# Beryl2000/SE-UNet-AirSeg

Measured on AMD Instinct MI355X. Metric: voxels/sec SE-UNet fwd+bwd, 128^3 patch, higher is better.
Workload: dtype bf16

## Files before the change

### include/seunet_hip.h

```cpp
#ifndef SEUNET_HIP_H
#define SEUNET_HIP_H
#include <stddef.h>

#ifdef __cplusplus
extern "C" {
#endif

#ifndef SEUNET_F32
#define SEUNET_F32 0
#define SEUNET_BF16 1
#define SEUNET_F16 2
#endif
#define SEUNET_CONV_MFMA 0
#define SEUNET_CONV_NAIVE 1
#define SEUNET_CONV_MARCH 2
#define SEUNET_CONV_TILED 3

typedef void* seunet_stream_t;
typedef struct seunet_dims { int n, d, h, w; } seunet_dims;

int seunet_version(void);
const char* seunet_last_error(void);
int seunet_init(int device);

int seunet_pack_cl(int dtype, const float* in_ncdhw, int c, void* out_cl, int c_pad, seunet_dims dims, seunet_stream_t s);
int seunet_unpack_cl(int dtype, const void* in_cl, int c, float* out_ncdhw, seunet_dims dims, seunet_stream_t s);

size_t seunet_conv_wpack_bytes(int dtype, int taps, int cin, int cout);
int seunet_conv_pack_weights(int dtype, const float* w, int taps, int cin, int cout, int transpose_flip, void* wpack, seunet_stream_t s);
int seunet_conv_stats_slots(int impl, int taps, int dilation, seunet_dims dims);
int seunet_conv3d_fwd(int dtype, int impl, int taps, int dilation, int nsrc, const void* const* src, const int* src_c,
                      int cin, const void* weights, int transpose_flip, const float* bias, int ndst, void* const* dst,
                      const int* dst_c, const int* dst_accumulate, double* stats_partial, seunet_dims dims, seunet_stream_t s);
int seunet_conv3d_stream_supported(int dtype, int dilation, int src_c, int dst_c);
size_t seunet_conv3d_stream_wpack_bytes(int src_c);
int seunet_conv3d_stream_slots(int dilation, seunet_dims dims);
int seunet_conv3d_stream_pack(int dtype, const float* w, int cin_w, int cout_w, int transpose_flip, int src_c, int dst_c, void* wpack,
                              seunet_stream_t s);
int seunet_conv3d_stream(int dtype, int dilation, const void* src, int src_c, const void* wpack, const float* bias, void* dst, int dst_c,
                         int dst_accumulate, double* stats_partial, seunet_dims dims, seunet_stream_t s);
int seunet_conv3d_march_supported(int dtype, int dilation, int nsrc, const int* src_c, int ndst, const int* dst_c);
size_t seunet_conv3d_march_wpack_bytes(int cin, int cout);
int seunet_conv3d_march_slots(int dilation, int cin, int cout, seunet_dims dims);
int seunet_conv3d_march_pack(int dtype, const float* w, int cin_w, int cout_w, int transpose_flip, int cin, int cout, void* wpack,
                             seunet_stream_t s);
int seunet_conv3d_march(int dtype, int dilation, int nsrc, const void* const* src, const int* src_c, const void* wpack, const float* bias,
                        int ndst, void* const* dst, const int* dst_c, const int* dst_accumulate, double* stats_partial, seunet_dims dims,
                        seunet_stream_t s);
int seunet_conv3d_wgrad_stream_supported(int dtype, int dilation, int x_c, int dy_c);
size_t seunet_conv3d_wgrad_stream_workspace_bytes(int x_c, int dy_c, int dilation, seunet_dims dims);
int seunet_conv3d_wgrad_stream(int dtype, int dilation, const void* x, int x_c, int cin, const void* dy, int dy_c, int cout, float* dw,
                               void* workspace, size_t workspace_bytes, seunet_dims dims, seunet_stream_t s);
size_t seunet_conv3d_wgrad_workspace_bytes(int taps, int cin, int cout);
int seunet_conv3d_wgrad(int dtype, int impl, int taps, int dilation, int nsrc, const void* const* src, const int* src_c,
                        int cin, const void* dy, int cout, float* dw, void* workspace, size_t workspace_bytes,
                        seunet_dims dims, seunet_stream_t s);

int seunet_epilogue_slots(seunet_dims dims);
int seunet_channel_stats(int dtype, const void* t, int c, double* partial, seunet_dims dims, seunet_stream_t s);
int seunet_stats_finalize(const double* partial, int slots, int c, int n, long long count, float eps, int mode,
                          float* out_a, float* out_b, seunet_stream_t s);

int seunet_gate_epilogue_fwd(int dtype, const void* raw, const float* mean, const float* rstd, int c, const float* w_se,
                             const float* w_se2, const float* w_side, const float* b_side, float slope, void* e_out,
                             float* side_out, float* level_map, int level_accumulate, const float* head_w,
                             const float* drop, int drop_stride, seunet_dims dims, seunet_stream_t s);
int seunet_gate_epilogue_bwd(int dtype, const void* raw, const float* mean, const float* rstd, int c, const float* w_se,
                             const float* w_se2, const float* w_side, const float* b_side, float slope, const void* g_e,
                             const float* g_side, const float* g_level, const float* head_w, const float* drop,
                             int drop_stride, const float* m1, const float* m2, void* draw_out, double* stat_partial,
                             float* pgrad_partial, seunet_dims dims, seunet_stream_t s);
int seunet_pgrad_reduce(const float* pgrad_partial, int records, int c, float* dw_se, float* dw_se2, float* dw_side,
                        float* db_side, float* dhead_w, seunet_stream_t s);
int seunet_gate_bwd_finalize(const double* stat_partial, int slots, int c, int n, long long count, float* m1, float* m2,
                             const float* pgrad_partial, int records, float* dw_se, float* dw_se2, float* dw_side,
                             float* db_side, float* dhead_w, seunet_stream_t s);

int seunet_cat_epilogue_fwd(int dtype, const void* raw, const float* mean, const float* rstd, const void* raw2,
                            const float* mean2, const float* rstd2, int c, float slope, void* out, seunet_dims dims,
                            seunet_stream_t s);
int seunet_cat_epilogue_bwd(int dtype, const void* g_out, const void* raw, const float* mean, const float* rstd,
                            const void* raw2, const float* mean2, const float* rstd2, int c, float slope,
                            const float* m1, const float* m2, const float* m1b, const float* m2b, void* dx, void* dx2,
                            double* stat_partial, double* stat_partial2, seunet_dims dims, seunet_stream_t s);

int seunet_xbranch_moment_slots(seunet_dims dims);
int seunet_xbranch_moments(int dtype, const void* x_in, double* partial , seunet_dims dims, seunet_stream_t s);
int seunet_xbranch_stats(const double* partial, int slots, const float* w2, int c, int in_channel, int n, long long count,
                         float eps, float* mean2, float* rstd2, double* moments_out , seunet_stream_t s);
int seunet_cat_epilogue_fwd_x(int dtype, const void* raw, const float* mean, const float* rstd, const void* x_in,
                              const float* w2, int in_channel, const float* mean2, const float* rstd2, int c, float slope,
                              void* out, seunet_dims dims, seunet_stream_t s);
int seunet_cat_epilogue_bwd_x(int dtype, const void* g_out, const void* raw, const float* mean, const float* rstd,
                              const void* x_in, const float* w2, int in_channel, const float* mean2, const float* rstd2,
                              int c, float slope, const float* m1, const float* m2, const float* m1b, const float* m2b,
                              void* dx, double* stat_partial, double* stat_partial2, double* xw_partial, seunet_dims dims,
                              seunet_stream_t s);
int seunet_cat_epilogue_fwd_x_pool(int dtype, const void* raw, const float* mean, const float* rstd, const void* x_in,
                                   const float* w2, int in_channel, const float* mean2, const float* rstd2, int c, float slope,
                                   void* out, void* pooled, unsigned int* argmax, seunet_dims dims, seunet_stream_t s);
int seunet_cat_epilogue_bwd_x_pool(int dtype, const void* g_out, const void* raw, const float* mean, const float* rstd,
                                   const void* x_in, const float* w2, int in_channel, const float* mean2, const float* rstd2,
                                   int c, float slope, const float* m1, const float* m2, const float* m1b, const float* m2b,
                                   void* dx, double* stat_partial, double* stat_partial2, double* xw_partial,
                                   const unsigned int* pool_argmax, const void* pool_g, seunet_dims dims, seunet_stream_t s);
int seunet_cat_xgrad_finalize(const double* xw_partial, const double* stat_partial2, int slots, const double* moments,
                              const float* w2, int c, int in_channel, int n, float eps, float* dw, seunet_stream_t s);

int seunet_maxpool_fwd(int dtype, const void* in, int c, void* out, seunet_dims in_dims, seunet_stream_t s);
int seunet_maxpool_bwd(int dtype, const void* in, const void* g_out, int c, void* g_in, int accumulate,
                       seunet_dims in_dims, seunet_stream_t s);
int seunet_upsample2_fwd(int dtype, const void* in, int c, void* out, seunet_dims in_dims, seunet_stream_t s);
int seunet_upsample2_bwd(int dtype, const void* g_out, int c, void* g_in, int accumulate, seunet_dims in_dims,
                         seunet_stream_t s);
int seunet_side_upsample(const float* side, int c, int scale, float* out_ncdhw, int c_total, int c_off,
                         seunet_dims low_dims, seunet_stream_t s);

int seunet_head_fwd(const float* const* level_maps, int nlevels, const float* bias, float* pred, seunet_dims dims,
                    seunet_stream_t s);
size_t seunet_head_bwd_tmp_floats(seunet_dims dims);
int seunet_head_bwd(const float* g_pred, float* const* g_levels, int nlevels, float* tmp, float* g_bias,
                    seunet_dims dims, seunet_stream_t s);

#define SEUNET_LOSS_DICE 1
#define SEUNET_LOSS_GUL 2
#define SEUNET_LOSS_ATR 4
int seunet_loss_partial_floats(void);
int seunet_loss_sums(const float* pred, int apply_sigmoid, const float* target, const float* weight, const float* skel,
                     long long n, float* partial, double* sums, int terms, seunet_stream_t s);
int seunet_loss_value(const double* sums0, double c_dice0, double c_gul0, double c_atr0, const double* sums1, double c_dice1,
                      double c_gul1, double c_atr1, float* value, seunet_stream_t s);
int seunet_loss_grad(const float* pred, int apply_sigmoid, const float* target, const float* weight, const float* skel,
                     long long n, const double* sums, float c_dice, float c_gul, float c_atr, float g_scale,
                     const float* g_scale_dev, float* g_pred, seunet_stream_t s);

int seunet_loss_sample_partial_floats(int batch);
int seunet_loss_sums_per_sample(const float* pred, int apply_sigmoid, const float* target, const float* weight, const float* skel,
                                int batch, long long n_per_sample, float* partial, double* sums, int terms, seunet_stream_t s);
int seunet_loss_sample_values(const double* sums, int batch, double c_dice, double c_gul, double c_atr, float* values,
                              seunet_stream_t s);

int seunet_pool_select(const float* new_keys, int batch, float* keys, long long* seq, long long* state, int capacity, int* slots_out,
                       seunet_stream_t s);
int seunet_pool_scatter(const int* slots_dev, int batch, int capacity, long long voxels, const float* data, const float* label,
                        const float* weight, const float* skel, float* pool_data, unsigned char* pool_label, float* pool_weight,
                        unsigned char* pool_skel, seunet_stream_t s);
int seunet_pool_gather(const int* slots_host, int n, int capacity, long long voxels, const float* pool_data,
                       const unsigned char* pool_label, const float* pool_weight, const unsigned char* pool_skel, float* data_out,
                       float* label_out, float* weight_out, float* skel_out, seunet_stream_t s);

int seunet_adamw_step(float* const* params, const float* const* grads, float* const* exp_avg, float* const* exp_avg_sq,
                      const long long* counts, int n_tensors, double lr, double beta1, double beta2, double eps,
                      double weight_decay, int step, int maximize, seunet_stream_t s);

#define SEUNET_IMG_I16 0
#define SEUNET_IMG_F32 1
#define SEUNET_W_F16 0
#define SEUNET_W_F32 1
#define SEUNET_W_F64 2
int seunet_crop_batch(const void* img, int img_dtype, const unsigned char* label, const void* weight, int weight_dtype,
                      const unsigned char* skeleton, int d, int h, int w, int cube, int ncrop, const int* starts, const int* aug,
                      double weight_exponent, int f64_math, float* data_out, float* label_out, float* weight_out, float* skel_out,
                      seunet_stream_t s);
int seunet_hu_two_channel(const void* img, int img_dtype, long long nvox, int f64_math, float* out, seunet_stream_t s);

int seunet_window_gather(const float* volume, int c, int x, int y, int z, int cube, int nwin, const int* starts, float* out,
                         seunet_stream_t s);
int seunet_window_accumulate(const float* logits, int apply_sigmoid, int nwin, const int* starts, int cube, double* acc, int x, int y,
                             int z, seunet_stream_t s);
int seunet_window_finalize(const double* acc, int x, int y, int z, int cube, int nx, const int* xs, int ny, const int* ys, int nz,
                           const int* zs, int dup0, double* out, seunet_stream_t s);

#define SEUNET_DTI_F64 0
#define SEUNET_DTI_F32 1
size_t seunet_dti_workspace_bytes(int h, int w, int z);
int seunet_dti(const double* pred, int h, int w, int z, double h_thresh, double l_thresh, int pred_dtype, unsigned char* out,
               void* workspace, size_t workspace_bytes, seunet_stream_t s);

#define SEUNET_CC_EVALUATION 0
#define SEUNET_CC_MAXIMUM_3D 1
#define SEUNET_CC_LARGEST_FILLED 2
size_t seunet_cc_workspace_bytes(int h, int w, int z);
int seunet_largest_component(const unsigned char* volume, int h, int w, int z, int rule, unsigned char* out, int* status_dev,
                             void* workspace, size_t workspace_bytes, seunet_stream_t s);
size_t seunet_metric_out_bytes(int nbins);
int seunet_metric_sums(const unsigned char* pred, const unsigned char* label, const unsigned char* skeleton, const int* parsing,
                       long long n, int nbins, void* out, size_t out_bytes, seunet_stream_t s);

size_t seunet_edt_workspace_bytes(int n0, int n1, int n2);
int seunet_edt(const unsigned char* volume, int n0, int n1, int n2, int* sqdist, double* dist, int* indices, int* status_dev,
               void* workspace, size_t workspace_bytes, seunet_stream_t s);
int seunet_mask_bits(const unsigned char* mask, long long n, unsigned long long* bits, seunet_stream_t s);
int seunet_hard_mining_masks(const unsigned char* label, const unsigned char* skeleton, const unsigned char* pred, int n0, int n1,
                             int n2, unsigned long long* skeleton_bits, unsigned long long* small_bits, seunet_stream_t s);
size_t seunet_lib_weight_workspace_bytes(int n0, int n1, int n2);
int seunet_lib_weight(const unsigned char* label, int n0, int n1, int n2, const float* table, void* out, void* workspace,
                      size_t workspace_bytes, seunet_stream_t s);
size_t seunet_break_weight_workspace_bytes(int n0, int n1, int n2);
int seunet_break_weight(const unsigned char* label, const unsigned char* pred, const unsigned char* skeleton, int n0, int n1, int n2,
                        void* w_br, unsigned char* br_skel, int* status_dev, void* workspace, size_t workspace_bytes,
                        seunet_stream_t s);

size_t seunet_skeleton_workspace_bytes(int n0, int n1, int n2);
int seunet_skeletonize(const unsigned char* volume, int n0, int n1, int n2, unsigned char* out, int* passes_dev, void* workspace,
                       size_t workspace_bytes, seunet_stream_t s);

size_t seunet_skeleton_branches_workspace_bytes(int n0, int n1, int n2);
int seunet_skeleton_branches(const unsigned char* skeleton, int n0, int n1, int n2, int min_voxels, int* cd, unsigned char* skeleton_parse,
                             int* num_dev, void* workspace, size_t workspace_bytes, seunet_stream_t s);
size_t seunet_parse_assign_workspace_bytes(int n0, int n1, int n2);
int seunet_parse_assign(const unsigned char* skeleton_parse, const int* cd, const unsigned char* label, int n0, int n1, int n2,
                        int* parsing, int* status_dev, void* workspace, size_t workspace_bytes, seunet_stream_t s);
int seunet_label_stats_max_num(void);
int seunet_label_stats(const int* parsing, int n0, int n1, int n2, int num, unsigned int* counts, unsigned long long* adjacency_bits,
                       int* status_dev, seunet_stream_t s);
int seunet_relabel(const int* parsing, long long n, const int* lut, int nlut, int* out, seunet_stream_t s);

#define SEUNET_MORPH_DILATE 0
#define SEUNET_MORPH_ERODE_BORDER0 1
#define SEUNET_MORPH_ERODE_BORDER1 2
#define SEUNET_MORPH_CLOSE 3
size_t seunet_binary_morph_workspace_bytes(int n0, int n1, int n2);
int seunet_binary_morph(const unsigned char* volume, int n0, int n1, int n2, int op, unsigned char* out, void* workspace,
                        size_t workspace_bytes, seunet_stream_t s);
int seunet_fill_holes(const unsigned char* volume, int n0, int n1, int n2, unsigned char* out, void* workspace, size_t workspace_bytes,
                      seunet_stream_t s);
int seunet_slice_moments(const unsigned char* mask, int n0, int n1, int n2, int k, unsigned long long* out_dev, seunet_stream_t s);
int seunet_scatter_labels(const long long* lin_index_dev, const int* value_dev, long long m, long long n, int* cd,
                          unsigned char* skeleton_parse, int* status_dev, seunet_stream_t s);

size_t seunet_mesh_workspace_bytes(int n0, int n1, int n2);
int seunet_mesh_count(const unsigned char* volume, int n0, int n1, int n2, long long* nverts, long long* nfaces, void* workspace,
                      size_t workspace_bytes, seunet_stream_t s);
int seunet_mesh_emit(int n0, int n1, int n2, double level, long long nverts, long long nfaces, float* verts, int* faces,
                     const void* workspace, size_t workspace_bytes, seunet_stream_t s);
int seunet_mesh_coord_sums(const unsigned char* mask, int n0, int n1, int n2, long long* sums_dev, seunet_stream_t s);
size_t seunet_mesh_adjacency_workspace_bytes(long long nverts, long long nfaces);
int seunet_mesh_adjacency(const int* faces, long long nfaces, long long nverts, int* indptr, int* indices, long long indices_capacity,
                          unsigned char* boundary, int* status_dev, void* workspace, size_t workspace_bytes, seunet_stream_t s);
int seunet_mesh_smooth(const float* verts, long long nverts, const int* indptr, const int* indices, const unsigned char* boundary,
                       int n_iter, float relaxation_factor, float* out, float* tmp, seunet_stream_t s);
int seunet_mesh_affine(const float* verts, long long nverts, const float* centre, const float* scale, float* out, seunet_stream_t s);
int seunet_mesh_stl_records(const float* verts, long long nverts, const int* faces, long long nfaces, const float* centre,
                            const float* scale, unsigned char* records, int* status_dev, seunet_stream_t s);

size_t seunet_mesh_label_workspace_bytes(int n0, int n1, int n2);
size_t seunet_mesh_label_sort_bytes(long long nverts, long long nfaces);
int seunet_mesh_label_count(const int* labels, int n0, int n1, int n2, int num, long long* nverts, long long* nfaces, int* num_used,
                            int* status, long long* vert_ptr_dev, long long* face_ptr_dev, int ptr_capacity, void* workspace,
                            size_t workspace_bytes, seunet_stream_t s);
int seunet_mesh_label_emit(const int* labels, int n0, int n1, int n2, int num, double level, long long nverts, long long nfaces,
                           float* verts, int* faces, const void* workspace, size_t workspace_bytes, void* sort_workspace,
                           size_t sort_bytes, seunet_stream_t s);

int seunet_value_counts(const short* ct, long long n, int shift, unsigned int* counts, seunet_stream_t s);
int seunet_shift_clamp(const short* ct, long long n, int shift, int clamp, int clamp_le, int clamp_to, short* out, seunet_stream_t s);
size_t seunet_get_l_workspace_bytes(int h, int w, int z);
int seunet_get_l(const short* ct, int h, int w, int z, double T, int min_area, unsigned char* out, void* workspace,
                 size_t workspace_bytes, seunet_stream_t s);
int seunet_mask_combine(const unsigned char* a, const unsigned char* b, long long n, int op, unsigned char* out, seunet_stream_t s);
int seunet_mask_box(const unsigned char* mask, int h, int w, int z, int* box_dev, seunet_stream_t s);
int seunet_crop3d(const void* src, int elem_bytes, int h, int w, int z, const int* box, void* dst, seunet_stream_t s);

typedef struct seunet_net_desc {
  int batch, in_channel, n_classes;
  int d, h, w;
  int width_mult;
  int dtype;
  int conv_impl;
  float negative_slope;
  float eps;
} seunet_net_desc;

int seunet_net_param_count(const seunet_net_desc* desc);
int seunet_net_param_info(const seunet_net_desc* desc, int index, char* name, int name_cap, int* shape5, int* ndim);
size_t seunet_net_workspace_bytes(const seunet_net_desc* desc);
int seunet_net_forward(const seunet_net_desc* desc, const float* const* params, const float* x, const float* drop1,
                       const float* drop2, float* pred0, float* pred1, void* workspace, size_t workspace_bytes,
                       seunet_stream_t s);
int seunet_net_forward_capture(const seunet_net_desc* desc, const float* const* params, const float* x, const float* drop1,
                               const float* drop2, float* pred0, float* pred1, void* workspace, size_t workspace_bytes,
                               seunet_stream_t s, void** graph_out);
int seunet_graph_launch(void* graph, seunet_stream_t s);
int seunet_graph_destroy(void* graph);
int seunet_net_read_tensor(const seunet_net_desc* desc, const float* const* params, const void* workspace, size_t workspace_bytes,
                           const char* name, int which, float* out, int* channels, seunet_stream_t s);
#define SEUNET_KERNEL_NAIVE 0
#define SEUNET_KERNEL_TILED 1
#define SEUNET_KERNEL_STREAM 2
#define SEUNET_KERNEL_MARCH 3
#define SEUNET_KERNEL_WGRAD1X1 4
typedef struct seunet_conv_info {
  char name[16];
  int taps, dilation, level;
  seunet_dims dims;
  int nsrc, src_c[3], src_is_input[3];
  int cin, cout;
  int need_dgrad;
  int fwd, dgrad, wgrad;
  char x_name[16];
  int x_materialised, x_fwd, x_wgrad;
  long long src_dist;
} seunet_conv_info;
int seunet_net_conv_info(const seunet_net_desc* desc, int index, seunet_conv_info* out);
int seunet_net_backward(const seunet_net_desc* desc, const float* const* params, const float* g_pred0,
                        const float* g_pred1, const float* drop1, const float* drop2, float* const* grads,
                        void* workspace, size_t workspace_bytes, seunet_stream_t s);
int seunet_net_backward_ev(const seunet_net_desc* desc, const float* const* params, const float* g_pred0,
                           const float* g_pred1, const float* drop1, const float* drop2, float* const* grads,
                           void* workspace, size_t workspace_bytes, seunet_stream_t s, void* decoder_done_event);
size_t seunet_net_input_grad_bytes(const seunet_net_desc* desc);
int seunet_net_backward_input(const seunet_net_desc* desc, const float* const* params, const float* g_pred0,
                              const float* g_pred1, const float* drop1, const float* drop2, float* const* grads, float* grad_x,
                              void* scratch, size_t scratch_bytes, void* workspace, size_t workspace_bytes, seunet_stream_t s,
                              void* decoder_done_event);

int seunet_prof_enable(int on);
int seunet_prof_enable_filtered(const char* tag_substring);
int seunet_prof_report(char* buf, size_t cap);

#ifdef __cplusplus
}
#endif
#endif
```

### se-unet-airseg_amd/_lib.py

```python
from __future__ import annotations

import ctypes as C
import os
from typing import Optional, Sequence

_HERE = os.path.dirname(os.path.abspath(__file__))
LIB_PATH = os.environ.get("SEUNET_LIB") or os.path.join(_HERE, "libseunet_hip.so")

F32, BF16, F16 = 0, 1, 2
CONV_MFMA, CONV_NAIVE, CONV_MARCH, CONV_TILED = 0, 1, 2, 3
LOSS_NSUMS = 7
DTI_F64, DTI_F32 = 0, 1
CC_EVALUATION, CC_MAXIMUM_3D, CC_LARGEST_FILLED = 0, 1, 2
MORPH_DILATE, MORPH_ERODE_BORDER0, MORPH_ERODE_BORDER1, MORPH_CLOSE = 0, 1, 2, 3


class Dims(C.Structure):
    _fields_ = [("n", C.c_int), ("d", C.c_int), ("h", C.c_int), ("w", C.c_int)]


class NetDesc(C.Structure):
    _fields_ = [("batch", C.c_int), ("in_channel", C.c_int), ("n_classes", C.c_int),
                ("d", C.c_int), ("h", C.c_int), ("w", C.c_int), ("width_mult", C.c_int),
                ("dtype", C.c_int), ("conv_impl", C.c_int),
                ("negative_slope", C.c_float), ("eps", C.c_float)]


KERNEL_NAIVE, KERNEL_TILED, KERNEL_STREAM, KERNEL_MARCH, KERNEL_WGRAD1X1 = range(5)
KERNEL_NAMES = ("Naive", "Tiled", "Stream", "March", "Wgrad1x1")


class ConvInfo(C.Structure):
    _fields_ = [("name", C.c_char * 16), ("taps", C.c_int), ("dilation", C.c_int), ("level", C.c_int), ("dims", Dims),
                ("nsrc", C.c_int), ("src_c", C.c_int * 3), ("src_is_input", C.c_int * 3), ("cin", C.c_int), ("cout", C.c_int),
                ("need_dgrad", C.c_int), ("fwd", C.c_int), ("dgrad", C.c_int), ("wgrad", C.c_int),
                ("x_name", C.c_char * 16), ("x_materialised", C.c_int), ("x_fwd", C.c_int), ("x_wgrad", C.c_int),
                ("src_dist", C.c_longlong)]


_vp, _i, _f, _ll, _sz, _d =C.c_void_p, C.c_int, C.c_float, C.c_longlong, C.c_size_t, C.c_double
_pp = C.POINTER(C.c_void_p)
_ip = C.POINTER(C.c_int)

PROTOTYPES = {
    "seunet_version": (_i, []),
    "seunet_last_error": (C.c_char_p, []),
    "seunet_pack_cl": (_i, [_i, _vp, _i, _vp, _i, Dims, _vp]),
    "seunet_unpack_cl": (_i, [_i, _vp, _i, _vp, Dims, _vp]),
    "seunet_conv_wpack_bytes": (_sz, [_i, _i, _i, _i]),
    "seunet_conv_pack_weights": (_i, [_i, _vp, _i, _i, _i, _i, _vp, _vp]),
    "seunet_conv_stats_slots": (_i, [_i, _i, _i, Dims]),
    "seunet_conv3d_fwd": (_i, [_i, _i, _i, _i, _i, _pp, _ip, _i, _vp, _i, _vp, _i, _pp, _ip, _ip, _vp, Dims, _vp]),
    "seunet_conv3d_stream_supported": (_i, [_i, _i, _i, _i]),
    "seunet_conv3d_stream_wpack_bytes": (_sz, [_i]),
    "seunet_conv3d_stream_slots": (_i, [_i, Dims]),
    "seunet_conv3d_stream_pack": (_i, [_i, _vp, _i, _i, _i, _i, _i, _vp, _vp]),
    "seunet_conv3d_stream": (_i, [_i, _i, _vp, _i, _vp, _vp, _vp, _i, _i, _vp, Dims, _vp]),
    "seunet_conv3d_march_supported": (_i, [_i, _i, _i, _ip, _i, _ip]),
    "seunet_conv3d_march_wpack_bytes": (_sz, [_i, _i]),
    "seunet_conv3d_march_slots": (_i, [_i, _i, _i, Dims]),
    "seunet_conv3d_march_pack": (_i, [_i, _vp, _i, _i, _i, _i, _i, _vp, _vp]),
    "seunet_conv3d_march": (_i, [_i, _i, _i, _pp, _ip, _vp, _vp, _i, _pp, _ip, _ip, _vp, Dims, _vp]),
    "seunet_conv3d_wgrad_stream_supported": (_i, [_i, _i, _i, _i]),
    "seunet_conv3d_wgrad_stream_workspace_bytes": (_sz, [_i, _i, _i, Dims]),
    "seunet_conv3d_wgrad_stream": (_i, [_i, _i, _vp, _i, _i, _vp, _i, _i, _vp, _vp, _sz, Dims, _vp]),
    "seunet_conv3d_wgrad_workspace_bytes": (_sz, [_i, _i, _i]),
    "seunet_conv3d_wgrad": (_i, [_i, _i, _i, _i, _i, _pp, _ip, _i, _vp, _i, _vp, _vp, _sz, Dims, _vp]),
    "seunet_epilogue_slots": (_i, [Dims]),
    "seunet_channel_stats": (_i, [_i, _vp, _i, _vp, Dims, _vp]),
    "seunet_stats_finalize": (_i, [_vp, _i, _i, _i, _ll, _f, _i, _vp, _vp, _vp]),
    "seunet_gate_epilogue_fwd": (_i, [_i, _vp, _vp, _vp, _i, _vp, _vp, _vp, _vp, _f, _vp, _vp, _vp, _i, _vp, _vp, _i, Dims, _vp]),
    "seunet_gate_epilogue_bwd": (_i, [_i, _vp, _vp, _vp, _i, _vp, _vp, _vp, _vp, _f, _vp, _vp, _vp, _vp, _vp, _i, _vp, _vp, _vp, _vp, _vp, Dims, _vp]),
    "seunet_pgrad_reduce": (_i, [_vp, _i, _i, _vp, _vp, _vp, _vp, _vp, _vp]),
    "seunet_gate_bwd_finalize": (_i, [_vp, _i, _i, _i, _ll, _vp, _vp, _vp, _i, _vp, _vp, _vp, _vp, _vp, _vp]),
    "seunet_cat_epilogue_fwd": (_i, [_i, _vp, _vp, _vp, _vp, _vp, _vp, _i, _f, _vp, Dims, _vp]),
    "seunet_cat_epilogue_bwd": (_i, [_i, _vp, _vp, _vp, _vp, _vp, _vp, _vp, _i, _f, _vp, _vp, _vp, _vp, _vp, _vp, _vp, _vp, Dims, _vp]),
    "seunet_maxpool_fwd": (_i, [_i, _vp, _i, _vp, Dims, _vp]),
    "seunet_maxpool_bwd": (_i, [_i, _vp, _vp, _i, _vp, _i, Dims, _vp]),
    "seunet_upsample2_fwd": (_i, [_i, _vp, _i, _vp, Dims, _vp]),
    "seunet_upsample2_bwd": (_i, [_i, _vp, _i, _vp, _i, Dims, _vp]),
    "seunet_side_upsample": (_i, [_vp, _i, _i, _vp, _i, _i, Dims, _vp]),
    "seunet_head_fwd": (_i, [_pp, _i, _vp, _vp, Dims, _vp]),
    "seunet_head_bwd_tmp_floats": (_sz, [Dims]),
    "seunet_head_bwd": (_i, [_vp, _pp, _i, _vp, _vp, Dims, _vp]),
    "seunet_loss_partial_floats": (_i, []),
    "seunet_loss_sums": (_i, [_vp, _i, _vp, _vp, _vp, _ll, _vp, _vp, _i, _vp]),
    "seunet_loss_value": (_i, [_vp, _d, _d, _d, _vp, _d, _d, _d, _vp, _vp]),
    "seunet_loss_grad": (_i, [_vp, _i, _vp, _vp, _vp, _ll, _vp, _f, _f, _f, _f, _vp, _vp, _vp]),
    "seunet_loss_sample_partial_floats": (_i, [_i]),
    "seunet_loss_sums_per_sample": (_i, [_vp, _i, _vp, _vp, _vp, _i, _ll, _vp, _vp, _i, _vp]),
    "seunet_loss_sample_values": (_i, [_vp, _i, _d, _d, _d, _vp, _vp]),
    "seunet_pool_select": (_i, [_vp, _i, _vp, _vp, _vp, _i, _vp, _vp]),
    "seunet_pool_scatter": (_i, [_vp, _i, _i, _ll, _vp, _vp, _vp, _vp, _vp, _vp, _vp, _vp, _vp]),
    "seunet_pool_gather": (_i, [_ip, _i, _i, _ll, _vp, _vp, _vp, _vp, _vp, _vp, _vp, _vp, _vp]),
    "seunet_xbranch_moment_slots": (_i, [Dims]),
    "seunet_xbranch_moments": (_i, [_i, _vp, _vp, Dims, _vp]),
    "seunet_xbranch_stats": (_i, [_vp, _i, _vp, _i, _i, _i, _ll, _f, _vp, _vp, _vp, _vp]),
    "seunet_cat_epilogue_fwd_x": (_i, [_i, _vp, _vp, _vp, _vp, _vp, _i, _vp, _vp, _i, _f, _vp, Dims, _vp]),
    "seunet_cat_epilogue_bwd_x": (_i, [_i, _vp, _vp, _vp, _vp, _vp, _vp, _i, _vp, _vp, _i, _f, _vp, _vp, _vp, _vp, _vp, _vp, _vp, _vp, Dims, _vp]),
    "seunet_cat_epilogue_fwd_x_pool": (_i, [_i, _vp, _vp, _vp, _vp, _vp, _i, _vp, _vp, _i, _f, _vp, _vp, _vp, Dims, _vp]),
    "seunet_cat_epilogue_bwd_x_pool": (_i, [_i, _vp, _vp, _vp, _vp, _vp, _vp, _i, _vp, _vp, _i, _f, _vp, _vp, _vp, _vp, _vp, _vp, _vp, _vp, _vp, _vp, Dims, _vp]),
    "seunet_cat_xgrad_finalize": (_i, [_vp, _vp, _i, _vp, _vp, _i, _i, _i, _f, _vp, _vp]),
    "seunet_cc_workspace_bytes": (_sz, [_i, _i, _i]),
    "seunet_largest_component": (_i, [_vp, _i, _i, _i, _i, _vp, _vp, _vp, _sz, _vp]),
    "seunet_metric_out_bytes": (_sz, [_i]),
    "seunet_metric_sums": (_i, [_vp, _vp, _vp, _vp, _ll, _i, _vp, _sz, _vp]),
    "seunet_value_counts": (_i, [_vp, _ll, _i, _vp, _vp]),
    "seunet_shift_clamp": (_i, [_vp, _ll, _i, _i, _i, _i, _vp, _vp]),
    "seunet_get_l_workspace_bytes": (_sz, [_i, _i, _i]),
    "seunet_get_l": (_i, [_vp, _i, _i, _i, _d, _i, _vp, _vp, _sz, _vp]),
    "seunet_mask_combine": (_i, [_vp, _vp, _ll, _i, _vp, _vp]),
    "seunet_mask_box": (_i, [_vp, _i, _i, _i, _vp, _vp]),
    "seunet_crop3d": (_i, [_vp, _i, _i, _i, _i, _ip, _vp, _vp]),
    "seunet_crop_batch": (_i, [_vp, _i, _vp, _vp, _i, _vp, _i, _i, _i, _i, _i, _ip, _ip, C.c_double, _i, _vp, _vp, _vp, _vp, _vp]),
    "seunet_hu_two_channel": (_i, [_vp, _i, _ll, _i, _vp, _vp]),
    "seunet_window_gather": (_i, [_vp, _i, _i, _i, _i, _i, _i, _ip, _vp, _vp]),
    "seunet_window_accumulate": (_i, [_vp, _i, _i, _ip, _i, _vp, _i, _i, _i, _vp]),
    "seunet_window_finalize": (_i, [_vp, _i, _i, _i, _i, _i, _ip, _i, _ip, _i, _ip, _i, _vp, _vp]),
    "seunet_dti_workspace_bytes": (_sz, [_i, _i, _i]),
    "seunet_dti": (_i, [_vp, _i, _i, _i, C.c_double, C.c_double, _i, _vp, _vp, _sz, _vp]),
    "seunet_edt_workspace_bytes": (_sz, [_i, _i, _i]),
    "seunet_edt": (_i, [_vp, _i, _i, _i, _vp, _vp, _vp, _vp, _vp, _sz, _vp]),
    "seunet_mask_bits": (_i, [_vp, _ll, _vp, _vp]),
    "seunet_hard_mining_masks": (_i, [_vp, _vp, _vp, _i, _i, _i, _vp, _vp, _vp]),
    "seunet_lib_weight_workspace_bytes": (_sz, [_i, _i, _i]),
    "seunet_lib_weight": (_i, [_vp, _i, _i, _i, _vp, _vp, _vp, _sz, _vp]),
    "seunet_break_weight_workspace_bytes": (_sz, [_i, _i, _i]),
    "seunet_break_weight": (_i, [_vp, _vp, _vp, _i, _i, _i, _vp, _vp, _vp, _vp, _sz, _vp]),
    "seunet_skeleton_workspace_bytes": (_sz, [_i, _i, _i]),
    "seunet_skeletonize": (_i, [_vp, _i, _i, _i, _vp, _vp, _vp, _sz, _vp]),
    "seunet_skeleton_branches_workspace_bytes": (_sz, [_i, _i, _i]),
    "seunet_skeleton_branches": (_i, [_vp, _i, _i, _i, _i, _vp, _vp, _vp, _vp, _sz, _vp]),
    "seunet_parse_assign_workspace_bytes": (_sz, [_i, _i, _i]),
    "seunet_parse_assign": (_i, [_vp, _vp, _vp, _i, _i, _i, _vp, _vp, _vp, _sz, _vp]),
    "seunet_label_stats_max_num": (_i, []),
    "seunet_label_stats": (_i, [_vp, _i, _i, _i, _i, _vp, _vp, _vp, _vp]),
    "seunet_relabel": (_i, [_vp, _ll, _vp, _i, _vp, _vp]),
    "seunet_binary_morph_workspace_bytes": (_sz, [_i, _i, _i]),
    "seunet_binary_morph": (_i, [_vp, _i, _i, _i, _i, _vp, _vp, _sz, _vp]),
    "seunet_fill_holes": (_i, [_vp, _i, _i, _i, _vp, _vp, _sz, _vp]),
    "seunet_slice_moments": (_i, [_vp, _i, _i, _i, _i, _vp, _vp]),
    "seunet_scatter_labels": (_i, [_vp, _vp, _ll, _ll, _vp, _vp, _vp, _vp]),
    "seunet_mesh_workspace_bytes": (_sz, [_i, _i, _i]),
    "seunet_mesh_count": (_i, [_vp, _i, _i, _i, C.POINTER(_ll), C.POINTER(_ll), _vp, _sz, _vp]),
    "seunet_mesh_emit": (_i, [_i, _i, _i, _d, _ll, _ll, _vp, _vp, _vp, _sz, _vp]),
    "seunet_mesh_label_workspace_bytes": (_sz, [_i, _i, _i]),
    "seunet_mesh_label_sort_bytes": (_sz, [_ll, _ll]),
    "seunet_mesh_label_count": (_i, [_vp, _i, _i, _i, _i, C.POINTER(_ll), C.POINTER(_ll), _ip, _ip, _vp, _vp, _i, _vp, _sz, _vp]),
    "seunet_mesh_label_emit": (_i, [_vp, _i, _i, _i, _i, _d, _ll, _ll, _vp, _vp, _vp, _sz, _vp, _sz, _vp]),
    "seunet_mesh_coord_sums": (_i, [_vp, _i, _i, _i, _vp, _vp]),
    "seunet_mesh_adjacency_workspace_bytes": (_sz, [_ll, _ll]),
    "seunet_mesh_adjacency": (_i, [_vp, _ll, _ll, _vp, _vp, _ll, _vp, _vp, _vp, _sz, _vp]),
    "seunet_mesh_smooth": (_i, [_vp, _ll, _vp, _vp, _vp, _i, _f, _vp, _vp, _vp]),
    "seunet_mesh_affine": (_i, [_vp, _ll, C.POINTER(_f), C.POINTER(_f), _vp, _vp]),
    "seunet_mesh_stl_records": (_i, [_vp, _ll, _vp, _ll, C.POINTER(_f), C.POINTER(_f), _vp, _vp, _vp]),
    "seunet_adamw_step": (_i, [_vp, _vp, _vp, _vp, _vp, _i, C.c_double, C.c_double, C.c_double, C.c_double, C.c_double, _i, _i, _vp]),
    "seunet_net_param_count": (_i, [C.POINTER(NetDesc)]),
    "seunet_net_param_info": (_i, [C.POINTER(NetDesc), _i, C.c_char_p, _i, _ip, _ip]),
    "seunet_net_workspace_bytes": (_sz, [C.POINTER(NetDesc)]),
    "seunet_net_forward": (_i, [C.POINTER(NetDesc), _pp, _vp, _vp, _vp, _vp, _vp, _vp, _sz, _vp]),
    "seunet_prof_enable": (_i, [_i]),
    "seunet_prof_enable_filtered": (_i, [C.c_char_p]),
    "seunet_prof_report": (_i, [C.c_char_p, _sz]),
    "seunet_init": (_i, [_i]),
    "seunet_net_forward_capture": (_i, [C.POINTER(NetDesc), _pp, _vp, _vp, _vp, _vp, _vp, _vp, _sz, _vp, C.POINTER(C.c_void_p)]),
    "seunet_graph_launch": (_i, [_vp, _vp]),
    "seunet_graph_destroy": (_i, [_vp]),
    "seunet_net_read_tensor": (_i, [C.POINTER(NetDesc), _pp, _vp, _sz, C.c_char_p, _i, _vp, _ip, _vp]),
    "seunet_net_conv_info": (_i, [C.POINTER(NetDesc), _i, C.POINTER(ConvInfo)]),
    "seunet_net_backward": (_i, [C.POINTER(NetDesc), _pp, _vp, _vp, _vp, _vp, _pp, _vp, _sz, _vp]),
    "seunet_net_backward_ev": (_i, [C.POINTER(NetDesc), _pp, _vp, _vp, _vp, _vp, _pp, _vp, _sz, _vp, _vp]),
    "seunet_net_input_grad_bytes": (_sz, [C.POINTER(NetDesc)]),
    "seunet_net_backward_input": (_i, [C.POINTER(NetDesc), _pp, _vp, _vp, _vp, _vp, _pp, _vp, _vp, _sz, _vp, _sz, _vp, _vp]),
}

_lib: Optional[C.CDLL] = None


def load() -> C.CDLL:
    global _lib
    if _lib is not None:
        return _lib
    if not os.path.exists(LIB_PATH):
        raise RuntimeError(
            f"{LIB_PATH} is missing: build it with `python -c 'import __graft_entry__ as g; g.build()'` "
            "(or `make -C se-unet-airseg_amd/csrc`).  There is no CPU or PyTorch fallback for the HIP path.")
    lib = C.CDLL(LIB_PATH)
    for name, (res, args) in PROTOTYPES.items():
        fn = getattr(lib, name)
        fn.restype, fn.argtypes = res, args
    _lib = lib
    return lib


def last_error() -> str:
    return load().seunet_last_error().decode(errors="replace")


def check(status: int, what: str = "") -> None:
    if status != 0:
        raise RuntimeError(f"libseunet_hip {what}: {last_error()}")


def ptr(t) -> Optional[int]:
    return None if t is None else t.data_ptr()


def ptr_array(tensors: Sequence) -> C.Array:
    arr = (C.c_void_p * len(tensors))()
    for i, t in enumerate(tensors):
        arr[i] = None if t is None else (t if isinstance(t, int) else t.data_ptr())
    return arr


def int_array(vals: Sequence[int]) -> C.Array:
    return (C.c_int * len(vals))(*vals)


def stream_ptr() -> int:
    import torch
    return torch.cuda.current_stream().cuda_stream


def dtype_code(name: str) -> int:
    name = str(name).lower().replace("torch.", "")
    if name in ("bf16", "bfloat16"):
        return BF16
    if name in ("fp32", "f32", "float32", "float"):
        return F32
    if name in ("fp16", "f16", "float16", "half"):
        return F16
    raise ValueError(f"unsupported activation dtype {name!r} (fp32, bf16 or fp16)")
```

### se-unet-airseg_amd/csrc/abi.cpp

```cpp
#include "seunet_common.h"
#include "epilogue.h"
#include "volume.h"
#include "../../include/seunet_hip.h"

using namespace seunet;

static inline Dims D(seunet_dims d) { return Dims{d.n, d.d, d.h, d.w}; }
static inline hipStream_t S(seunet_stream_t s) { return reinterpret_cast<hipStream_t>(s); }

static int make_src(int nsrc, const void* const* src, const int* src_c, SrcList& l) {
  SEUNET_CHECK(nsrc >= 1 && nsrc <= 3 && src && src_c, "bad source list");
  l = SrcList{};
  l.n = nsrc;
  for (int i = 0; i < nsrc; ++i) { l.ptr[i] = src[i]; l.C[i] = src_c[i]; }
  return 0;
}

namespace seunet { extern unsigned long long* g_conv_debug; }

extern "C" {

int seunet_debug_set_buffer(void* p) { seunet::g_conv_debug = reinterpret_cast<unsigned long long*>(p); return 0; }
int seunet_debug_upsample2_form(int dtype, int c, seunet_dims dims, int backward) { return upsample2_form(dtype, c, D(dims), backward != 0); }

int seunet_debug_volume_layout(int op, int n0, int n1, int n2, size_t* offsets, int cap) {
  if (n0 < 1 || n1 < 1 || n2 < 1) return 0;
  size_t at[16];
  WsCarver c(nullptr);
  c.log = at;
  c.log_cap = 16;
  switch (op) {
    case 0: cc_ws(c, n0, n1, n2); break;
    case 1: get_l_ws(c, n0, n1, n2); break;
    case 2: case 8: edt_ws(c, n0, n1, n2); break;
    case 3: lib_weight_ws(c, n0, n1, n2); break;
    case 4: break_weight_ws(c, n0, n1, n2); break;
    case 5: branches_ws(c, n0, n1, n2); break;
    case 6: dti_ws(c, n0, n1, n2); break;
    case 7: if (!skeleton_ws(c, n0, n1, n2)) return 0; break;
    case 9: morph_ws(c, n0, n1, n2); break;
    case 10: if ((long long)n0 * n1 * n2 >= (1ll << 31)) return 0; mesh_ws(c, n0, n1, n2); break;
    case 11: if ((long long)n0 * n1 * n2 >= (1ll << 31)) return 0; mesh_label_ws(c, n0, n1, n2); break;
    default: return -1;
  }
  if (c.taken > c.log_cap) return -1;
  for (int i = 0; i < c.taken && i < cap && offsets; ++i) {
    offsets[2 * i] = at[i];
    offsets[2 * i + 1] = (i + 1 < c.taken ? at[i + 1] : c.bytes()) - at[i];
  }
  return c.taken;
}

int seunet_version(void) { return 201; }
const char* seunet_last_error(void) { return get_error(); }

int seunet_init(int device) {
  int count = 0, prev = 0;
  SEUNET_HIP(hipGetDeviceCount(&count));
  SEUNET_CHECK(device >= 0 && device < count, "init: device %d out of range (%d visible)", device, count);
  SEUNET_HIP(hipGetDevice(&prev));
  SEUNET_HIP(hipSetDevice(device));
  const void* page = seunet::device_zero_page();
  (void)hipSetDevice(prev);
  SEUNET_CHECK(page != nullptr, "init: could not allocate the zero page on device %d", device);
  return 0;
}

int seunet_pack_cl(int dtype, const float* in, int c, void* out, int c_pad, seunet_dims dims, seunet_stream_t s) {
  SEUNET_CHECK(in && out, "pack_cl: null tensor");
  return launch_pack_cl(dtype, in, c, out, c_pad, D(dims), S(s));
}
int seunet_unpack_cl(int dtype, const void* in, int c, float* out, seunet_dims dims, seunet_stream_t s) {
  SEUNET_CHECK(in && out, "unpack_cl: null tensor");
  return launch_unpack_cl(dtype, in, c, out, D(dims), S(s));
}

size_t seunet_conv_wpack_bytes(int dtype, int taps, int cin, int cout) { return conv_wpack_bytes(dtype, taps, cin, cout); }
int seunet_conv_pack_weights(int dtype, const float* w, int taps, int cin, int cout, int tflip, void* wpack, seunet_stream_t s) {
  SEUNET_CHECK(w && wpack, "conv_pack_weights: null tensor");
  return launch_conv_pack_weights(dtype, w, taps, cin, cout, tflip, wpack, S(s));
}
int seunet_conv_stats_slots(int impl, int taps, int dilation, seunet_dims dims) {
  return impl == SEUNET_CONV_NAIVE ? epi_partials(D(dims)) : conv_stats_tiles(D(dims), taps, dilation);
}
int seunet_conv3d_fwd(int dtype, int impl, int taps, int dilation, int nsrc, const void* const* src, const int* src_c, int cin,
                      const void* weights, int tflip, const float* bias, int ndst, void* const* dst, const int* dst_c,
                      const int* dst_acc, double* stats_partial, seunet_dims dims, seunet_stream_t s) {
  SrcList sl;
  if (int e = make_src(nsrc, src, src_c, sl)) return e;
  SEUNET_CHECK(ndst >= 1 && ndst <= 3 && dst && dst_c && weights, "conv3d_fwd: bad destination list / weights");
  DstList dl{};
  dl.n = ndst;
  for (int i = 0; i < ndst; ++i) { dl.ptr[i] = dst[i]; dl.C[i] = dst_c[i]; dl.acc[i] = dst_acc ? dst_acc[i] : 0; }
  if (impl == SEUNET_CONV_NAIVE) {
    if (int e = launch_conv_naive(dtype, taps, dilation, sl, cin, (const float*)weights, tflip, bias, dl, D(dims), S(s))) return e;
    if (stats_partial) {
      SEUNET_CHECK(ndst == 1, "conv3d_fwd: statistics need a single destination");
      return launch_channel_stats(dtype, dst[0], dst_c[0], stats_partial, D(dims), S(s));
    }
    return 0;
  }
  return launch_conv_igemm(dtype, taps, dilation, sl, cin, weights, bias, dl, stats_partial, D(dims), S(s));
}
int seunet_conv3d_stream_supported(int dtype, int dilation, int src_c, int dst_c) { return conv_stream_supported(dtype, 27, dilation, src_c, dst_c) ? 1 : 0; }
size_t seunet_conv3d_stream_wpack_bytes(int src_c) { return conv_stream_wpack_bytes(src_c); }
int seunet_conv3d_stream_slots(int dilation, seunet_dims dims) { return conv_stream_slots(D(dims), dilation); }
int seunet_conv3d_stream_pack(int dtype, const float* w, int cin_w, int cout_w, int transpose_flip, int src_c, int dst_c, void* wpack,
                              seunet_stream_t s) {
  return launch_conv_stream_pack(dtype, w, cin_w, cout_w, transpose_flip, src_c, dst_c, wpack, S(s));
}
int seunet_conv3d_stream(int dtype, int dilation, const void* src, int src_c, const void* wpack, const float* bias, void* dst, int dst_c,
                         int dst_accumulate, double* stats_partial, seunet_dims dims, seunet_stream_t s) {
  return launch_conv_stream(dtype, dilation, src, src_c, wpack, bias, dst, dst_c, dst_accumulate, stats_partial, D(dims), S(s));
}
static int make_dst(int ndst, void* const* dst, const int* dst_c, const int* dst_acc, DstList& dl) {
  SEUNET_CHECK(ndst >= 1 && ndst <= 3 && dst_c, "bad destination list");
  dl = DstList{};
  dl.n = ndst;
  for (int i = 0; i < ndst; ++i) { dl.ptr[i] = dst ? dst[i] : nullptr; dl.C[i] = dst_c[i]; dl.acc[i] = dst_acc ? dst_acc[i] : 0; }
  return 0;
}
int seunet_conv3d_march_supported(int dtype, int dilation, int nsrc, const int* src_c, int ndst, const int* dst_c) {
  if (nsrc < 1 || nsrc > 3 || ndst < 1 || ndst > 3 || !src_c || !dst_c) return 0;
  SrcList sl{}; DstList dl{};
  sl.n = nsrc; dl.n = ndst;
  for (int i = 0; i < nsrc; ++i) sl.C[i] = src_c[i];
  for (int i = 0; i < ndst; ++i) dl.C[i] = dst_c[i];
  return conv_march_supported(dtype, 27, dilation, sl, dl) ? 1 : 0;
}
size_t seunet_conv3d_march_wpack_bytes(int cin, int cout) { return conv_march_wpack_bytes(cin, cout); }
int seunet_conv3d_march_slots(int dilation, int cin, int cout, seunet_dims dims) { return conv_march_slots(D(dims), dilation, cin, cout); }
int seunet_conv3d_march_pack(int dtype, const float* w, int cin_w, int cout_w, int transpose_flip, int cin, int cout, void* wpack,
                             seunet_stream_t s) {
  return launch_conv_march_pack(dtype, w, cin_w, cout_w, transpose_flip, cin, cout, wpack, S(s));
}
int seunet_conv3d_march(int dtype, int dilation, int nsrc, const void* const* src, const int* src_c, const void* wpack, const float* bias,
                        int ndst, void* const* dst, const int* dst_c, const int* dst_accumulate, double* stats_partial, seunet_dims dims,
                        seunet_stream_t s) {
  SrcList sl; DstList dl;
  if (int e = make_src(nsrc, src, src_c, sl)) return e;
  SEUNET_CHECK(dst != nullptr, "conv3d_march: null destination list");
  if (int e = make_dst(ndst, dst, dst_c, dst_accumulate, dl)) return e;
  return launch_conv_march(dtype, dilation, sl, wpack, bias, dl, stats_partial, D(dims), S(s));
}
int seunet_conv3d_wgrad_stream_supported(int dtype, int dilation, int x_c, int dy_c) { return wgrad_stream_supported(dtype, 27, dilation, x_c, dy_c) ? 1 : 0; }
size_t seunet_conv3d_wgrad_stream_workspace_bytes(int x_c, int dy_c, int dilation, seunet_dims dims) {
  return wgrad_stream_workspace_bytes(x_c, dy_c, dilation, D(dims));
}
int seunet_conv3d_wgrad_stream(int dtype, int dilation, const void* x, int x_c, int cin, const void* dy, int dy_c, int cout, float* dw,
                               void* workspace, size_t workspace_bytes, seunet_dims dims, seunet_stream_t s) {
  return launch_wgrad_stream(dtype, dilation, x, x_c, cin, dy, dy_c, cout, dw, workspace, workspace_bytes, D(dims), S(s));
}
size_t seunet_conv3d_wgrad_workspace_bytes(int taps, int cin, int cout) { return wgrad_workspace_bytes(taps, cin, cout); }
int seunet_conv3d_wgrad(int dtype, int impl, int taps, int dilation, int nsrc, const void* const* src, const int* src_c, int cin,
                        const void* dy, int cout, float* dw, void* workspace, size_t workspace_bytes, seunet_dims dims,
                        seunet_stream_t s) {
  SrcList sl;
  if (int e = make_src(nsrc, src, src_c, sl)) return e;
  SEUNET_CHECK(dy && dw, "conv3d_wgrad: null tensor");
  if (impl == SEUNET_CONV_NAIVE) return launch_wgrad_naive(dtype, taps, dilation, sl, cin, dy, cout, dw, D(dims), S(s));
  SEUNET_CHECK(workspace, "conv3d_wgrad: null workspace");
  const ConvKernel k = impl == SEUNET_CONV_MARCH ? (taps == 1 ? ConvKernel::Wgrad1x1 : ConvKernel::March)
                       : impl == SEUNET_CONV_TILED ? ConvKernel::Tiled
                                                   : wgrad_kernel(dtype, taps, dilation, sl, cin, cout, D(dims), sl.gap());
  return run_wgrad(k, dtype, taps, dilation, sl, cin, dy, cout, dw, workspace, workspace_bytes, D(dims), S(s));
}

int seunet_epilogue_slots(seunet_dims dims) { return epi_partials(D(dims)); }
int seunet_channel_stats(int dtype, const void* t, int c, double* partial, seunet_dims dims, seunet_stream_t s) {
  SEUNET_CHECK(t && partial, "channel_stats: null tensor");
  return launch_channel_stats(dtype, t, c, partial, D(dims), S(s));
}
int seunet_stats_finalize(const double* partial, int slots, int c, int n, long long count, float eps, int mode, float* out_a,
                          float* out_b, seunet_stream_t s) {
  SEUNET_CHECK(partial && out_a && out_b && slots >= 1 && count >= 1, "stats_finalize: bad argument");
  return launch_stats_finalize(partial, slots, c, n, count, eps, mode, out_a, out_b, S(s));
}

int seunet_gate_epilogue_fwd(int dtype, const void* raw, const float* mean, const float* rstd, int c, const float* w_se,
                             const float* w_se2, const float* w_side, const float* b_side, float slope, void* e_out,
                             float* side_out, float* level_map, int level_accumulate, const float* head_w, const float* drop,
                             int drop_stride, seunet_dims dims, seunet_stream_t s) {
  SEUNET_CHECK(raw && mean && rstd && w_se && w_side && b_side && e_out, "gate_epilogue_fwd: null tensor");
  SEUNET_CHECK(!level_map || head_w, "gate_epilogue_fwd: level_map needs head_w");
  const GateBlock b{{raw, mean, rstd}, c, {w_se, w_se2, w_side, b_side, slope}};
  SseHead h{side_out, level_map, level_accumulate, head_w, drop, drop_stride};
  return launch_sse_fwd(dtype, b, e_out, h, D(dims), S(s));
}
int seunet_gate_epilogue_bwd(int dtype, const void* raw, const float* mean, const float* rstd, int c, const float* w_se,
                             const float* w_se2, const float* w_side, const float* b_side, float slope, const void* g_e,
                             const float* g_side, const float* g_level, const float* head_w, const float* drop, int drop_stride,
                             const float* m1, const float* m2, void* draw_out, double* stat_partial, float* pgrad_partial,
                             seunet_dims dims, seunet_stream_t s) {
  SEUNET_CHECK(raw && mean && rstd && w_se && w_side && b_side, "gate_epilogue_bwd: null tensor");
  SEUNET_CHECK(!g_level || head_w, "gate_epilogue_bwd: g_level needs head_w");
  const GateBlock b{{raw, mean, rstd}, c, {w_se, w_se2, w_side, b_side, slope}};
  SseBwdIn g{g_e, g_side, g_level};
  SseHead h{nullptr, nullptr, 0, head_w, drop, drop_stride};
  if (m1 == nullptr) return launch_sse_bwd_sums(dtype, b, g, h, {stat_partial, pgrad_partial}, D(dims), S(s));
  return launch_sse_bwd_apply(dtype, b, g, h, {m1, m2, draw_out}, D(dims), S(s));
}
int seunet_pgrad_reduce(const float* pgrad_partial, int records, int c, float* dw_se, float* dw_se2, float* dw_side,
                        float* db_side, float* dhead_w, seunet_stream_t s) {
  SEUNET_CHECK(pgrad_partial && records >= 1, "pgrad_reduce: bad argument");
  return launch_pgrad_reduce(pgrad_partial, records, c, dw_se, dw_se2, dw_side, db_side, dhead_w, S(s));
}
int seunet_gate_bwd_finalize(const double* stat_partial, int slots, int c, int n, long long count, float* m1, float* m2,
                             const float* pgrad_partial, int records, float* dw_se, float* dw_se2, float* dw_side,
                             float* db_side, float* dhead_w, seunet_stream_t s) {
  SEUNET_CHECK(stat_partial && m1 && m2 && pgrad_partial && slots >= 1 && n >= 1 && count >= 1, "gate_bwd_finalize: bad argument");
  SEUNET_CHECK(c % 8 == 0 && c >= 8 && c <= 128 && (c & (c - 1)) == 0, "channel count %d must be a power of two in [8,128]", c);
  SEUNET_CHECK(records == n * slots, "gate_bwd_finalize: records=%d, pass A wrote n * slots = %d", records, n * slots);
  return launch_gate_bwd_finalize(stat_partial, slots, c, n, count, m1, m2, pgrad_partial, records, dw_se, dw_se2, dw_side,
                                  db_side, dhead_w, S(s));
}
static int cat_epilogue_bwd(int dtype, const CatBlock& b, const void* g_out, const PoolGrad& pool, const float* m1, const float* m2,
                            const float* m1b, const float* m2b, void* dx, void* dx2, double* stat_partial, double* stat_partial2,
                            double* xw_partial, seunet_dims dims, seunet_stream_t s) {
  if (m1 == nullptr) return launch_cat_bwd_sums(dtype, b, g_out, pool, {stat_partial, stat_partial2, xw_partial}, D(dims), S(s));
  return launch_cat_bwd_apply(dtype, b, g_out, pool, {m1, m2, m1b, m2b, dx, dx2, nullptr, 0}, D(dims), S(s));
}
int seunet_cat_epilogue_fwd(int dtype, const void* raw, const float* mean, const float* rstd, const void* raw2,
                            const float* mean2, const float* rstd2, int c, float slope, void* out, seunet_dims dims,
                            seunet_stream_t s) {
  SEUNET_CHECK(raw && mean && rstd && out && (!raw2 || (mean2 && rstd2)), "cat_epilogue_fwd: null tensor");
  const CatBlock b{{raw, mean, rstd}, {raw2 ? Branch2::Stored : Branch2::None, raw2, mean2, rstd2, nullptr, 0}, c, slope};
  return launch_cat_fwd(dtype, b, out, PoolOut{}, D(dims), S(s));
}
int seunet_cat_epilogue_bwd(int dtype, const void* g_out, const void* raw, const float* mean, const float* rstd,
                            const void* raw2, const float* mean2, const float* rstd2, int c, float slope, const float* m1,
                            const float* m2, const float* m1b, const float* m2b, void* dx, void* dx2, double* stat_partial,
                            double* stat_partial2, seunet_dims dims, seunet_stream_t s) {
  SEUNET_CHECK(g_out && raw && mean && rstd, "cat_epilogue_bwd: null tensor");
  SEUNET_CHECK(!raw2 || (mean2 && rstd2), "cat_epilogue_bwd: second branch incomplete");
  const CatBlock b{{raw, mean, rstd}, {raw2 ? Branch2::Stored : Branch2::None, raw2, mean2, rstd2, nullptr, 0}, c, slope};
  return cat_epilogue_bwd(dtype, b, g_out, PoolGrad{}, m1, m2, m1b, m2b, dx, dx2, stat_partial, stat_partial2, nullptr, dims, s);
}

int seunet_maxpool_fwd(int dtype, const void* in, int c, void* out, seunet_dims d, seunet_stream_t s) {
  SEUNET_CHECK(in && out, "maxpool_fwd: null tensor");
  return launch_maxpool_fwd(dtype, in, c, out, D(d), S(s));
}
int seunet_maxpool_bwd(int dtype, const void* in, const void* g_out, int c, void* g_in, int accumulate, seunet_dims d,
                       seunet_stream_t s) {
  SEUNET_CHECK(in && g_out && g_in, "maxpool_bwd: null tensor");
  return launch_maxpool_bwd(dtype, in, g_out, c, g_in, accumulate, D(d), S(s));
}
int seunet_upsample2_fwd(int dtype, const void* in, int c, void* out, seunet_dims d, seunet_stream_t s) {
  SEUNET_CHECK(in && out, "upsample2_fwd: null tensor");
  return launch_upsample2_fwd(dtype, in, c, out, D(d), S(s));
}
int seunet_upsample2_bwd(int dtype, const void* g_out, int c, void* g_in, int accumulate, seunet_dims d, seunet_stream_t s) {
  SEUNET_CHECK(g_out && g_in, "upsample2_bwd: null tensor");
  return launch_upsample2_bwd(dtype, g_out, c, g_in, accumulate, D(d), S(s));
}
int seunet_side_upsample(const float* side, int c, int scale, float* out, int c_total, int c_off, seunet_dims low,
                         seunet_stream_t s) {
  SEUNET_CHECK(side && out && scale >= 1, "side_upsample: bad argument");
  return launch_side_upsample(side, c, scale, out, c_total, c_off, D(low), S(s));
}

int seunet_head_fwd(const float* const* level_maps, int nlevels, const float* bias, float* pred, seunet_dims d, seunet_stream_t s) {
  SEUNET_CHECK(level_maps && bias && pred, "head_fwd: null tensor");
  return launch_head_fwd(level_maps, nlevels, bias, pred, D(d), S(s));
}
size_t seunet_head_bwd_tmp_floats(seunet_dims d) { return head_bwd_tmp_floats(D(d)); }
int seunet_head_bwd(const float* g_pred, float* const* g_levels, int nlevels, float* tmp, float* g_bias, seunet_dims d,
                    seunet_stream_t s) {
  SEUNET_CHECK(g_pred && g_levels && tmp, "head_bwd: null tensor");
  return launch_head_bwd(g_pred, g_levels, nlevels, tmp, g_bias, D(d), S(s));
}

int seunet_loss_partial_floats(void) { return loss_partials() * SEUNET_LOSS_NSUMS; }
int seunet_loss_sums(const float* pred, int apply_sigmoid, const float* target, const float* weight, const float* skel,
                     long long n, float* partial, double* sums, int terms, seunet_stream_t s) {
  SEUNET_CHECK(pred && target && partial && sums && n >= 1, "loss_sums: bad argument");
  SEUNET_CHECK(terms >= 0 && terms <= 7, "loss_sums: terms=%d is not a mask of SEUNET_LOSS_DICE | _GUL | _ATR", terms);
  return launch_loss_sums(pred, apply_sigmoid, target, weight, skel, n, partial, sums, S(s), terms);
}
int seunet_loss_value(const double* sums0, double c_dice0, double c_gul0, double c_atr0, const double* sums1, double c_dice1,
                      double c_gul1, double c_atr1, float* value, seunet_stream_t s) {
  SEUNET_CHECK(sums0 && value, "loss_value: null argument");
  return launch_loss_value(sums0, c_dice0, c_gul0, c_atr0, sums1, c_dice1, c_gul1, c_atr1, value, S(s));
}
int seunet_loss_grad(const float* pred, int apply_sigmoid, const float* target, const float* weight, const float* skel,
                     long long n, const double* sums, float c_dice, float c_gul, float c_atr, float g_scale,
                     const float* g_scale_dev, float* g_pred, seunet_stream_t s) {
  SEUNET_CHECK(pred && target && sums && g_pred && n >= 1, "loss_grad: bad argument");
  return launch_loss_grad(pred, apply_sigmoid, target, weight, skel, n, sums, c_dice, c_gul, c_atr, g_scale, g_scale_dev, g_pred, S(s));
}

int seunet_loss_sample_partial_floats(int batch) {
  if (batch < 1 || batch > 65535) { fail("loss_sample_partial_floats: batch %d (1..65535)", batch); return 0; }
  return loss_sample_partials(batch) * SEUNET_LOSS_NSUMS;
}
int seunet_loss_sums_per_sample(const float* pred, int apply_sigmoid, const float* target, const float* weight, const float* skel,
                                int batch, long long n_per_sample, float* partial, double* sums, int terms, seunet_stream_t s) {
  SEUNET_CHECK(pred && target && partial && sums && n_per_sample >= 1, "loss_sums_per_sample: bad argument");
  SEUNET_CHECK(batch >= 1 && batch <= 65535, "loss_sums_per_sample: batch %d (1..65535)", batch);
  SEUNET_CHECK(terms >= 0 && terms <= 7, "loss_sums_per_sample: terms=%d is not a mask of SEUNET_LOSS_DICE | _GUL | _ATR", terms);
  return launch_loss_sums_per_sample(pred, apply_sigmoid, target, weight, skel, batch, n_per_sample, partial, sums, terms, S(s));
}
int seunet_loss_sample_values(const double* sums, int batch, double c_dice, double c_gul, double c_atr, float* values, seunet_stream_t s) {
  SEUNET_CHECK(sums && values && batch >= 1, "loss_sample_values: bad argument");
  return launch_loss_sample_values(sums, batch, c_dice, c_gul, c_atr, values, S(s));
}

int seunet_pool_select(const float* new_keys, int batch, float* keys, long long* seq, long long* state, int capacity, int* slots_out,
                       seunet_stream_t s) {
  return launch_pool_select(new_keys, batch, keys, seq, state, capacity, slots_out, S(s));
}
int seunet_pool_scatter(const int* slots_dev, int batch, int capacity, long long voxels, const float* data, const float* label,
                        const float* weight, const float* skel, float* pool_data, unsigned char* pool_label, float* pool_weight,
                        unsigned char* pool_skel, seunet_stream_t s) {
  return launch_pool_scatter(slots_dev, batch, capacity, voxels, data, label, weight, skel, pool_data, pool_label, pool_weight, pool_skel,
                             S(s));
}
int seunet_pool_gather(const int* slots_host, int n, int capacity, long long voxels, const float* pool_data,
                       const unsigned char* pool_label, const float* pool_weight, const unsigned char* pool_skel, float* data_out,
                       float* label_out, float* weight_out, float* skel_out, seunet_stream_t s) {
// ... 285 lines not shown
```

### se-unet-airseg_amd/csrc/net.cpp

```cpp
#include "seunet_common.h"
#include "epilogue.h"
#include "../../include/seunet_hip.h"

#include <algorithm>
#include <cstdio>
#include <cstdlib>
#include <cstring>
#include <string>
#include <vector>

namespace seunet {
namespace {

struct BlockDesc { const char* name; char kind; int cin; int cout; };
const BlockDesc kBlocks[] = {
    {"ec1", 'g', -1, 8},   {"ec2", 'g', 8, 16},    {"ec3", 'g', 16, 32},  {"ec33", 'c', 56, 32},  {"x33", 'c', -1, 32},
    {"ec4", 'G', 32, 32},  {"ec5", 'G', 32, 32},   {"ec6", 'G', 32, 64},  {"ec63", 'c', 128, 64}, {"x63", 'c', -1, 64},
    {"ec7", 'G', 64, 64},  {"ec8", 'G', 64, 64},   {"ec9", 'G', 64, 64},  {"ec93", 'c', 192, 64}, {"x93", 'c', -1, 64},
    {"ec10", 'G', 64, 64}, {"ec11", 'G', 64, 64},  {"ec12", 'G', 64, 64}, {"ec123", 'c', 192, 64},
    {"dc1", 'G', 128, 64}, {"dc2", 'G', 64, 64},   {"dc22", 'c', 128, 64},
    {"dc3", 'G', 128, 64}, {"dc4", 'G', 64, 32},   {"dc42", 'c', 96, 32},
    {"dc5", 'g', 64, 32},  {"dc6", 'g', 32, 16},   {"dc62", 'c', 48, 16},
};
constexpr int kNumBlocks = sizeof(kBlocks) / sizeof(kBlocks[0]);
// ... 46 lines not shown
    {0, 8}, {0, 16}, {0, 32}, {0, 32}, {1, 32}, {1, 32}, {1, 32}, {1, 64}, {1, 64}, {2, 64}, {2, 64}, {2, 64}, {2, 64}, {2, 64},
    {3, 64}, {3, 64}, {3, 64}, {3, 64}, {3, 64}, {2, 64}, {2, 64}, {2, 64}, {2, 64}, {1, 64}, {1, 64}, {1, 32}, {1, 32}, {0, 32}, {0, 32}, {0, 16},
};

enum OpKind { OP_GATED, OP_CAT, OP_POOL, OP_UP };
struct OpDesc {
  OpKind kind; const char* name; int nsrc; int src[3]; int dst;
  int dil; int gates; int head; int m;
  const char* xname; int xsrc;
};
const OpDesc kOps[] = {
    {OP_GATED, "ec1", 1, {T_X0, 0, 0}, T_E0, 1, 1, 0, 0, nullptr, 0},
    {OP_GATED, "ec2", 1, {T_E0, 0, 0}, T_E1A, 1, 1, 0, 1, nullptr, 0},
    {OP_GATED, "ec3", 1, {T_E1A, 0, 0}, T_E1_1, 2, 1, 0, 2, nullptr, 0},
    {OP_CAT, "ec33", 3, {T_E1_1, T_E0, T_E1A}, T_E1, 0, 0, 0, 0, "x33", T_X0},
    {OP_POOL, "pool0", 1, {T_E1, 0, 0}, T_E2IN, 0, 0, 0, 0, nullptr, 0},
    {OP_POOL, "pool0x", 1, {T_X0, 0, 0}, T_X1, 0, 0, 0, 0, nullptr, 0},
    {OP_GATED, "ec4", 1, {T_E2IN, 0, 0}, T_E2, 1, 2, 0, 3, nullptr, 0},
    {OP_GATED, "ec5", 1, {T_E2, 0, 0}, T_E3A, 2, 2, 0, 4, nullptr, 0},
    {OP_GATED, "ec6", 1, {T_E3A, 0, 0}, T_E3_1, 2, 2, 0, 5, nullptr, 0},
    {OP_CAT, "ec63", 3, {T_E3_1, T_E2, T_E3A}, T_E3, 0, 0, 0, 0, "x63", T_X1},
    {OP_POOL, "pool1", 1, {T_E3, 0, 0}, T_E4IN, 0, 0, 0, 0, nullptr, 0},
    {OP_POOL, "pool1x", 1, {T_X1, 0, 0}, T_X2, 0, 0, 0, 0, nullptr, 0},
    {OP_GATED, "ec7", 1, {T_E4IN, 0, 0}, T_E4, 1, 2, 0, 6, nullptr, 0},
    {OP_GATED, "ec8", 1, {T_E4, 0, 0}, T_E5A, 2, 2, 0, 7, nullptr, 0},
    {OP_GATED, "ec9", 1, {T_E5A, 0, 0}, T_E5_1, 2, 2, 0, 8, nullptr, 0},
    {OP_CAT, "ec93", 3, {T_E5_1, T_E4, T_E5A}, T_E5, 0, 0, 0, 0, "x93", T_X2},
    {OP_POOL, "pool2", 1, {T_E5, 0, 0}, T_E6IN, 0, 0, 0, 0, nullptr, 0},
    {OP_GATED, "ec10", 1, {T_E6IN, 0, 0}, T_E6, 1, 2, 0, 9, nullptr, 0},
    {OP_GATED, "ec11", 1, {T_E6, 0, 0}, T_E7A, 1, 2, 0, 10, nullptr, 0},
    {OP_GATED, "ec12", 1, {T_E7A, 0, 0}, T_E7_1, 1, 2, 0, 11, nullptr, 0},
    {OP_CAT, "ec123", 3, {T_E7_1, T_E6, T_E7A}, T_E7, 0, 0, 0, 0, nullptr, 0},
    {OP_UP, "up0", 1, {T_E7, 0, 0}, T_E8, 0, 0, 0, 0, nullptr, 0},
    {OP_GATED, "dc1", 2, {T_E8, T_E5, 0}, T_D0A, 1, 2, 1, 0, nullptr, 0},
    {OP_GATED, "dc2", 1, {T_D0A, 0, 0}, T_D0_1, 1, 2, 1, 1, nullptr, 0},
    {OP_CAT, "dc22", 2, {T_D0_1, T_D0A, 0}, T_D0, 0, 0, 0, 0, nullptr, 0},
    {OP_UP, "up1", 1, {T_D0, 0, 0}, T_D1U, 0, 0, 0, 0, nullptr, 0},
    {OP_GATED, "dc3", 2, {T_D1U, T_E3, 0}, T_D1A, 1, 2, 1, 2, nullptr, 0},
    {OP_GATED, "dc4", 1, {T_D1A, 0, 0}, T_D1_1, 1, 2, 1, 3, nullptr, 0},
    {OP_CAT, "dc42", 2, {T_D1_1, T_D1A, 0}, T_D1, 0, 0, 0, 0, nullptr, 0},
    {OP_UP, "up2", 1, {T_D1, 0, 0}, T_D2U, 0, 0, 0, 0, nullptr, 0},
    {OP_GATED, "dc5", 2, {T_D2U, T_E1, 0}, T_D2A, 1, 1, 1, 4, nullptr, 0},
    {OP_GATED, "dc6", 1, {T_D2A, 0, 0}, T_D2_1, 1, 1, 1, 5, nullptr, 0},
};
constexpr int kNumOps = sizeof(kOps) / sizeof(kOps[0]);

inline bool is_input(int t) { return t <= T_X2; }

inline bool march_level(const Dims& d, int dil) {
  return d.W >= 32 && (d.vox() >= 48LL * 48 * 48 || (dil == 2 && d.vox() >= 32LL * 32 * 32));
}

int conv_slots(ConvKernel k, const Dims& dm, int taps, int dil, int cin, int cout) {
  switch (k) {
    case ConvKernel::Stream: return conv_stream_slots(dm, dil);
    case ConvKernel::March: return conv_march_slots(dm, dil, cin, cout);
    case ConvKernel::Naive: return epi_partials(dm);
    default: return conv_stats_tiles(dm, taps, dil);
  }
}

}

ConvKernel wgrad_kernel(int dtype, int taps, int dil, const SrcList& x, int cin_logical, int cout, Dims d, long long src_dist) {
  if (taps == 1) {
    const int combos = cdiv(cin_logical, 32) * cdiv(cout, 32);
    const long long nv = (long long)d.N * d.vox();
    const bool pays = combos >= 16 || (combos >= 8 && nv >= 500000);
    return pays && wgrad_1x1_supported(dtype, x, cin_logical, cout) ? ConvKernel::Wgrad1x1 : ConvKernel::Tiled;
  }
  const bool fine = d.W >= 32 && (long long)d.D * d.H * d.W >= 48LL * 48 * 48;
  const bool pays = fine || dil == 2 || cin_logical >= 256;
  return pays && wgrad_march_supported(dtype, taps, dil, x, cin_logical, cout, d, src_dist) ? ConvKernel::March : ConvKernel::Tiled;
}

int run_wgrad(ConvKernel k, int dtype, int taps, int dil, const SrcList& x, int cin_logical, const void* dy, int cout, float* dw,
              void* workspace, size_t ws_bytes, Dims d, hipStream_t s) {
  switch (k) {
    case ConvKernel::Naive: return launch_wgrad_naive(dtype, taps, dil, x, cin_logical, dy, cout, dw, d, s);
    case ConvKernel::Tiled: return launch_wgrad(dtype, taps, dil, x, cin_logical, dy, cout, dw, workspace, ws_bytes, d, s);
    case ConvKernel::Stream:
      return launch_wgrad_stream(dtype, dil, x.ptr[0], x.C[0], cin_logical, dy, cout, cout, dw, workspace, ws_bytes, d, s);
    case ConvKernel::March: return launch_wgrad_march(dtype, taps, dil, x, cin_logical, dy, cout, dw, workspace, ws_bytes, d, s);
    case ConvKernel::Wgrad1x1: return launch_wgrad_1x1(dtype, x, cin_logical, dy, cout, dw, workspace, ws_bytes, d, s);
  }
  return fail("wgrad: unknown kernel %d", (int)k);
}

namespace {

struct OpRes {
  size_t raw = 0, raw2 = 0, mean = 0, rstd = 0, mean2 = 0, rstd2 = 0, xtot = 0, wp_f = 0, wp_d = 0, wp_x = 0;
  int cin = 0, cout = 0, taps = 0;
  bool need_dgrad = false;
  ConvKernel fwd = ConvKernel::Tiled, dgrad = ConvKernel::Tiled, wgrad = ConvKernel::Tiled;
  ConvKernel x_fwd = ConvKernel::Tiled, x_wgrad = ConvKernel::Tiled;
  size_t pool_idx = 0; bool has_pool_idx = false;
  size_t side = 0;
};

struct Plan {
  seunet_net_desc d;
  size_t esz;
  Dims dims[4];
  int C[T_COUNT];
  size_t feat[T_COUNT], grad[T_COUNT];
  OpRes op[kNumOps];
  size_t lvl[2][4], glvl[2][4];
  size_t stats, stats2, pgrad, m1, m2, m1b, m2b, wgrad_ws, head_tmp, gx, gx_bytes = 0, xwp = 0, xmom = 0;
  size_t gside = 0, cls_part = 0, cls_bias = 0;
  bool fuse_x = false;
  size_t wgrad_ws_bytes;
  size_t total;
  int stat_slots_max;
  size_t ig_gx[3] = {0, 0, 0}, ig_total = 0;
  void plan_input_grad() {
    size_t c = 0;
    for (int l = 0; l < 3; ++l) { ig_gx[l] = c; c = align_up(c + (size_t)d.batch * dims[l].vox() * d.in_channel * 4, 256); }
    ig_total = c;
  }

  size_t cur = 0;
  size_t take(size_t bytes) { size_t o = cur; cur = align_up(cur + bytes, 256); return o; }

  void route(int i) {
    const OpDesc& o = kOps[i];
    OpRes& r = op[i];
    if (d.conv_impl == SEUNET_CONV_NAIVE) { r.fwd = r.dgrad = r.wgrad = r.x_fwd = r.x_wgrad = ConvKernel::Naive; return; }
    const Dims& dm = dims[kT[o.dst].level];
    SrcList x{}, gy{};
    DstList y{}, gx{};
    x.n = gx.n = o.nsrc;
    for (int k = 0; k < o.nsrc; ++k) x.C[k] = gx.C[k] = C[o.src[k]];
    y.n = gy.n = 1;
    y.C[0] = gy.C[0] = r.cout;
    const int c0 = C[o.src[0]];
    const bool stream_ok = o.kind == OP_GATED && o.nsrc == 1 && (long long)dm.D * dm.H * dm.W * 32 * (long long)esz < 0xFFFFFFFFll;
    const bool stream_f = stream_ok && conv_stream_supported(d.dtype, 27, o.dil, c0, r.cout);
    const bool stream_d = stream_ok && conv_stream_supported(d.dtype, 27, o.dil, r.cout, c0);
    const bool march_ok = o.kind == OP_GATED && !stream_f && march_level(dm, o.dil);
    r.fwd = stream_f ? ConvKernel::Stream
          : march_ok && conv_march_supported(d.dtype, 27, o.dil, x, y) ? ConvKernel::March : ConvKernel::Tiled;
    r.dgrad = stream_d ? ConvKernel::Stream
            : march_ok && conv_march_supported(d.dtype, 27, o.dil, gy, gx) ? ConvKernel::March : ConvKernel::Tiled;
    const long long src_dist = o.nsrc == 2 ? (long long)feat[o.src[1]] - (long long)feat[o.src[0]] : 0;
    r.wgrad = stream_ok && wgrad_stream_supported(d.dtype, 27, o.dil, c0, r.cout)
                  ? ConvKernel::Stream : wgrad_kernel(d.dtype, r.taps, o.dil, x, r.cin, r.cout, dm, src_dist);
    if (o.xname) {
      SrcList xs{};
      xs.n = 1; xs.C[0] = 8;
      r.x_fwd = ConvKernel::Tiled;
      r.x_wgrad = wgrad_kernel(d.dtype, 1, 1, xs, d.in_channel, r.cout, dm, 0);
    }
  }
  size_t wpack_bytes(ConvKernel k, int taps, int src_c, int cin, int cout) const {
    switch (k) {
      case ConvKernel::Stream: return conv_stream_wpack_bytes(src_c);
      case ConvKernel::March: return conv_march_wpack_bytes(cin, cout);
      default: return conv_wpack_bytes(d.dtype, taps, cin, cout);
    }
  }

  int init(const seunet_net_desc& desc) {
    d = desc;
    SEUNET_CHECK(d.batch >= 1 && d.in_channel >= 1 && d.in_channel <= 8, "net: batch/in_channel out of range");
    SEUNET_CHECK(d.n_classes >= 1 && d.n_classes <= class_max(), "net: n_classes=%d out of range (1 .. %d)", d.n_classes, class_max());
    SEUNET_CHECK(d.d % 8 == 0 && d.h % 8 == 0 && d.w % 8 == 0 && d.d >= 8 && d.h >= 8 && d.w >= 8,
                 "net: spatial extents (%d,%d,%d) must be multiples of 8", d.d, d.h, d.w);
    SEUNET_CHECK(d.width_mult == 1 || d.width_mult == 2, "net: width_mult %d unsupported (1 or 2)", d.width_mult);
    SEUNET_CHECK(dtype_ok(d.dtype), "net: dtype %d unsupported (SEUNET_F32 | SEUNET_BF16 | SEUNET_F16)", d.dtype);
    esz = dtype_size(d.dtype);
    for (int l = 0; l < 4; ++l) dims[l] = Dims{d.batch, d.d >> l, d.h >> l, d.w >> l};
    for (int t = 0; t < T_COUNT; ++t) C[t] = kT[t].cbase == 0 ? 8 : kT[t].cbase * d.width_mult;
    bool placed[T_COUNT] = {};
    for (int t = 0; t < T_COUNT; ++t) {
      const size_t bytes = (size_t)d.batch * dims[kT[t].level].vox() * C[t] * esz;
      if (!placed[t]) { feat[t] = take(bytes); placed[t] = true; }
      const int mate = t == T_E1 ? T_D2U : -1;
      if (mate >= 0 && !placed[mate]) {
        feat[mate] = take((size_t)d.batch * dims[kT[mate].level].vox() * C[mate] * esz);
        placed[mate] = true;
      }
      grad[t] = is_input(t) ? 0 : take(bytes);
    }
    size_t gx_max = 0, wg_max = 0, xw_max = 0, xmom_max = 0;
    fuse_x = d.in_channel <= 2 && d.conv_impl != SEUNET_CONV_NAIVE;
    int slots_max = 1, cmax = 8;
    for (int i = 0; i < kNumOps; ++i) {
      const OpDesc& o = kOps[i];
      OpRes& r = op[i];
      if (o.kind == OP_POOL && i > 0 && kOps[i - 1].kind == OP_CAT && kOps[i - 1].xname && kOps[i - 1].dst == o.src[0] &&
          fuse_x && !is_input(o.src[0])) {
        const Dims& dl = dims[kT[o.dst].level];
        r.pool_idx = take((size_t)d.batch * dl.vox() * (C[o.src[0]] / 8) * 4);
        r.has_pool_idx = true;
      }
      if (o.kind == OP_POOL || o.kind == OP_UP) continue;
      const int lv = kT[o.dst].level;
      r.cout = C[o.dst];
      r.taps = o.kind == OP_GATED ? 27 : 1;
      int cin = 0;
      bool any_grad = false;
      for (int k = 0; k < o.nsrc; ++k) { cin += C[o.src[k]]; any_grad |= !is_input(o.src[k]); }
      if (o.nsrc == 1 && is_input(o.src[0])) cin = d.in_channel;
      r.cin = cin;
      r.need_dgrad = any_grad;
      const size_t act = (size_t)d.batch * dims[lv].vox() * r.cout * esz;
      r.raw = take(act);
      r.mean = take((size_t)d.batch * r.cout * 4);
      r.rstd = take((size_t)d.batch * r.cout * 4);
      route(i);
      r.wp_f = take(wpack_bytes(r.fwd, r.taps, C[o.src[0]], r.cin, r.cout));
      if (r.need_dgrad) r.wp_d = take(wpack_bytes(r.dgrad, r.taps, r.cout, r.cout, r.cin));
      slots_max = std::max(slots_max, conv_slots(r.fwd, dims[lv], r.taps, o.dil, cin, r.cout));
      if (r.wgrad == ConvKernel::Stream) wg_max = std::max(wg_max, wgrad_stream_workspace_bytes(C[o.src[0]], r.cout, o.dil, dims[lv]));
      wg_max = std::max(wg_max, wgrad_workspace_bytes(r.taps, r.cin, r.cout));
      if (o.xname) {
        r.mean2 = take((size_t)d.batch * r.cout * 4);
        r.rstd2 = take((size_t)d.batch * r.cout * 4);
        if (fuse_x) {
          xw_max = std::max(xw_max, (size_t)d.batch * epi_partials(dims[lv]) * r.cout * 2 * 8);
          r.xtot = take((size_t)d.batch * 5 * 8);
          xmom_max = std::max(xmom_max, (size_t)d.batch * xbranch_moment_slots(dims[lv]) * 5 * 8);
        } else {
          r.raw2 = take(act);
          r.wp_x = take(wpack_bytes(r.x_fwd, 1, 8, d.in_channel, r.cout));
          gx_max = std::max(gx_max, act);
          wg_max = std::max(wg_max, wgrad_workspace_bytes(1, d.in_channel, r.cout));
        }
      }
      slots_max = std::max(slots_max, std::max(std::max(conv_stats_tiles(dims[lv], 27, 1), conv_stats_tiles(dims[lv], 27, 2)), epi_partials(dims[lv])));
      cmax = std::max(cmax, r.cout);
      if (d.n_classes > 1 && o.kind == OP_GATED) r.side = take((size_t)d.batch * dims[lv].vox() * 2 * 4);
    }
    stat_slots_max = slots_max;
    for (int h = 0; h < 2; ++h)
      for (int l = 0; l < 4; ++l) {
        lvl[h][l] = take((size_t)d.n_classes * d.batch * dims[l].vox() * 4);
        glvl[h][l] = take((size_t)d.n_classes * d.batch * dims[l].vox() * 4);
      }
    if (d.n_classes > 1) {
      gside = take((size_t)d.batch * dims[0].vox() * 2 * 4);
      cls_part = take((size_t)d.batch * 256 * 2 * d.n_classes * 8);
      cls_bias = take((size_t)d.batch * d.n_classes * 4);
    }
    const size_t stat_bytes = (size_t)d.batch * slots_max * cmax * 2 * 8;
    stats = take(stat_bytes);
    stats2 = take(stat_bytes);
    pgrad = take((size_t)d.batch * slots_max * (4 * cmax + 4) * 4);
    m1 = take((size_t)d.batch * cmax * 4);
    m2 = take((size_t)d.batch * cmax * 4);
    m1b = take((size_t)d.batch * cmax * 4);
    m2b = take((size_t)d.batch * cmax * 4);
    wgrad_ws_bytes = wg_max;
    wgrad_ws = take(wg_max);
    head_tmp = take(head_bwd_tmp_floats(dims[0]) * 4);
    gx = take(gx_max);
    gx_bytes = gx_max;
    xwp = take(xw_max);
    xmom = take(xmom_max);
    total = cur;
    plan_input_grad();
    return 0;
  }
};

struct Exec {
  Plan p;
  unsigned char* ws = nullptr;
  const float* const* params = nullptr;
  hipStream_t s = nullptr;
  float* grad_x = nullptr;
  unsigned char* igs = nullptr;

  BlockParams opp[kNumOps];
  int head_w[2], head_b[2];
  const float* drops[2] = {nullptr, nullptr};

  float* gxl(int l) const { return reinterpret_cast<float*>(igs + p.ig_gx[l]); }
  void mark(const char* tag, const char* name = "") const { if (prof_on()) prof_mark((std::string(tag) + name).c_str(), s); }
  void* at(size_t off) const { return ws + off; }
  float* fat(size_t off) const { return reinterpret_cast<float*>(ws + off); }
  double* dat(size_t off) const { return reinterpret_cast<double*>(ws + off); }
  const float* par(int i) const { return i < 0 ? nullptr : params[i]; }

  int setup(const seunet_net_desc* desc, const float* const* prm, void* workspace, size_t bytes, hipStream_t st) {
    SEUNET_CHECK(desc && prm && workspace, "net: null argument");
    if (int e = p.init(*desc)) return e;
    SEUNET_CHECK(bytes >= p.total, "net: workspace too small (%zu < %zu bytes)", bytes, p.total);
    SEUNET_CHECK((reinterpret_cast<uintptr_t>(workspace) & 255) == 0, "net: workspace must be 256-byte aligned");
    BlockParams blocks[kNumBlocks];
    const std::vector<ParamInfo> reg = build_registry(p.d, blocks, head_w, head_b);
    for (int i = 0; i < kNumOps; ++i) {
      const OpDesc& o = kOps[i];
      if (o.kind != OP_GATED && o.kind != OP_CAT) continue;
      const int b = find_block(o.name), bx = o.xname ? find_block(o.xname) : -1;
      SEUNET_CHECK(b >= 0 && (!o.xname || bx >= 0), "net: internal: no parameters for %s", o.name);
      opp[i] = blocks[b];
      if (bx >= 0) opp[i].xw = blocks[bx].conv1_w;
    }
    ws = reinterpret_cast<unsigned char*>(workspace);
    params = prm;
    s = st;
    for (size_t i = 0; i < reg.size(); ++i)
      SEUNET_CHECK(prm[i] != nullptr || reg[i].name.rfind("dc62", 0) == 0, "net: parameter %s is null", reg[i].name.c_str());
    return 0;
// ... 30 lines not shown
    }
    mark("stats");
    return launch_stats_finalize(dat(p.stats), conv_slots(k, dm, taps, dil, src.total(), cout), cout, dm.N, dm.vox(), p.d.eps, 0,
                                 fat(mean_off), fat(rstd_off), s);
  }

  GateBlock gate_block(int i) const {
    const OpRes& r = p.op[i];
    const BlockParams& bp = opp[i];
    return GateBlock{{at(r.raw), fat(r.mean), fat(r.rstd)}, r.cout,
                     {par(bp.se), par(bp.se2), par(bp.conv2_w), par(bp.conv2_b), p.d.negative_slope}};
  }
  CatBlock cat_block(int i) const {
    const OpDesc& o = kOps[i];
    const OpRes& r = p.op[i];
    Branch2 x{};
    if (o.xname && p.fuse_x) x = {Branch2::Recomputed, at(p.feat[o.xsrc]), fat(r.mean2), fat(r.rstd2), par(opp[i].xw), p.d.in_channel};
    else if (o.xname) x = {Branch2::Stored, at(r.raw2), fat(r.mean2), fat(r.rstd2), nullptr, 0};
    return CatBlock{{at(r.raw), fat(r.mean), fat(r.rstd)}, x, r.cout, p.d.negative_slope};
  }
  SrcList xbranch_src(const OpDesc& o) const { return SrcList{{at(p.feat[o.xsrc])}, {8}, 1}; }
  bool skip_enc_head = false;

  struct HeadSlice { const float* w; const float* drop; int stride; float* gw; };
  HeadSlice head_slice(const OpDesc& o, float* const* grads = nullptr) const {
    const float* dr = drops[o.head];
    float* g = grads ? grads[head_w[o.head]] : nullptr;
    return HeadSlice{params[head_w[o.head]] + 2 * o.m, dr ? dr + 2 * o.m : nullptr, o.head == 0 ? 24 : 12, g ? g + 2 * o.m : nullptr};
  }

  SseHead sse_head(const OpDesc& o, bool first_of_level) const {
    if (o.head == 0 && skip_enc_head) return SseHead{};
    const int acc = first_of_level ? 0 : 1;
    if (p.d.n_classes > 1) return SseHead{fat(p.op[&o - kOps].side), nullptr, acc, nullptr, nullptr, 0};
    const HeadSlice hs = head_slice(o);
    return SseHead{nullptr, fat(p.lvl[o.head][kT[o.dst].level]), acc, hs.w, hs.drop, hs.stride};
  }

  int pack_all_weights(bool dgrad) {
    if (p.d.conv_impl == SEUNET_CONV_NAIVE) return 0;
    mark("pack_w");
    std::vector<ConvPackJob> jobs;
    std::vector<MarchPackJob> mjobs;
    std::vector<StreamPackJob> sjobs;
    const int tf = dgrad ? 1 : 0;
    auto add = [&](ConvKernel k, const float* w, size_t wp, int taps, int cin, int cout, int src_c, int dst_c) {
      if (k == ConvKernel::Stream) sjobs.push_back({w, at(wp), cin, cout, tf, src_c, dst_c});
      else if (k == ConvKernel::March) mjobs.push_back({w, at(wp), cin, cout, tf, src_c, dst_c});
      else jobs.push_back({w, at(wp), taps, cin, cout, tf});
    };
    for (int i = 0; i < kNumOps; ++i) {
      const OpDesc& o = kOps[i];
      if (o.kind != OP_GATED && o.kind != OP_CAT) continue;
      const OpRes& r = p.op[i];
      int ctot = 0;
      for (int k = 0; k < o.nsrc; ++k) ctot += p.C[o.src[k]];
      if (!dgrad) {
        add(r.fwd, par(opp[i].conv1_w), r.wp_f, r.taps, r.cin, r.cout, ctot, r.cout);
        if (o.xname && !p.fuse_x) add(r.x_fwd, par(opp[i].xw), r.wp_x, 1, p.d.in_channel, r.cout, 8, r.cout);
      } else if (r.need_dgrad) {
        add(r.dgrad, par(opp[i].conv1_w), r.wp_d, r.taps, r.cin, r.cout, r.cout, ctot);
      }
    }
    if (!sjobs.empty())
      if (int e = launch_conv_stream_pack_multi(p.d.dtype, sjobs.data(), (int)sjobs.size(), s)) return e;
    if (!mjobs.empty())
      if (int e = launch_conv_march_pack_multi(p.d.dtype, mjobs.data(), (int)mjobs.size(), s)) return e;
    return launch_conv_pack_weights_multi(p.d.dtype, jobs.data(), (int)jobs.size(), s);
  }

  int forward(const float* x, const float* drop1, const float* drop2, float* pred0, float* pred1) {
    skip_enc_head = pred0 == nullptr;
    drops[0] = drop1; drops[1] = drop2;
    if (int e = pack_all_weights(false)) return e;
    mark("pack_input");
    if (int e = launch_pack_input(p.d.dtype, x, p.d.in_channel, at(p.feat[T_X0]), p.dims[0], s)) return e;
    bool lvl_written[2][4] = {{false, false, false, false}, {false, false, false, false}};
    bool pool_done[kNumOps] = {};
    for (int i = 0; i < kNumOps; ++i) {
      const OpDesc& o = kOps[i];
      const OpRes& r = p.op[i];
      const BlockParams& bp = opp[i];
      const int lv = kT[o.dst].level;
      const Dims& dm = p.dims[lv];
      if (o.kind == OP_POOL) {
        if (pool_done[i]) continue;
        mark("pool_fwd:", o.name);
        if (int e = launch_maxpool_fwd(p.d.dtype, at(p.feat[o.src[0]]), p.C[o.src[0]], at(p.feat[o.dst]), p.dims[kT[o.src[0]].level], s)) return e;
      } else if (o.kind == OP_UP) {
        mark("up_fwd:", o.name);
        if (int e = launch_upsample2_fwd(p.d.dtype, at(p.feat[o.src[0]]), p.C[o.src[0]], at(p.feat[o.dst]), p.dims[kT[o.src[0]].level], s)) return e;
      } else if (o.kind == OP_GATED) {
        if (int e = conv_and_stats(o.name, r.fwd, 27, o.dil, srcs(o), r.cin, par(bp.conv1_w), par(bp.conv1_b), r.wp_f, r.raw,
                                   r.cout, r.mean, r.rstd, dm)) return e;
        const SseHead hd = sse_head(o, !lvl_written[o.head][lv]);
        lvl_written[o.head][lv] = true;
        mark("epi_fwd:", o.name);
        if (int e = launch_sse_fwd(p.d.dtype, gate_block(i), at(p.feat[o.dst]), hd, dm, s)) return e;
        if (p.d.n_classes > 1 && hd.side_out != nullptr) {
          const HeadSlice hs = head_slice(o);
          if (int e = launch_side_to_level(fat(r.side), hs.w, hs.stride, hs.drop, hs.stride, p.d.n_classes, fat(p.lvl[o.head][lv]),
                                           hd.level_accumulate, dm, s)) return e;
        }
      } else {
        const CatBlock blk = cat_block(i);
        if (int e = conv_and_stats(o.name, r.fwd, 1, 1, srcs(o), r.cin, par(bp.conv1_w), nullptr, r.wp_f, r.raw, r.cout, r.mean,
                                   r.rstd, dm)) return e;
        PoolOut pool_out{};
        if (blk.b.kind == Branch2::Recomputed) {
          mark("stats");
          if (int e = launch_xbranch_moments(p.d.dtype, blk.b.src, dat(p.xmom), dm, s)) return e;
          if (int e = launch_xbranch_stats(dat(p.xmom), xbranch_moment_slots(dm), blk.b.w2, r.cout, p.d.in_channel, dm.N, dm.vox(),
                                           p.d.eps, fat(r.mean2), fat(r.rstd2), dat(r.xtot), s)) return e;
          const OpDesc& pool = kOps[i + 1];
          SEUNET_CHECK(pool.kind == OP_POOL && pool.src[0] == o.dst && p.op[i + 1].has_pool_idx,
                       "net: internal: %s is not followed by its max-pool", o.name);
          pool_out = PoolOut{at(p.feat[pool.dst]), reinterpret_cast<unsigned*>(at(p.op[i + 1].pool_idx))};
          pool_done[i + 1] = true;
        } else if (blk.b.kind == Branch2::Stored) {
          if (int e = conv_and_stats(o.xname, r.x_fwd, 1, 1, xbranch_src(o), p.d.in_channel, par(bp.xw), nullptr, r.wp_x, r.raw2,
                                     r.cout, r.mean2, r.rstd2, dm)) return e;
        }
        mark("cat_fwd:", o.name);
        if (int e = launch_cat_fwd(p.d.dtype, blk, at(p.feat[o.dst]), pool_out, dm, s)) return e;
      }
    }
    const float* enc[4] = {fat(p.lvl[0][0]), fat(p.lvl[0][1]), fat(p.lvl[0][2]), fat(p.lvl[0][3])};
    const float* dec[3] = {fat(p.lvl[1][0]), fat(p.lvl[1][1]), fat(p.lvl[1][2])};
    mark("head_fwd");
    if (p.d.n_classes > 1) {
      const int K = p.d.n_classes, N = p.d.batch;
      const Dims d1{1, p.dims[0].D, p.dims[0].H, p.dims[0].W};
      for (int hd = 0; hd < 2; ++hd) {
        float* pred = hd == 0 ? pred0 : pred1;
        if (pred == nullptr) continue;
        const int nl = hd == 0 ? 4 : 3;
        for (int n = 0; n < N; ++n)
          for (int c = 0; c < K; ++c) {
            const float* lm[4] = {nullptr, nullptr, nullptr, nullptr};
            for (int l = 0; l < nl; ++l) lm[l] = fat(p.lvl[hd][l]) + ((size_t)c * N + n) * p.dims[l].vox();
            if (int e = launch_head_fwd(lm, nl, par(head_b[hd]) + c, pred + ((size_t)n * K + c) * d1.vox(), d1, s)) return e;
          }
      }
      mark("outside");
      return 0;
    }
    if (!skip_enc_head)
      if (int e = launch_head_fwd(enc, 4, par(head_b[0]), pred0, p.dims[0], s)) return e;
    if (int e = launch_head_fwd(dec, 3, par(head_b[1]), pred1, p.dims[0], s)) return e;
    mark("outside");
    return 0;
  }

  int conv_backward(int i, const SrcList& x, float* const* grads, bool* written) {
    const OpDesc& o = kOps[i];
    const OpRes& r = p.op[i];
    const int lv = kT[o.dst].level;
    const int wi = opp[i].conv1_w;
    if (grads[wi]) {
      mark("wgrad:", o.name);
      if (int e = run_wgrad(r.wgrad, p.d.dtype, r.taps, o.dil, x, r.cin, at(p.grad[o.dst]), r.cout, grads[wi], at(p.wgrad_ws),
                            p.wgrad_ws_bytes, p.dims[lv], s)) return e;
    }
    if (!r.need_dgrad) return 0;
    SrcList gsrc{};
    gsrc.n = 1; gsrc.ptr[0] = at(p.grad[o.dst]); gsrc.C[0] = r.cout;
    DstList gd{};
    gd.n = o.nsrc;
    for (int k = 0; k < o.nsrc; ++k) {
      const int t = o.src[k];
      gd.C[k] = p.C[t];
      gd.ptr[k] = is_input(t) ? nullptr : at(p.grad[t]);
      gd.acc[k] = (!is_input(t) && written[t]) ? 1 : 0;
      if (!is_input(t)) written[t] = true;
    }
    mark("dgrad:", o.name);
    return run_conv(r.dgrad, r.taps, o.dil, gsrc, r.cout, params[wi], 1, at(r.wp_d), nullptr, gd, nullptr, p.dims[lv]);
  }

  hipEvent_t decoder_done = nullptr;

  int backward(const float* g_pred0, const float* g_pred1, const float* drop1, const float* drop2, float* const* grads) {
    drops[0] = drop1; drops[1] = drop2;
    if (int e = pack_all_weights(true)) return e;
    bool written[T_COUNT];
    for (int t = 0; t < T_COUNT; ++t) written[t] = false;
    {
      mark("head_bwd");
      float* ge[4] = {nullptr, fat(p.glvl[0][1]), fat(p.glvl[0][2]), fat(p.glvl[0][3])};
      float* gd[4] = {nullptr, fat(p.glvl[1][1]), fat(p.glvl[1][2]), nullptr};
      if (p.d.n_classes > 1) {
        const int K = p.d.n_classes, N = p.d.batch;
        const Dims d1{1, p.dims[0].D, p.dims[0].H, p.dims[0].W};
        for (int hd = 0; hd < 2; ++hd) {
          const float* gp = hd == 0 ? g_pred0 : g_pred1;
          const int nl = hd == 0 ? 4 : 3;
          for (int n = 0; n < N; ++n)
            for (int c = 0; c < K; ++c) {
              float* gl[4] = {nullptr, nullptr, nullptr, nullptr};
              for (int l = 1; l < nl; ++l) gl[l] = fat(p.glvl[hd][l]) + ((size_t)c * N + n) * p.dims[l].vox();
              if (int e = launch_head_bwd(gp + ((size_t)n * K + c) * d1.vox(), gl, nl, fat(p.head_tmp), fat(p.cls_bias) + n * K + c, d1, s)) return e;
            }
          if (float* gb = grads[head_b[hd]])
            if (int e = launch_class_bias_grad(fat(p.cls_bias), N, K, gb, s)) return e;
        }
      } else {
      if (int e = launch_head_bwd(g_pred0, ge, 4, fat(p.head_tmp), grads[head_b[0]], p.dims[0], s)) return e;
      if (int e = launch_head_bwd(g_pred1, gd, 3, fat(p.head_tmp), grads[head_b[1]], p.dims[0], s)) return e;
      }
    }
    std::vector<float*> zero_ptrs;
    std::vector<int> zero_counts;
    PoolGrad pool_grad[T_COUNT] = {};
    for (int i = kNumOps - 1; i >= 0; --i) {
      const OpDesc& o = kOps[i];
      const OpRes& r = p.op[i];
      const BlockParams& bp = opp[i];
      if (decoder_done && strcmp(o.name, "up0") == 0) {
        SEUNET_HIP(hipEventRecord(decoder_done, s));
      }
      if (o.kind == OP_POOL || o.kind == OP_UP) {
        const int t = o.src[0];
        if (grad_x && o.dst == T_X2) {
          mark("input_grad:unpool1");
          if (int e = launch_xgrad_unpool(p.d.dtype, at(p.feat[T_X1]), p.d.in_channel, gxl(2), gxl(1), p.dims[1], s)) return e;
        }
        if (is_input(t)) continue;
        SEUNET_CHECK(written[o.dst], "net: internal: gradient of %s output missing", o.name);
        mark(o.kind == OP_POOL ? "pool_bwd:" : "up_bwd:", o.name);
        if (o.kind == OP_POOL) {
          if (r.has_pool_idx) {
            SEUNET_CHECK(written[t], "net: internal: gradient of %s input missing before its deferred pool gradient", o.name);
            pool_grad[t] = PoolGrad{reinterpret_cast<const unsigned*>(at(r.pool_idx)), at(p.grad[o.dst])};
            continue;
          }
          if (int e = launch_maxpool_bwd(p.d.dtype, at(p.feat[t]), at(p.grad[o.dst]), p.C[t], at(p.grad[t]), written[t] ? 1 : 0,
                                         p.dims[kT[t].level], s)) return e;
        } else {
          if (int e = launch_upsample2_bwd(p.d.dtype, at(p.grad[o.dst]), p.C[t], at(p.grad[t]), written[t] ? 1 : 0,
                                           p.dims[kT[t].level], s)) return e;
        }
        written[t] = true;
        continue;
      }
      const int lv = kT[o.dst].level;
      const Dims& dm = p.dims[lv];
      const int P_slots = epi_partials(dm);
      if (o.kind == OP_GATED) {
        const GateBlock blk = gate_block(i);
        SseBwdIn g{written[o.dst] ? at(p.grad[o.dst]) : nullptr, nullptr,
                   lv == 0 ? (o.head == 0 ? g_pred0 : g_pred1) : fat(p.glvl[o.head][lv])};
        SseHead hd = sse_head(o, false);
        const HeadSlice hs = head_slice(o, grads);
        float* g_head = hs.gw;
        if (p.d.n_classes > 1) {
          const int K = p.d.n_classes;
          const long long V = dm.vox();
          const long long cstride = lv == 0 ? V : (long long)dm.N * V, nstride = lv == 0 ? (long long)K * V : V;
          mark("epi_bwd:", o.name);
          if (int e = launch_level_to_side_grad(g.g_level, cstride, nstride, fat(r.side), hs.w, hs.stride, hs.drop, hs.stride, K,
                                                fat(p.gside), dat(p.cls_part), hs.gw, dm, s)) return e;
          g.g_level = nullptr;
          g.g_side = fat(p.gside);
          hd.side_out = nullptr;
          g_head = nullptr;
        }
        mark("epi_bwd:", o.name);
        if (int e = launch_sse_bwd_sums(p.d.dtype, blk, g, hd, SseSums{dat(p.stats), fat(p.pgrad)}, dm, s)) return e;
        mark("stats");
        if (int e = launch_gate_bwd_finalize(dat(p.stats), P_slots, r.cout, dm.N, dm.vox(), fat(p.m1), fat(p.m2), fat(p.pgrad),
                                             dm.N * P_slots, grads[bp.se], bp.se2 >= 0 ? grads[bp.se2] : nullptr, grads[bp.conv2_w],
                                             grads[bp.conv2_b], g_head, s)) return e;
        mark("in_bwd:", o.name);
        if (int e = launch_sse_bwd_apply(p.d.dtype, blk, g, hd, SseApply{fat(p.m1), fat(p.m2), at(p.grad[o.dst])}, dm, s)) return e;
        written[o.dst] = true;
        if (float* gb = grads[bp.conv1_b]) { zero_ptrs.push_back(gb); zero_counts.push_back(r.cout); }
        if (int e = conv_backward(i, srcs(o), grads, written)) return e;
      } else {
        SEUNET_CHECK(written[o.dst], "net: internal: gradient of %s output missing", o.name);
        const CatBlock blk = cat_block(i);
        const bool two = blk.b.kind != Branch2::None, recomputed = blk.b.kind == Branch2::Recomputed;
        float* gxw = two ? grads[bp.xw] : nullptr;
        const void* g_out = at(p.grad[o.dst]);
        const PoolGrad pool = pool_grad[o.dst];
        mark("cat_bwd:", o.name);
        const CatSums sums{dat(p.stats), dat(p.stats2), recomputed && gxw ? dat(p.xwp) : nullptr};
        if (int e = launch_cat_bwd_sums(p.d.dtype, blk, g_out, pool, sums, dm, s)) return e;
        mark("stats");
        if (recomputed && gxw)
          if (int e = launch_cat_xgrad_finalize(dat(p.xwp), dat(p.stats2), P_slots, dat(r.xtot), blk.b.w2, r.cout, p.d.in_channel, dm.N,
                                                p.d.eps, gxw, s)) return e;
        if (int e = launch_stats_finalize(dat(p.stats), P_slots, r.cout, dm.N, dm.vox(), 0.f, 1, fat(p.m1), fat(p.m2), s)) return e;
        if (two)
          if (int e = launch_stats_finalize(dat(p.stats2), P_slots, r.cout, dm.N, dm.vox(), 0.f, 1, fat(p.m1b), fat(p.m2b), s)) return e;
        mark("in_bwd:", o.name);
        CatApply ap{fat(p.m1), fat(p.m2), fat(p.m1b), fat(p.m2b), at(p.grad[o.dst]), two && !recomputed ? at(p.gx) : nullptr, nullptr, 0};
        if (recomputed && grad_x) { ap.gx_out = gxl(lv); ap.gx_acc = lv == 1 ? 1 : 0; }
        if (int e = launch_cat_bwd_apply(p.d.dtype, blk, g_out, pool, ap, dm, s)) return e;
        if (two && !recomputed) {
          if (grad_x) {
            mark("input_grad:", o.xname);
            if (int e = launch_xgrad_contract(p.d.dtype, at(p.gx), r.cout, par(bp.xw), p.d.in_channel, gxl(lv), lv == 1 ? 1 : 0, dm, s)) return e;
          }
          if (gxw) {
            mark("wgrad:", o.xname);
            if (int e = run_wgrad(r.x_wgrad, p.d.dtype, 1, 1, xbranch_src(o), p.d.in_channel, at(p.gx), r.cout, gxw, at(p.wgrad_ws),
                                  p.wgrad_ws_bytes, dm, s)) return e;
          }
        }
        if (int e = conv_backward(i, srcs(o), grads, written)) return e;
      }
    }
    if (!zero_ptrs.empty()) {
      mark("stats");
      if (int e = launch_multi_zero(zero_ptrs.data(), zero_counts.data(), (int)zero_ptrs.size(), s)) return e;
    }
    if (grad_x) {
      mark("input_grad:ec1");
      if (int e = launch_input_grad(p.d.dtype, at(p.grad[T_E0]), p.C[T_E0], par(opp[0].conv1_w), at(p.feat[T_X0]), p.d.in_channel,
                                    gxl(0), gxl(1), grad_x, p.dims[0], s)) return e;
    }
    mark("outside");
    return 0;
  }
};

}
}

using namespace seunet;

extern "C" {

int seunet_net_param_count(const seunet_net_desc* desc) {
  if (!desc) return -1;
  return (int)build_registry(*desc).size();
}

int seunet_net_param_info(const seunet_net_desc* desc, int index, char* name, int name_cap, int* shape5, int* ndim) {
  SEUNET_CHECK(desc && name && shape5 && ndim, "param_info: null argument");
  const std::vector<ParamInfo> reg = build_registry(*desc);
  SEUNET_CHECK(index >= 0 && index < (int)reg.size(), "param_info: index %d out of range", index);
  snprintf(name, (size_t)name_cap, "%s", reg[index].name.c_str());
  for (int k = 0; k < 5; ++k) shape5[k] = reg[index].shape[k];
  *ndim = reg[index].ndim;
  return 0;
}

size_t seunet_net_workspace_bytes(const seunet_net_desc* desc) {
  if (!desc) return 0;
  Plan p;
  if (p.init(*desc)) return 0;
  return p.total;
}

int seunet_net_forward(const seunet_net_desc* desc, const float* const* params, const float* x, const float* drop1,
                       const float* drop2, float* pred0, float* pred1, void* workspace, size_t workspace_bytes,
                       seunet_stream_t s) {
  SEUNET_CHECK(x && pred1, "net_forward: null tensor");
  Exec ex;
  if (int e = ex.setup(desc, params, workspace, workspace_bytes, (hipStream_t)s)) return e;
  return ex.forward(x, drop1, drop2, pred0, pred1);
}

struct NetGraph {
  hipGraph_t graph = nullptr;
  hipGraphExec_t exec = nullptr;
};

int seunet_net_forward_capture(const seunet_net_desc* desc, const float* const* params, const float* x, const float* drop1,
                               const float* drop2, float* pred0, float* pred1, void* workspace, size_t workspace_bytes,
                               seunet_stream_t s, void** graph_out) {
  SEUNET_CHECK(x && pred1 && graph_out, "net_forward_capture: null argument");
  SEUNET_CHECK(s != nullptr, "net_forward_capture: stream capture needs a stream other than the null stream");
  SEUNET_CHECK(!prof_on(), "net_forward_capture: switch the launch-group timer off before capturing");
  *graph_out = nullptr;
  Exec ex;
  if (int e = ex.setup(desc, params, workspace, workspace_bytes, (hipStream_t)s)) return e;
  SEUNET_CHECK(device_zero_page() != nullptr, "net_forward_capture: zero page allocation failed");
  SEUNET_HIP(hipStreamBeginCapture((hipStream_t)s, hipStreamCaptureModeThreadLocal));
  const int rc = ex.forward(x, drop1, drop2, pred0, pred1);
  NetGraph* g = new NetGraph;
  const hipError_t e_end = hipStreamEndCapture((hipStream_t)s, &g->graph);
  if (rc != 0 || e_end != hipSuccess) {
    if (g->graph) (void)hipGraphDestroy(g->graph);
    delete g;
    if (rc != 0) return rc;
    return fail("net_forward_capture: hipStreamEndCapture failed: %s", hipGetErrorString(e_end));
  }
  const hipError_t e_inst = hipGraphInstantiate(&g->exec, g->graph, nullptr, nullptr, 0);
  if (e_inst != hipSuccess) {
    (void)hipGraphDestroy(g->graph);
    delete g;
    return fail("net_forward_capture: hipGraphInstantiate failed: %s", hipGetErrorString(e_inst));
  }
  *graph_out = g;
  return 0;
}

int seunet_graph_launch(void* graph, seunet_stream_t s) {
  SEUNET_CHECK(graph != nullptr, "graph_launch: null graph");
  SEUNET_HIP(hipGraphLaunch(static_cast<NetGraph*>(graph)->exec, (hipStream_t)s));
  return 0;
}

int seunet_graph_destroy(void* graph) {
  if (!graph) return 0;
  NetGraph* g = static_cast<NetGraph*>(graph);
  if (g->exec) (void)hipGraphExecDestroy(g->exec);
  if (g->graph) (void)hipGraphDestroy(g->graph);
  delete g;
  return 0;
}

int seunet_net_read_tensor(const seunet_net_desc* desc, const float* const* params, const void* workspace, size_t workspace_bytes,
                           const char* name, int which, float* out, int* channels, seunet_stream_t s) {
  SEUNET_CHECK(desc && workspace && name && out, "net_read_tensor: null argument");
  Plan p;
  if (int e = p.init(*desc)) return e;
  SEUNET_CHECK(workspace_bytes >= p.total, "net_read_tensor: workspace too small");
  const unsigned char* ws = reinterpret_cast<const unsigned char*>(workspace);
  for (int i = 0; i < kNumOps; ++i) {
    const OpDesc& o = kOps[i];
    if (o.kind != OP_GATED && o.kind != OP_CAT) continue;
    const OpRes& r = p.op[i];
    const int lv = kT[o.dst].level;
    if (o.xname && std::string(o.xname) == name) {
      SEUNET_CHECK(which >= 0 && which <= 2, "net_read_tensor: which=%d is not stored for an x-branch", which);
      if (channels) *channels = r.cout;
      if (which == 0 && p.fuse_x) {
        SEUNET_CHECK(params != nullptr, "net_read_tensor: the recomputed x-branch %s needs the parameter list", name);
        BlockParams blocks[kNumBlocks];
        build_registry(p.d, blocks);
        const int wi = blocks[find_block(o.xname)].conv1_w;
        SEUNET_CHECK(params[wi], "net_read_tensor: no weight for %s", name);
        return launch_xbranch_values(p.d.dtype, ws + p.feat[o.xsrc], params[wi], r.cout, p.d.in_channel, out, p.dims[lv], (hipStream_t)s);
      }
      if (which == 0) return launch_unpack_cl(p.d.dtype, ws + r.raw2, r.cout, out, p.dims[lv], (hipStream_t)s);
      SEUNET_HIP(hipMemcpyAsync(out, ws + (which == 1 ? r.mean2 : r.rstd2), (size_t)p.d.batch * r.cout * 4, hipMemcpyDeviceToDevice, (hipStream_t)s));
      return 0;
    }
    if (std::string(o.name) != name) continue;
    if (channels) *channels = which == 3 ? p.C[o.dst] : r.cout;
    if (which == 0) return launch_unpack_cl(p.d.dtype, ws + r.raw, r.cout, out, p.dims[lv], (hipStream_t)s);
    if (which == 3) return launch_unpack_cl(p.d.dtype, ws + p.feat[o.dst], p.C[o.dst], out, p.dims[lv], (hipStream_t)s);
    SEUNET_CHECK(which == 1 || which == 2, "net_read_tensor: which=%d", which);
    SEUNET_HIP(hipMemcpyAsync(out, ws + (which == 1 ? r.mean : r.rstd), (size_t)p.d.batch * r.cout * 4, hipMemcpyDeviceToDevice, (hipStream_t)s));
    return 0;
  }
  return fail("net_read_tensor: no block named %s", name);
}

static_assert((int)ConvKernel::Naive == SEUNET_KERNEL_NAIVE && (int)ConvKernel::Tiled == SEUNET_KERNEL_TILED &&
                  (int)ConvKernel::Stream == SEUNET_KERNEL_STREAM && (int)ConvKernel::March == SEUNET_KERNEL_MARCH &&
                  (int)ConvKernel::Wgrad1x1 == SEUNET_KERNEL_WGRAD1X1,
              "SEUNET_KERNEL_* are the values of ConvKernel");

int seunet_net_conv_info(const seunet_net_desc* desc, int index, seunet_conv_info* out) {
  SEUNET_CHECK(desc && out, "net_conv_info: null argument");
  Plan p;
  if (int e = p.init(*desc)) return e;
  SEUNET_CHECK(index >= 0, "net_conv_info: index %d out of range", index);
  int seen = 0;
  for (int i = 0; i < kNumOps; ++i) {
    const OpDesc& o = kOps[i];
    if (o.kind != OP_GATED && o.kind != OP_CAT) continue;
    if (seen++ != index) continue;
    const OpRes& r = p.op[i];
    const int lv = kT[o.dst].level;
    *out = seunet_conv_info{};
    snprintf(out->name, sizeof out->name, "%s", o.name);
    out->taps = r.taps;
    out->dilation = o.kind == OP_GATED ? o.dil : 1;
    out->level = lv;
    out->dims = seunet_dims{p.dims[lv].N, p.dims[lv].D, p.dims[lv].H, p.dims[lv].W};
    out->nsrc = o.nsrc;
    for (int k = 0; k < o.nsrc; ++k) { out->src_c[k] = p.C[o.src[k]]; out->src_is_input[k] = is_input(o.src[k]) ? 1 : 0; }
    out->cin = r.cin;
    out->cout = r.cout;
    out->need_dgrad = r.need_dgrad ? 1 : 0;
    out->fwd = (int)r.fwd;
    out->dgrad = (int)r.dgrad;
    out->wgrad = (int)r.wgrad;
    if (o.xname) {
      snprintf(out->x_name, sizeof out->x_name, "%s", o.xname);
      out->x_materialised = p.fuse_x ? 0 : 1;
      out->x_fwd = (int)r.x_fwd;
      out->x_wgrad = (int)r.x_wgrad;
    }
    out->src_dist = o.nsrc == 2 ? (long long)p.feat[o.src[1]] - (long long)p.feat[o.src[0]] : 0;
    return 0;
  }
  return fail("net_conv_info: index %d is past the last convolution (%d)", index, seen);
}

int seunet_net_backward(const seunet_net_desc* desc, const float* const* params, const float* g_pred0,
                        const float* g_pred1, const float* drop1, const float* drop2, float* const* grads,
                        void* workspace, size_t workspace_bytes, seunet_stream_t s) {
  return seunet_net_backward_ev(desc, params, g_pred0, g_pred1, drop1, drop2, grads, workspace, workspace_bytes, s, nullptr);
}

int seunet_net_backward_ev(const seunet_net_desc* desc, const float* const* params, const float* g_pred0,
                           const float* g_pred1, const float* drop1, const float* drop2, float* const* grads,
                           void* workspace, size_t workspace_bytes, seunet_stream_t s, void* decoder_done_event) {
  SEUNET_CHECK(g_pred0 && g_pred1 && grads, "net_backward: null tensor");
  Exec ex;
  if (int e = ex.setup(desc, params, workspace, workspace_bytes, (hipStream_t)s)) return e;
  ex.decoder_done = reinterpret_cast<hipEvent_t>(decoder_done_event);
  return ex.backward(g_pred0, g_pred1, drop1, drop2, grads);
}

size_t seunet_net_input_grad_bytes(const seunet_net_desc* desc) {
  if (!desc) { (void)fail("net_input_grad_bytes: null descriptor"); return 0; }
  Plan p;
  if (p.init(*desc)) return 0;
  return p.ig_total;
}

int seunet_net_backward_input(const seunet_net_desc* desc, const float* const* params, const float* g_pred0, const float* g_pred1,
                              const float* drop1, const float* drop2, float* const* grads, float* grad_x, void* scratch,
                              size_t scratch_bytes, void* workspace, size_t workspace_bytes, seunet_stream_t s,
                              void* decoder_done_event) {
  if (grad_x == nullptr)
    return seunet_net_backward_ev(desc, params, g_pred0, g_pred1, drop1, drop2, grads, workspace, workspace_bytes, s, decoder_done_event);
  SEUNET_CHECK(g_pred0 && g_pred1 && grads && scratch, "net_backward_input: null tensor");
  Exec ex;
  if (int e = ex.setup(desc, params, workspace, workspace_bytes, (hipStream_t)s)) return e;
  SEUNET_CHECK(scratch_bytes >= ex.p.ig_total, "net_backward_input: scratch too small (%zu < %zu bytes)", scratch_bytes, ex.p.ig_total);
  SEUNET_CHECK((reinterpret_cast<uintptr_t>(scratch) & 255) == 0, "net_backward_input: scratch must be 256-byte aligned");
  ex.decoder_done = reinterpret_cast<hipEvent_t>(decoder_done_event);
  ex.grad_x = grad_x;
  ex.igs = reinterpret_cast<unsigned char*>(scratch);
  return ex.backward(g_pred0, g_pred1, drop1, drop2, grads);
}

}
```

### se-unet-airseg_amd/csrc/seunet_common.h

```cpp
#pragma once
#include <hip/hip_runtime.h>
#include <stdint.h>
#include <string>

#define SEUNET_F32 0
#define SEUNET_BF16 1
#define SEUNET_F16 2

typedef __bf16 bf16_t;
typedef _Float16 f16_t;

namespace seunet {

void set_error(const std::string& msg);
const char* get_error();
int fail(const char* fmt, ...);
bool prof_on();
void prof_mark(const char* tag, hipStream_t s);

#define SEUNET_CHECK(cond, ...)                       \
  do {                                                \
    if (!(cond)) return ::seunet::fail(__VA_ARGS__);  \
  } while (0)

// ... 97 lines not shown
  v[0] = bf16_bits_to_f32(u.x & 0xffffu); v[1] = bf16_bits_to_f32(u.x >> 16);
  v[2] = bf16_bits_to_f32(u.y & 0xffffu); v[3] = bf16_bits_to_f32(u.y >> 16);
  v[4] = bf16_bits_to_f32(u.z & 0xffffu); v[5] = bf16_bits_to_f32(u.z >> 16);
  v[6] = bf16_bits_to_f32(u.w & 0xffffu); v[7] = bf16_bits_to_f32(u.w >> 16);
}
__device__ __forceinline__ void load8(const f16_t* p, float (&v)[8]) {
  const uint4 u = *reinterpret_cast<const uint4*>(p);
  v[0] = unpack_lo<f16_t>(u.x); v[1] = unpack_hi<f16_t>(u.x); v[2] = unpack_lo<f16_t>(u.y); v[3] = unpack_hi<f16_t>(u.y);
  v[4] = unpack_lo<f16_t>(u.z); v[5] = unpack_hi<f16_t>(u.z); v[6] = unpack_lo<f16_t>(u.w); v[7] = unpack_hi<f16_t>(u.w);
}
__device__ __forceinline__ void store8(f16_t* p, const float (&v)[8]) {
  uint4 u;
  u.x = pack2<f16_t>(v[0], v[1]); u.y = pack2<f16_t>(v[2], v[3]); u.z = pack2<f16_t>(v[4], v[5]); u.w = pack2<f16_t>(v[6], v[7]);
  *reinterpret_cast<uint4*>(p) = u;
}
__device__ __forceinline__ void store8(float* p, const float (&v)[8]) {
  reinterpret_cast<float4*>(p)[0] = make_float4(v[0], v[1], v[2], v[3]);
  reinterpret_cast<float4*>(p)[1] = make_float4(v[4], v[5], v[6], v[7]);
}
__device__ __forceinline__ void store8(bf16_t* p, const float (&v)[8]) {
  uint4 u;
  u.x = pack2<bf16_t>(v[0], v[1]); u.y = pack2<bf16_t>(v[2], v[3]); u.z = pack2<bf16_t>(v[4], v[5]); u.w = pack2<bf16_t>(v[6], v[7]);
  *reinterpret_cast<uint4*>(p) = u;
}

template <typename T> struct Pack8;
template <> struct Pack8<bf16_t> { uint4 u; };
template <> struct Pack8<float> { float4 a, b; };
template <> struct Pack8<f16_t> { uint4 u; };
__device__ __forceinline__ void load8p(const f16_t* p, Pack8<f16_t>& k) { k.u = *reinterpret_cast<const uint4*>(p); }
__device__ __forceinline__ void unpack8(const Pack8<f16_t>& k, float (&v)[8]) {
  v[0] = unpack_lo<f16_t>(k.u.x); v[1] = unpack_hi<f16_t>(k.u.x); v[2] = unpack_lo<f16_t>(k.u.y); v[3] = unpack_hi<f16_t>(k.u.y);
  v[4] = unpack_lo<f16_t>(k.u.z); v[5] = unpack_hi<f16_t>(k.u.z); v[6] = unpack_lo<f16_t>(k.u.w); v[7] = unpack_hi<f16_t>(k.u.w);
}
__device__ __forceinline__ void zero8p(Pack8<f16_t>& k) { k.u = make_uint4(0, 0, 0, 0); }
__device__ __forceinline__ void load8p(const bf16_t* p, Pack8<bf16_t>& k) { k.u = *reinterpret_cast<const uint4*>(p); }
__device__ __forceinline__ void load8p(const float* p, Pack8<float>& k) {
  k.a = reinterpret_cast<const float4*>(p)[0];
  k.b = reinterpret_cast<const float4*>(p)[1];
}
__device__ __forceinline__ void unpack8(const Pack8<bf16_t>& k, float (&v)[8]) {
  v[0] = bf16_bits_to_f32(k.u.x & 0xffffu); v[1] = bf16_bits_to_f32(k.u.x >> 16);
  v[2] = bf16_bits_to_f32(k.u.y & 0xffffu); v[3] = bf16_bits_to_f32(k.u.y >> 16);
  v[4] = bf16_bits_to_f32(k.u.z & 0xffffu); v[5] = bf16_bits_to_f32(k.u.z >> 16);
  v[6] = bf16_bits_to_f32(k.u.w & 0xffffu); v[7] = bf16_bits_to_f32(k.u.w >> 16);
}
__device__ __forceinline__ void unpack8(const Pack8<float>& k, float (&v)[8]) {
  v[0] = k.a.x; v[1] = k.a.y; v[2] = k.a.z; v[3] = k.a.w; v[4] = k.b.x; v[5] = k.b.y; v[6] = k.b.z; v[7] = k.b.w;
}
__device__ __forceinline__ void zero8p(Pack8<bf16_t>& k) { k.u = make_uint4(0, 0, 0, 0); }
__device__ __forceinline__ void zero8p(Pack8<float>& k) { k.a = k.b = make_float4(0.f, 0.f, 0.f, 0.f); }

__device__ __forceinline__ int xcd_contiguous_tile(int b, int nt) {
  const int q = nt >> 3, r = nt & 7, xcd = b & 7;
  return (xcd < r ? xcd * (q + 1) : r * (q + 1) + (xcd - r) * q) + (b >> 3);
}
struct TileIdx3 { int x, y, z; };
__device__ __forceinline__ TileIdx3 xcd_contiguous_tile3() {
  const int b = (int)(blockIdx.x + gridDim.x * (blockIdx.y + gridDim.y * blockIdx.z));
  const int t = xcd_contiguous_tile(b, (int)(gridDim.x * gridDim.y * gridDim.z));
  TileIdx3 r;
  r.x = t % (int)gridDim.x;
  r.y = (t / (int)gridDim.x) % (int)gridDim.y;
  r.z = t / (int)(gridDim.x * gridDim.y);
  return r;
}
__device__ __forceinline__ float dpp_settle(float v) {
  asm volatile("v_mov_b32 %0, %0" : "+v"(v));
  return v;
}
__device__ __forceinline__ int dpp_settle(int v) {
  asm volatile("v_mov_b32 %0, %0" : "+v"(v));
  return v;
}
__device__ __forceinline__ unsigned long long dpp_settle(unsigned long long u) {
  unsigned lo = (unsigned)u, hi = (unsigned)(u >> 32);
  asm volatile("v_mov_b32 %0, %0\n\tv_mov_b32 %1, %1" : "+v"(lo), "+v"(hi));
  return ((unsigned long long)hi << 32) | lo;
}
__device__ __forceinline__ double dpp_settle(double v) {
  return __builtin_bit_cast(double, dpp_settle(__builtin_bit_cast(unsigned long long, v)));
}
template <typename V> __device__ __forceinline__ V shfl_xor_settled(V v, int off) { return dpp_settle(__shfl_xor(v, off, 64)); }
template <int CTRL> __device__ __forceinline__ int dpp_fetch_bits(int v) {
  return __builtin_amdgcn_update_dpp(0, v, CTRL, 0xF, 0xF, true);
}
template <int CTRL> __device__ __forceinline__ float dpp_fetch(float v) {
  return __builtin_bit_cast(float, dpp_fetch_bits<CTRL>(__builtin_bit_cast(int, v)));
}
template <int LPV> __device__ __forceinline__ float group_sum(float v) {
  static_assert(LPV == 1 || LPV == 2 || LPV == 4 || LPV == 8 || LPV == 16, "group_sum: LPV must be 1..16");
  if (LPV >= 2) v += dpp_fetch<0xB1>(v);
  if (LPV >= 4) v += dpp_fetch<0x4E>(v);
  if (LPV >= 8) v += dpp_fetch<0x141>(v);
  if (LPV >= 16) v += dpp_fetch<0x140>(v);
  return LPV >= 2 ? dpp_settle(v) : v;
}
template <int LPV> __device__ __forceinline__ float stride_sum(float v) {
#pragma unroll
  for (int off = 32; off >= LPV; off >>= 1) v += shfl_xor_settled(v, off);
  return v;
}
template <int LPV> __device__ __forceinline__ double stride_sum_d(double v) {
#pragma unroll
  for (int off = 32; off >= LPV; off >>= 1) v += shfl_xor_settled(v, off);
  return v;
}
#endif

int launch_pack_input(int dtype, const float* x_ncdhw, int in_channel, void* out_cl8, Dims d, hipStream_t s);
int launch_unpack_cl(int dtype, const void* in_cl, int C, float* out_ncdhw, Dims d, hipStream_t s);
int launch_pack_cl(int dtype, const float* in_ncdhw, int C, void* out_cl, int Cpad, Dims d, hipStream_t s);

size_t conv_wpack_bytes(int dtype, int taps, int cin, int cout);
int launch_conv_pack_weights(int dtype, const float* w_torch, int taps, int cin_w, int cout_w,
                             int transpose_flip, void* wpack, hipStream_t s);
int conv_stats_tiles(Dims d, int taps, int dil);
struct ConvPackJob { const float* w; void* wpack; int taps, cin_w, cout_w, tflip; };
int launch_conv_pack_weights_multi(int dtype, const ConvPackJob* jobs, int n, hipStream_t s);
int launch_conv_igemm(int dtype, int taps, int dil, const SrcList& src, int cin_logical,
                      const void* wpack, const float* bias, const DstList& dst,
                      double* stats_partial, Dims d, hipStream_t s);
int launch_conv_naive(int dtype, int taps, int dil, const SrcList& src, int cin_logical,
                      const float* w_torch, int transpose_flip, const float* bias,
                      const DstList& dst, Dims d, hipStream_t s);

bool conv_stream_supported(int dtype, int taps, int dil, int src_c, int dst_c);
size_t conv_stream_wpack_bytes(int src_c);
int conv_stream_slots(Dims d, int dil);
int launch_conv_stream_pack(int dtype, const float* w, int cin_w, int cout_w, int tflip, int src_c, int dst_c, void* wpack, hipStream_t s);
struct StreamPackJob { const float* w; void* wpack; int cin_w, cout_w, tflip, src_c, dst_c; };
int launch_conv_stream_pack_multi(int dtype, const StreamPackJob* jobs, int n, hipStream_t s);
int launch_conv_stream(int dtype, int dil, const void* src, int src_c, const void* wpack, const float* bias, void* dst, int dst_c,
                       int dst_accumulate, double* stats, Dims d, hipStream_t s);

bool conv_march_supported(int dtype, int taps, int dil, const SrcList& src, const DstList& dst);
size_t conv_march_wpack_bytes(int cin_e, int cout_e);
int conv_march_slots(Dims d, int dil, int cin_e, int cout_e);
int launch_conv_march_pack(int dtype, const float* w, int cin_w, int cout_w, int tflip, int cin_e, int cout_e, void* wpack, hipStream_t s);
struct MarchPackJob { const float* w; void* wpack; int cin_w, cout_w, tflip, cin_e, cout_e; };
int launch_conv_march_pack_multi(int dtype, const MarchPackJob* jobs, int n, hipStream_t s);
int launch_conv_march(int dtype, int dil, const SrcList& src, const void* wpack, const float* bias, const DstList& dst, double* stats,
                      Dims d, hipStream_t s);

bool wgrad_stream_supported(int dtype, int taps, int dil, int x_c, int dy_c);
size_t wgrad_stream_workspace_bytes(int x_c, int dy_c, int dil, Dims d);
int launch_wgrad_stream(int dtype, int dil, const void* x, int x_c, int cin_w, const void* dy, int dy_c, int cout_w, float* dw,
                        void* workspace, size_t ws_bytes, Dims d, hipStream_t s);

static constexpr int WG_TILED_SLABS = 512;
size_t wgrad_workspace_bytes(int taps, int cin, int cout);
int launch_wgrad(int dtype, int taps, int dil, const SrcList& x, int cin_logical, const void* dy,
                 int cout, float* dw_torch, void* workspace, size_t ws_bytes, Dims d, hipStream_t s);
bool wgrad_march_supported(int dtype, int taps, int dil, const SrcList& x, int cin_logical, int cout, Dims d, long long src_dist);
int launch_wgrad_march(int dtype, int taps, int dil, const SrcList& x, int cin_logical, const void* dy, int cout,
                       float* dw, void* workspace, size_t ws_bytes, Dims d, hipStream_t s);
size_t wgrad_march_workspace_bytes(int taps, int cin, int cout);
bool wgrad_1x1_supported(int dtype, const SrcList& x, int cin_logical, int cout);
int launch_wgrad_1x1(int dtype, const SrcList& x, int cin_logical, const void* dy, int cout, float* dw, void* workspace,
                     size_t ws_bytes, Dims d, hipStream_t s);
size_t wgrad_1x1_workspace_bytes(int cin, int cout);
int launch_wgrad_naive(int dtype, int taps, int dil, const SrcList& x, int cin_logical,
                       const void* dy, int cout, float* dw_torch, Dims d, hipStream_t s);
enum class ConvKernel { Naive, Tiled, Stream, March, Wgrad1x1 };
ConvKernel wgrad_kernel(int dtype, int taps, int dil, const SrcList& x, int cin_logical, int cout, Dims d, long long src_dist);
int run_wgrad(ConvKernel k, int dtype, int taps, int dil, const SrcList& x, int cin_logical, const void* dy, int cout, float* dw,
              void* workspace, size_t ws_bytes, Dims d, hipStream_t s);


int launch_xgrad_contract(int dtype, const void* d2, int C, const float* w2, int in_channel, float* gx, int accumulate, Dims d,
                          hipStream_t s);
int launch_xgrad_unpool(int dtype, const void* x_fine, int in_channel, const float* gx_coarse, float* gx_fine, Dims fine, hipStream_t s);
int launch_input_grad(int dtype, const void* draw, int ce, const float* w_ec1, const void* x0, int in_channel, const float* gx0,
                      const float* gx1, float* grad_x, Dims d, hipStream_t s);
int launch_maxpool_fwd(int dtype, const void* in, int C, void* out, Dims din, hipStream_t s);
int launch_maxpool_bwd(int dtype, const void* in, const void* g_out, int C, void* g_in,
                       int accumulate, Dims din, hipStream_t s);
int launch_upsample2_fwd(int dtype, const void* in, int C, void* out, Dims din, hipStream_t s);
int launch_upsample2_bwd(int dtype, const void* g_out, int C, void* g_in, int accumulate,
                         Dims din, hipStream_t s);
int upsample2_form(int dtype, int C, Dims din, bool backward);
int launch_multi_zero(float* const* ptrs, const int* counts, int n, hipStream_t s);
int class_max();
int class_grad_records(Dims d);
int launch_side_to_level(const float* side, const float* head_w, int wstride, const float* drop, int drop_stride, int K, float* level,
                         int accumulate, Dims d, hipStream_t s);
int launch_level_to_side_grad(const float* glev, long long cstride, long long nstride, const float* side, const float* head_w, int wstride,
                              const float* drop, int drop_stride, int K, float* g_side, double* partial, float* dhead, Dims d,
                              hipStream_t s);
int launch_class_bias_grad(const float* per_sample, int N, int K, float* out, hipStream_t s);
int launch_crop_batch(const void* img, int img_dtype, const unsigned char* label, const void* weight, int w_dtype,
                      const unsigned char* skel, int D, int H, int W, int cube, int ncrop, const int* starts, const int* aug,
                      double weight_exponent, int f64_math, float* data_out, float* label_out, float* weight_out, float* skel_out,
                      hipStream_t s);
int launch_hu_two_channel(const void* img, int img_dtype, long long nvox, int f64_math, float* out, hipStream_t s);
int launch_window_gather(const float* vol, int C, int X, int Y, int Z, int cube, int nwin, const int* starts, float* out, hipStream_t s);
int launch_window_accumulate(const float* logits, int apply_sigmoid, int nwin, const int* starts, int cube, double* acc, int X, int Y,
                             int Z, hipStream_t s);
int launch_window_finalize(const double* acc, int X, int Y, int Z, int cube, int nx, const int* xs, int ny, const int* ys, int nz,
                           const int* zs, int dup0, double* out, hipStream_t s);
int launch_adamw(float* const* params, const float* const* grads, float* const* exp_avg, float* const* exp_avg_sq,
                 const long long* counts, int n, double lr, double beta1, double beta2, double eps, double weight_decay,
                 int step, int maximize, hipStream_t s);
int configure_kernel_lds(unsigned long long& mask, const void* fn, int bytes);
const void* device_zero_page();
int launch_side_upsample(const float* side, int C, int scale, float* out_ncdhw, int c_total,
                         int c_off, Dims dlow, hipStream_t s);
int launch_head_fwd(const float* const* level_maps, int nlevels, const float* bias, float* pred,
                    Dims d0, hipStream_t s);
int launch_head_bwd(const float* g_pred, float* const* g_levels, int nlevels, float* tmp,
                    float* g_bias, Dims d0, hipStream_t s);
size_t head_bwd_tmp_floats(Dims d0);

#define SEUNET_LOSS_NSUMS 7
int loss_partials();
int launch_loss_sums(const float* pred, int apply_sigmoid, const float* target,
                     const float* weight, const float* skel, long long n, float* partial,
                     double* sums, hipStream_t s, int terms = 7);
int launch_loss_value(const double* sums0, double c_dice0, double c_gul0, double c_atr0, const double* sums1, double c_dice1,
                      double c_gul1, double c_atr1, float* value, hipStream_t s);
int launch_loss_grad(const float* pred, int apply_sigmoid, const float* target,
                     const float* weight, const float* skel, long long n, const double* sums,
                     float c_dice, float c_gul, float c_atr, float g_scale,
                     const float* g_scale_dev, float* g_pred, hipStream_t s);
int loss_sample_partials(int batch);
int launch_loss_sums_per_sample(const float* pred, int apply_sigmoid, const float* target, const float* weight, const float* skel,
                                int batch, long long n, float* partial, double* sums, int terms, hipStream_t s);
int launch_loss_sample_values(const double* sums, int batch, double c_dice, double c_gul, double c_atr, float* values, hipStream_t s);
#define SEUNET_POOL_MAX_CAPACITY 65535
#define SEUNET_POOL_MAX_BATCH 1024
#define SEUNET_POOL_MAX_GATHER 32
int launch_pool_select(const float* new_keys, int batch, float* keys, long long* seq, long long* state, int capacity, int* slots_out,
                       hipStream_t s);
int launch_pool_scatter(const int* slots_dev, int batch, int capacity, long long voxels, const float* data, const float* label,
                        const float* weight, const float* skel, float* pool_data, unsigned char* pool_label, float* pool_weight,
                        unsigned char* pool_skel, hipStream_t s);
int launch_pool_gather(const int* slots_host, int n, int capacity, long long voxels, const float* pool_data,
                       const unsigned char* pool_label, const float* pool_weight, const unsigned char* pool_skel, float* data_out,
                       float* label_out, float* weight_out, float* skel_out, hipStream_t s);
}
```

### se-unet-airseg_amd/csrc/wgrad.hip

```cpp
#include "seunet_common.h"
#include "mfma.h"
#include <climits>
#include <cstdlib>

namespace seunet {

extern unsigned long long* g_conv_debug;

struct WgArgs {
  const void* src0; const void* src1; const void* src2;
  int srcC0, srcC1, srcC2;
  int cum1, cum2;
  int cin;
  const void* dy; int cout;
  float* slab;
  const void* zero;
  int N, D, H, W;
  int tx, ty, tz;
  int co_tiles;
  unsigned long long* debug;
};

template <typename T> struct WgTile;
template <> struct WgTile<bf16_t> { static constexpr int TZ = 2, TY = 4; };
template <> struct WgTile<f16_t> { static constexpr int TZ = 2, TY = 4; };
template <> struct WgTile<float> { static constexpr int TZ = 1, TY = 4; };

__device__ __forceinline__ const void* wg_uniform_ptr(const void* p) {
  const unsigned long long u = reinterpret_cast<unsigned long long>(p);
  const unsigned lo = __builtin_amdgcn_readfirstlane((unsigned)u), hi = __builtin_amdgcn_readfirstlane((unsigned)(u >> 32));
  return reinterpret_cast<const void*>(((unsigned long long)hi << 32) | lo);
}

#ifdef SEUNET_STAMP
#define WSTAMP(i) do { const unsigned long long _t = __builtin_readcyclecounter(); ph[i] += _t - t_last; t_last = _t; } while (0)
#else
#define WSTAMP(i) do {} while (0)
#endif

template <typename T, int TAPS, int DIL, int NW>
__global__ void __launch_bounds__(NW * 64, NW == 4 ? 2 : 4)
wgrad_kernel(WgArgs a) {
#ifdef SEUNET_STAMP
  unsigned long long ph[6] = {0, 0, 0, 0, 0, 0};
  unsigned long long t_last = __builtin_readcyclecounter();
#endif
  constexpr int HALO = (TAPS == 27) ? 1 : 0;
  constexpr int STEP = (TAPS == 27) ? DIL : 1;
  constexpr int TZ = WgTile<T>::TZ, TY = WgTile<T>::TY, TX = 32;
  constexpr int HZ = TZ + 2 * HALO, HY = TY + 2 * HALO, HX = TX + 2 * HALO;
  constexpr int NVH = HZ * HY * HX, NVT = TZ * TY * TX;
  constexpr int EPP = 16 / sizeof(T);
  constexpr int PPV = 32 / EPP;
  constexpr int XG = (NVH + 63) / 64, YG = (NVT + 63) / 64;
  constexpr int X_ITEMS = (XG * PPV + NW - 1) / NW, Y_ITEMS = (YG * PPV + NW - 1) / NW;
  constexpr int XPL = (XG * 64 + 4) * 16, YPL = (YG * 64 + 4) * 16;
  constexpr int NT = (TAPS == 27) ? (27 + NW - 1) / NW : 1;
  extern __shared__ __attribute__((aligned(16))) unsigned char smem[];
  unsigned char* xs = smem;
  unsigned char* ys = smem + PPV * XPL;
  typedef __attribute__((address_space(3))) void lds_void;
  typedef const __attribute__((address_space(1))) void glb_void;

  const int tid = threadIdx.x, lane = tid & 63, wave = tid >> 6;
  const int col = lane & 31, h = lane >> 5;
  const int combo = blockIdx.y;
  const int ci0 = (combo / a.co_tiles) * 32, co0 = (combo % a.co_tiles) * 32;
  const long long V = (long long)a.D * a.H * a.W;
  const int tiles_per_par = a.tx * a.ty * a.tz;
  const int tiles_per_sample = tiles_per_par * STEP * STEP * STEP;
  const int total_tiles = tiles_per_sample * a.N;

  int tapoff[NT];
#pragma unroll
  for (int ti = 0; ti < NT; ++ti) {
    int tap = wave + NW * ti;
    if (tap > TAPS - 1) tap = TAPS - 1;
    if (TAPS == 27) tapoff[ti] = (((tap / 9) * HALO) * HY + ((tap / 3) % 3) * HALO) * HX + (tap % 3) * HALO;
    else tapoff[ti] = 0;
  }
  f32x16 acc[NT];
#pragma unroll
  for (int ti = 0; ti < NT; ++ti)
#pragma unroll
    for (int r = 0; r < 16; ++r) acc[ti][r] = 0.f;
  const unsigned char* abase[NT];
  const unsigned char* bbase;
  {
    const int grp = lane >> 4, li = lane & 15;
    const int pl = (li & 3) >> 1;
    const int vo = 8 * grp + (li >> 2);
    const int sub = (li & 1) * 8;
    const int wrow = (TAPS == 27) ? 0 : wave;
#pragma unroll
    for (int ti = 0; ti < NT; ++ti)
      abase[ti] = xs + (PPV == 4 ? pl : 0) * XPL + ((wrow / TY * HY + wrow % TY) * HX + tapoff[ti] + vo) * 16 + sub;
    bbase = ys + (PPV == 4 ? pl : 0) * YPL + (wrow * TX + vo) * 16 + sub;
  }

  static_assert(PPV % NW == 0, "pieces per voxel must be a multiple of the wave count");
  constexpr int PV = PPV / NW;
  const int wave_s = __builtin_amdgcn_readfirstlane(wave);
  static_assert(XG <= 16 && HZ <= 4 && HY <= 8 && HX <= 64, "packed halo coordinates");
  u32x4* cslot = reinterpret_cast<u32x4*>(smem + PPV * (XPL + YPL) + tid * 32);
  {
    unsigned w[8] = {0, 0, 0, 0, 0, 0, 0, 0};
#pragma unroll
    for (int g = 0; g < XG; ++g) {
      const int vox = g * 64 + lane;
      const int hx = vox % HX, r2 = vox / HX;
      const int hy = r2 % HY, hz = r2 / HY;
      const unsigned c = vox < NVH ? ((unsigned)hz | ((unsigned)hy << 2) | ((unsigned)hx << 5)) : 0x8000u;
      w[g >> 1] |= c << (16 * (g & 1));
    }
    u32x4 lo, hi;
    lo.x = w[0]; lo.y = w[1]; lo.z = w[2]; lo.w = w[3]; hi.x = w[4]; hi.y = w[5]; hi.z = w[6]; hi.w = w[7];
    cslot[0] = lo; cslot[1] = hi;
  }
  const unsigned char* xbase[PV]; long long xstride[PV]; bool xvalid[PV];
  const unsigned char* ybase[PV]; bool yvalid[PV];
#pragma unroll
  for (int j = 0; j < PV; ++j) {
    const int piece = wave_s + NW * j;
    const int ch0 = ci0 + piece * EPP;
    const void* sp = a.src0; int sC = a.srcC0, c = ch0;
    if (ch0 >= a.cum2) { sp = a.src2; sC = a.srcC2; c = ch0 - a.cum2; }
    else if (ch0 >= a.cum1) { sp = a.src1; sC = a.srcC1; c = ch0 - a.cum1; }
    xvalid[j] = ch0 < a.cin;
    xbase[j] = reinterpret_cast<const unsigned char*>(reinterpret_cast<const T*>(sp) + c);
    xstride[j] = (long long)sC * (long long)sizeof(T);
    const int cy0 = co0 + piece * EPP;
    yvalid[j] = cy0 < a.cout;
    ybase[j] = reinterpret_cast<const unsigned char*>(reinterpret_cast<const T*>(a.dy) + cy0);
  }
  const long long ystride = (long long)a.cout * (long long)sizeof(T);
  const unsigned char* zero_page = reinterpret_cast<const unsigned char*>(a.zero);

  auto stage = [&](int tile) __attribute__((always_inline)) {
    const int n = tile / tiles_per_sample;
    int t = tile % tiles_per_sample;
    const int par = t / tiles_per_par; t %= tiles_per_par;
    const int bx = t % a.tx; t /= a.tx;
    const int by = t % a.ty;
    const int bz = t / a.ty;
    const int px = par % STEP, py = (par / STEP) % STEP, pz = par / (STEP * STEP);
    const int x0 = bx * TX, y0 = by * TY, z0 = bz * TZ;
    const int zlo = z0 >= HALO ? 0 : HALO - z0, ylo = y0 >= HALO ? 0 : HALO - y0, xlo = x0 >= HALO ? 0 : HALO - x0;
    const int zmax = (a.D - 1 - pz + STEP) / STEP - 1, ymax = (a.H - 1 - py + STEP) / STEP - 1, xmax = (a.W - 1 - px + STEP) / STEP - 1;
    int zsp = zmax - (z0 - HALO) - zlo, ysp = ymax - (y0 - HALO) - ylo, xsp = xmax - (x0 - HALO) - xlo;
    const bool any = zsp >= 0 && ysp >= 0 && xsp >= 0;
    if (!any) zsp = ysp = xsp = 0;
    const long long origin = ((long long)(STEP * (z0 - HALO) + pz) * a.H + (STEP * (y0 - HALO) + py)) * a.W + (STEP * (x0 - HALO) + px);
    const long long nofs = (long long)n * V;
    const u32x4 clo = cslot[0], chi = cslot[1];
    const unsigned cw[8] = {clo.x, clo.y, clo.z, clo.w, chi.x, chi.y, chi.z, chi.w};
#pragma unroll
    for (int k = 0; k < X_ITEMS; ++k) {
      const int j = k % PV, g = k / PV;
      if (g < XG) {
        const unsigned c = cw[g >> 1] >> (16 * (g & 1));
        const unsigned cz = c & 3u, cy = (c >> 2) & 7u, cx = (c >> 5) & 63u;
        const bool ok = (int)(any & xvalid[j]) & (int)((c & 0x8000u) == 0) & (int)((cz - (unsigned)zlo) <= (unsigned)zsp) &
                        (int)((cy - (unsigned)ylo) <= (unsigned)ysp) & (int)((cx - (unsigned)xlo) <= (unsigned)xsp);
        const unsigned rel = (unsigned)STEP * ((cz * (unsigned)a.H + cy) * (unsigned)a.W + cx);
        const unsigned char* sb = xbase[j] + (nofs + origin) * xstride[j];
        const unsigned char* gp = sb + (unsigned long long)rel * (unsigned long long)(unsigned)xstride[j];
        gp = ok ? gp : zero_page;
        __builtin_amdgcn_global_load_lds((glb_void*)gp, (lds_void*)(xs + (wave_s + NW * j) * XPL + g * 1024), 16, 0, 0);
      }
    }
    const long long yorigin = ((long long)(STEP * z0 + pz) * a.H + (STEP * y0 + py)) * a.W + (STEP * x0 + px);
    const int yzsp = zmax - z0, yysp = ymax - y0, yxsp = xmax - x0;
    int lane_t = lane;
    asm volatile("" : "+v"(lane_t));
#pragma unroll
    for (int k = 0; k < Y_ITEMS; ++k) {
      const int j = k % PV, g = k / PV;
      if (g < YG) {
        const int vox = g * 64 + lane_t;
        const int lx = vox % TX, r2 = vox / TX;
        const int ly = r2 % TY, lz = r2 / TY;
        const bool ok = (int)yvalid[j] & (int)(vox < NVT) & (int)(lz <= yzsp) & (int)(ly <= yysp) & (int)(lx <= yxsp);
        const unsigned rel = (unsigned)STEP * (unsigned)((lz * a.H + ly) * a.W + lx);
        const unsigned char* sb = ybase[j] + (nofs + yorigin) * ystride;
        const unsigned char* gp = sb + (unsigned long long)rel * (unsigned long long)(unsigned)ystride;
        gp = ok ? gp : zero_page;
        __builtin_amdgcn_global_load_lds((glb_void*)gp, (lds_void*)(ys + (wave_s + NW * j) * YPL + g * 1024), 16, 0, 0);
      }
    }
  };

  WSTAMP(0);
  for (int tile = blockIdx.x; tile < total_tiles; tile += gridDim.x) {
    __syncthreads();
    WSTAMP(1);
    stage(tile);
    WSTAMP(2);
    __syncthreads();
    WSTAMP(3);
    if constexpr (sizeof(T) == 2) {
      constexpr int ROWS = (TAPS == 27) ? TZ * TY : TZ * TY / NW;
      constexpr int NSTEP = ROWS * NT;
      auto a_off = [](int ri) constexpr {
        const int row = (TAPS == 27) ? ri : ri * NW;
        return ((row / TY * HY + row % TY) * HX) * 16;
      };
      auto b_off = [](int ri) constexpr {
        const int row = (TAPS == 27) ? ri : ri * NW;
        return (row * TX) * 16;
      };
      bf16x4 abuf[3][2][2], bbuf[2][2][2];
      auto load_a = [&](auto step_c) __attribute__((always_inline)) {
        constexpr int st = decltype(step_c)::value;
        if constexpr (st < NSTEP) {
          constexpr int ti = st % NT, ri = st / NT;
#pragma unroll
          for (int blk = 0; blk < 2; ++blk) {
            abuf[st % 3][blk][0] = read_tr16((const lds_bf16x4*)(abase[ti] + a_off(ri) + blk * 2 * XPL));
            abuf[st % 3][blk][1] = read_tr16((const lds_bf16x4*)(abase[ti] + a_off(ri) + blk * 2 * XPL + 64));
          }
        }
      };
      auto load_b = [&](auto ri_c) __attribute__((always_inline)) {
        constexpr int ri = decltype(ri_c)::value;
        if constexpr (ri < ROWS) {
#pragma unroll
          for (int blk = 0; blk < 2; ++blk) {
            bbuf[ri % 2][blk][0] = read_tr16((const lds_bf16x4*)(bbase + b_off(ri) + blk * 2 * YPL));
            bbuf[ri % 2][blk][1] = read_tr16((const lds_bf16x4*)(bbase + b_off(ri) + blk * 2 * YPL + 64));
          }
        }
      };
      load_b(std::integral_constant<int, 0>{});
      load_a(std::integral_constant<int, 0>{});
      load_a(std::integral_constant<int, 1>{});
      static_for<NSTEP>([&](auto st_c) __attribute__((always_inline)) {
        constexpr int ST = decltype(st_c)::value, ti = ST % NT, ri = ST / NT;
        load_a(std::integral_constant<int, ST + 2>{});
        if constexpr (ti == 0) load_b(std::integral_constant<int, ri + 1>{});
        __builtin_amdgcn_sched_barrier(0);
#pragma unroll
        for (int ab = 0; ab < 2; ++ab) {
          const bf16x8 afr = frag_join(abuf[ST % 3][ab][0], abuf[ST % 3][ab][1]);
#pragma unroll
          for (int bb = 0; bb < 2; ++bb) {
            const bf16x8 bfr = frag_join(bbuf[ri % 2][bb][0], bbuf[ri % 2][bb][1]);
            const int q = 4 * (2 * ab + bb);
            f32x4 c = {acc[ti][q], acc[ti][q + 1], acc[ti][q + 2], acc[ti][q + 3]};
            c = mfma_16x16x32<T>(afr, bfr, c);
            acc[ti][q] = c[0]; acc[ti][q + 1] = c[1]; acc[ti][q + 2] = c[2]; acc[ti][q + 3] = c[3];
          }
        }
        __builtin_amdgcn_sched_barrier(0);
      });
    } else {
      for (int row = 0; row < TZ * TY; ++row) {
        if (TAPS == 1 && (row % NW) != wave) continue;
        const int lz = row / TY, ly = row % TY;
        const int xrow = (lz * HY + ly) * HX;
        const int yrow = row * TX;
        const int pl = col >> 2, sub = (col & 3) * 4;
#pragma unroll 4
        for (int kk = 0; kk < 16; ++kk) {
          const int xo = 2 * kk + h;
          const float bfr = *reinterpret_cast<const float*>(ys + pl * YPL + (yrow + xo) * 16 + sub);
#pragma unroll
          for (int ti = 0; ti < NT; ++ti) {
            const float afr = *reinterpret_cast<const float*>(xs + pl * XPL + (xrow + tapoff[ti] + xo) * 16 + sub);
            acc[ti] = __builtin_amdgcn_mfma_f32_32x32x2f32(afr, bfr, acc[ti], 0, 0, 0);
          }
        }
      }
    }
    WSTAMP(4);
  }
  if (TAPS == 27) {
    float* out = a.slab + ((size_t)combo * gridDim.x + blockIdx.x) * (27 * 1024);
#pragma unroll
    for (int ti = 0; ti < NT; ++ti) {
      const int tap = wave + NW * ti;
      if (tap < 27) {
#pragma unroll
        for (int r = 0; r < 16; ++r) {
          const int row = sizeof(T) == 4 ? (r & 3) + 8 * (r >> 2) + 4 * h : 16 * (r >> 3) + 4 * (lane >> 4) + (r & 3);
          const int cc = sizeof(T) == 4 ? col : 16 * ((r >> 2) & 1) + (lane & 15);
          out[(tap * 32 + row) * 32 + cc] = acc[ti][r];
        }
      }
    }
  } else {
    __syncthreads();
    float* part = reinterpret_cast<float*>(smem);
#pragma unroll
    for (int r = 0; r < 16; ++r) {
      const int row = sizeof(T) == 4 ? (r & 3) + 8 * (r >> 2) + 4 * h : 16 * (r >> 3) + 4 * (lane >> 4) + (r & 3);
      const int cc = sizeof(T) == 4 ? col : 16 * ((r >> 2) & 1) + (lane & 15);
      part[wave * 1024 + row * 32 + cc] = acc[0][r];
    }
    __syncthreads();
    float* out = a.slab + ((size_t)combo * gridDim.x + blockIdx.x) * 1024;
    for (int e = tid; e < 1024; e += NW * 64) {
      float t = part[e];
#pragma unroll
      for (int w = 1; w < NW; ++w) t += part[w * 1024 + e];
      out[e] = t;
    }
  }
#ifdef SEUNET_STAMP
  WSTAMP(5);
  if (a.debug != nullptr && lane == 0) {
    const size_t w = ((size_t)blockIdx.y * gridDim.x + blockIdx.x) * NW + wave;
    for (int i = 0; i < 6; ++i) a.debug[w * 12 + i] = ph[i];
    for (int i = 6; i < 12; ++i) a.debug[w * 12 + i] = 0;
  }
#endif
}

__global__ void __launch_bounds__(256)
wgrad_reduce_kernel(const float* __restrict__ slab, int nslab, int taps, int cin_w, int cout_w, int co_tiles,
                    float* __restrict__ dw) {
  const int per = taps * 1024;
  const int el = threadIdx.x & 15, part = threadIdx.x >> 4;
  const int e = blockIdx.x * 16 + el;
  const int combo = blockIdx.y;
  const float* p = slab + (size_t)combo * nslab * per + e;
  double s0 = 0.0, s1 = 0.0;
  int k = part;
  for (; k + 16 < nslab; k += 32) {
    s0 += (double)p[(size_t)k * per];
    s1 += (double)p[(size_t)(k + 16) * per];
  }
  if (k < nslab) s0 += (double)p[(size_t)k * per];
  __shared__ double red[16][17];
  red[part][el] = s0 + s1;
  __syncthreads();
  if (part == 0) {
    double t = red[0][el];
#pragma unroll
    for (int q = 1; q < 16; ++q) t += red[q][el];
    const int tap = e >> 10, ci = (combo / co_tiles) * 32 + ((e >> 5) & 31), co = (combo % co_tiles) * 32 + (e & 31);
    if (ci < cin_w && co < cout_w) dw[((size_t)co * cin_w + ci) * taps + tap] = (float)t;
  }
}

static inline int wgrad_groups(int combos, int total_tiles) {
  int g = WG_TILED_SLABS / combos;
  if (g < 16) g = 16;
  if (g > WG_TILED_SLABS) g = WG_TILED_SLABS;
  if (g > total_tiles) g = total_tiles;
  if (g < 1) g = 1;
  return g;
}
static size_t wgrad_tiled_bytes(int taps, int combos, int groups) {
  return 256 + (size_t)combos * groups * taps * 1024 * sizeof(float);
}

size_t wgrad_workspace_bytes(int taps, int cin, int cout) {
  const int combos = cdiv(cin, 32) * cdiv(cout, 32);
  const size_t tiled = wgrad_tiled_bytes(taps, combos, wgrad_groups(combos, INT_MAX));
  const size_t other = taps == 1 ? wgrad_1x1_workspace_bytes(cin, cout) : wgrad_march_workspace_bytes(taps, cin, cout);
  return tiled > other ? tiled : other;
}

template <typename T, int TAPS, int DIL, int NW>
static int wgrad_launch_one(const WgArgs& a, dim3 grid, hipStream_t s) {
  constexpr int HALO = (TAPS == 27) ? 1 : 0;
  constexpr int TZ = WgTile<T>::TZ, TY = WgTile<T>::TY;
  constexpr int PPV = 32 / (16 / (int)sizeof(T));
  constexpr int NVH = (TZ + 2 * HALO) * (TY + 2 * HALO) * (32 + 2 * HALO), NVT = TZ * TY * 32;
  constexpr int LDS = PPV * ((((NVH + 63) / 64) * 64 + 4) + (((NVT + 63) / 64) * 64 + 4)) * 16 + NW * 64 * 32;
  static unsigned long long configured = 0;
  if (int e = configure_kernel_lds(configured, reinterpret_cast<const void*>(&wgrad_kernel<T, TAPS, DIL, NW>), LDS)) return e;
  wgrad_kernel<T, TAPS, DIL, NW><<<grid, NW * 64, LDS, s>>>(a);
  SEUNET_LAUNCH_CHECK();
  return 0;
}

static void wg_sources(WgArgs& a, const SrcList& x, int cin_logical) {
  a.src0 = x.ptr[0]; a.srcC0 = x.C[0];
  a.src1 = x.n > 1 ? x.ptr[1] : nullptr; a.srcC1 = x.n > 1 ? x.C[1] : 0;
  a.src2 = x.n > 2 ? x.ptr[2] : nullptr; a.srcC2 = x.n > 2 ? x.C[2] : 0;
  a.cin = cin_logical;
  a.cum1 = x.n > 1 ? x.C[0] : x.total();
  a.cum2 = x.n > 2 ? x.C[0] + x.C[1] : x.total();
}

int launch_wgrad(int dtype, int taps, int dil, const SrcList& x, int cin_logical, const void* dy, int cout,
                 float* dw, void* workspace, size_t ws_bytes, Dims d, hipStream_t s) {
  SEUNET_CHECK(taps == 27 || taps == 1, "wgrad: taps=%d unsupported", taps);
  SEUNET_CHECK(taps == 1 || dil == 1 || dil == 2, "wgrad: dilation %d unsupported", dil);
  SEUNET_CHECK(x.n >= 1 && x.n <= 3, "wgrad: 1..3 sources");
  SEUNET_CHECK(cout % 8 == 0 && cin_logical >= 1 && cin_logical <= x.total(), "wgrad: bad channel counts");
  SEUNET_CHECK(ws_bytes >= wgrad_workspace_bytes(taps, cin_logical, cout), "wgrad: workspace too small");
  WgArgs a{};
  wg_sources(a, x, cin_logical);
  a.dy = dy; a.cout = cout;
  a.zero = device_zero_page();
  SEUNET_CHECK(a.zero != nullptr, "wgrad: cannot allocate the device zero page");
  a.slab = reinterpret_cast<float*>(reinterpret_cast<unsigned char*>(workspace) + 256);
  a.N = d.N; a.D = d.D; a.H = d.H; a.W = d.W;
  const int tz = dtype_size(dtype) == 2 ? WgTile<bf16_t>::TZ : WgTile<float>::TZ;
  const int ty = dtype_size(dtype) == 2 ? WgTile<bf16_t>::TY : WgTile<float>::TY;
  const int st = taps == 27 ? dil : 1;
  a.tx = cdiv(cdiv(d.W, st), 32); a.ty = cdiv(cdiv(d.H, st), ty); a.tz = cdiv(cdiv(d.D, st), tz);
  a.co_tiles = cdiv(cout, 32);
  a.debug = g_conv_debug;
  const int combos = cdiv(cin_logical, 32) * a.co_tiles;
  const int G = wgrad_groups(combos, a.tx * a.ty * a.tz * st * st * st * d.N);
  dim3 grid(G, combos);
  int e;
  SEUNET_DTYPE_SWITCH(dtype, {
    if (taps == 1) e = wgrad_launch_one<T, 1, 1, 4>(a, grid, s);
    else if (dil == 1) e = wgrad_launch_one<T, 27, 1, 4>(a, grid, s);
    else e = wgrad_launch_one<T, 27, 2, 4>(a, grid, s);
  });
  if (e) return e;
  wgrad_reduce_kernel<<<dim3(taps * 1024 / 16, combos), 256, 0, s>>>(a.slab, G, taps, cin_logical, cout,
                                                                            a.co_tiles, dw);
  SEUNET_LAUNCH_CHECK();
  return 0;
}

template <typename T>
__global__ void wgrad_naive_kernel(WgArgs a, int taps, int dil, float* __restrict__ dw, long long total) {
  const long long V = (long long)a.D * a.H * a.W;
  const int t3 = taps == 27 ? 3 : 1, c = taps == 27 ? 1 : 0;
  for (long long i = blockIdx.x * (long long)blockDim.x + threadIdx.x; i < total;
       i += (long long)gridDim.x * blockDim.x) {
    const int tap = (int)(i % taps);
    const int ci = (int)((i / taps) % a.cin);
    const int co = (int)(i / ((long long)taps * a.cin));
    const int dz = (tap / (t3 * t3) - c) * dil, dy = ((tap / t3) % t3 - c) * dil, dx = (tap % t3 - c) * dil;
    const void* sp = a.src0; int sC = a.srcC0, cc = ci;
    if (ci >= a.cum2) { sp = a.src2; sC = a.srcC2; cc = ci - a.cum2; }
    else if (ci >= a.cum1) { sp = a.src1; sC = a.srcC1; cc = ci - a.cum1; }
    double s = 0.0;
    for (int n = 0; n < a.N; ++n)
      for (int z = 0; z < a.D; ++z) {
        const int zz = z + dz;
        if ((unsigned)zz >= (unsigned)a.D) continue;
        for (int y = 0; y < a.H; ++y) {
          const int yy = y + dy;
          if ((unsigned)yy >= (unsigned)a.H) continue;
          for (int x = 0; x < a.W; ++x) {
            const int xx = x + dx;
            if ((unsigned)xx >= (unsigned)a.W) continue;
            const float xv = to_f32(reinterpret_cast<const T*>(sp)[(n * V + ((long long)zz * a.H + yy) * a.W + xx) * sC + cc]);
            const float gv = to_f32(reinterpret_cast<const T*>(a.dy)[(n * V + ((long long)z * a.H + y) * a.W + x) * a.cout + co]);
            s += (double)xv * (double)gv;
          }
        }
      }
    dw[i] = (float)s;
  }
}

int launch_wgrad_naive(int dtype, int taps, int dil, const SrcList& x, int cin_logical, const void* dy, int cout,
                       float* dw, Dims d, hipStream_t s) {
  WgArgs a{};
  wg_sources(a, x, cin_logical);
  a.dy = dy; a.cout = cout;
  a.N = d.N; a.D = d.D; a.H = d.H; a.W = d.W;
  const long long total = (long long)cout * cin_logical * taps;
  const int grid = (int)((total + 63) / 64);
  SEUNET_DTYPE_SWITCH(dtype, wgrad_naive_kernel<T><<<grid, 64, 0, s>>>(a, taps, dil, dw, total));
  SEUNET_LAUNCH_CHECK();
  return 0;
}

}
```

### se-unet-airseg_amd/ops.py

```python
from __future__ import annotations

import ctypes as C
from typing import List, Optional, Sequence, Tuple

import torch

from . import _lib
from ._lib import Dims


def _tdtype(code: int):
    return {_lib.BF16: torch.bfloat16, _lib.F16: torch.float16}.get(code, torch.float32)


def _code(t: torch.Tensor) -> int:
    return {torch.bfloat16: _lib.BF16, torch.float16: _lib.F16}.get(t.dtype, _lib.F32)


def _dims_cl(t: torch.Tensor) -> Dims:
    n, d, h, w, _ = t.shape
    return Dims(n, d, h, w)


def _s():
    return _lib.stream_ptr()


def to_cl(x: torch.Tensor, dtype="bf16", c_pad: Optional[int] = None) -> torch.Tensor:
    code = dtype if isinstance(dtype, int) else _lib.dtype_code(dtype)
    x = x.contiguous().float()
    n, c, d, h, w = x.shape
    c_pad = c_pad or (c + 7) // 8 * 8
    out = torch.empty((n, d, h, w, c_pad), dtype=_tdtype(code), device=x.device)
    _lib.check(_lib.load().seunet_pack_cl(code, x.data_ptr(), c, out.data_ptr(), c_pad, Dims(n, d, h, w), _s()), "pack_cl")
    return out


def from_cl(t: torch.Tensor, c: Optional[int] = None) -> torch.Tensor:
    n, d, h, w, cp = t.shape
    out = torch.empty((n, cp, d, h, w), dtype=torch.float32, device=t.device)
    _lib.check(_lib.load().seunet_unpack_cl(_code(t), t.data_ptr(), cp, out.data_ptr(), Dims(n, d, h, w), _s()), "unpack_cl")
    return out if c is None else out[:, :c].contiguous()


def pack_weights(w: torch.Tensor, code: int, transpose_flip: bool = False) -> torch.Tensor:
    lib = _lib.load()
    co, ci = w.shape[0], w.shape[1]
    taps = w.shape[2] * w.shape[3] * w.shape[4]
    ce_in, ce_out = (co, ci) if transpose_flip else (ci, co)
    nbytes = lib.seunet_conv_wpack_bytes(code, taps, ce_in, ce_out)
    buf = torch.empty(nbytes, dtype=torch.uint8, device=w.device)
    w = w.contiguous().float()
    _lib.check(lib.seunet_conv_pack_weights(code, w.data_ptr(), taps, ci, co, int(transpose_flip), buf.data_ptr(), _s()),
               "conv_pack_weights")
    return buf


def conv3d(srcs: Sequence[torch.Tensor], weight: torch.Tensor, bias: Optional[torch.Tensor] = None, dilation: int = 1,
           impl: int = _lib.CONV_MFMA, transpose_flip: bool = False, cin: Optional[int] = None,
           dsts: Optional[Sequence[Optional[torch.Tensor]]] = None, dst_channels: Optional[Sequence[int]] = None,
           accumulate: Optional[Sequence[int]] = None, want_stats: bool = False):
    lib = _lib.load()
    code = _code(srcs[0])
    dims = _dims_cl(srcs[0])
    taps = weight.shape[2] * weight.shape[3] * weight.shape[4]
    co_w, ci_w = weight.shape[0], weight.shape[1]
    cin_e, cout_e = (co_w, ci_w) if transpose_flip else (ci_w, co_w)
    cin = cin or cin_e
    if dsts is None:
        dst_channels = dst_channels or [(cout_e + 7) // 8 * 8]
        dsts = [torch.empty(tuple(srcs[0].shape[:4]) + (c,), dtype=srcs[0].dtype, device=srcs[0].device) for c in dst_channels]
        accumulate = [0] * len(dsts)
    else:
        dst_channels = dst_channels or [t.shape[4] for t in dsts]
        accumulate = list(accumulate or [0] * len(dsts))
    wbuf = weight.contiguous().float() if impl == _lib.CONV_NAIVE else pack_weights(weight, code, transpose_flip)
    stats, slots = None, 0
    if want_stats:
        slots = lib.seunet_conv_stats_slots(impl, taps, dilation, dims)
        stats = torch.zeros((dims.n, slots, sum(dst_channels), 2), dtype=torch.float64, device=srcs[0].device)
    b = None if bias is None else bias.contiguous().float()
    _lib.check(lib.seunet_conv3d_fwd(code, impl, taps, dilation, len(srcs), _lib.ptr_array(list(srcs)),
                                     _lib.int_array([t.shape[4] for t in srcs]), cin, wbuf.data_ptr(), int(transpose_flip),
                                     _lib.ptr(b), len(dsts), _lib.ptr_array(list(dsts)), _lib.int_array(list(dst_channels)),
                                     _lib.int_array(list(accumulate)), _lib.ptr(stats), dims, _s()), "conv3d_fwd")
    return list(dsts), stats, slots


def conv3d_stream(src: torch.Tensor, weight: torch.Tensor, bias: Optional[torch.Tensor] = None, dilation: int = 1,
                  transpose_flip: bool = False, dst: Optional[torch.Tensor] = None, dst_channels: Optional[int] = None,
                  accumulate: bool = False, want_stats: bool = False):
    lib = _lib.load()
    code, dims = _code(src), _dims_cl(src)
    co_w, ci_w = weight.shape[0], weight.shape[1]
    cout_e = ci_w if transpose_flip else co_w
    src_c = src.shape[4]
    dst_c = dst.shape[4] if dst is not None else (dst_channels or (cout_e + 7) // 8 * 8)
    if not lib.seunet_conv3d_stream_supported(code, dilation, src_c, dst_c):
        raise RuntimeError(f"conv3d_stream: {src_c} -> {dst_c} channels, dilation {dilation}, dtype {src.dtype} is not served by this kernel")
    wbuf = torch.empty(lib.seunet_conv3d_stream_wpack_bytes(src_c), dtype=torch.uint8, device=src.device)
    w = weight.contiguous().float()
    _lib.check(lib.seunet_conv3d_stream_pack(code, w.data_ptr(), ci_w, co_w, int(transpose_flip), src_c, dst_c, wbuf.data_ptr(), _s()),
               "conv3d_stream_pack")
    if dst is None:
        dst = torch.empty(tuple(src.shape[:4]) + (dst_c,), dtype=src.dtype, device=src.device)
    stats, slots = None, 0
    if want_stats:
        slots = lib.seunet_conv3d_stream_slots(dilation, dims)
        stats = torch.zeros((dims.n, slots, dst_c, 2), dtype=torch.float64, device=src.device)
    b = None
    if bias is not None:
        b = torch.zeros(dst_c, dtype=torch.float32, device=src.device)
        b[:bias.numel()] = bias.float()
    _lib.check(lib.seunet_conv3d_stream(code, dilation, src.data_ptr(), src_c, wbuf.data_ptr(), _lib.ptr(b), dst.data_ptr(), dst_c,
                                        int(accumulate), _lib.ptr(stats), dims, _s()), "conv3d_stream")
    return dst, stats, slots


def conv3d_march_supported(srcs: Sequence[torch.Tensor], dst_channels: Sequence[int], dilation: int = 1) -> bool:
    return bool(_lib.load().seunet_conv3d_march_supported(_code(srcs[0]), dilation, len(srcs), _lib.int_array([t.shape[4] for t in srcs]),
                                                          len(dst_channels), _lib.int_array(list(dst_channels))))


def conv3d_march(srcs: Sequence[torch.Tensor], weight: torch.Tensor, bias: Optional[torch.Tensor] = None, dilation: int = 1,
                 transpose_flip: bool = False, dsts: Optional[Sequence[Optional[torch.Tensor]]] = None,
                 dst_channels: Optional[Sequence[int]] = None, accumulate: Optional[Sequence[int]] = None, want_stats: bool = False):
    lib = _lib.load()
    code, dims = _code(srcs[0]), _dims_cl(srcs[0])
    co_w, ci_w = weight.shape[0], weight.shape[1]
    cout_e = ci_w if transpose_flip else co_w
    cin = sum(t.shape[4] for t in srcs)
    if dsts is None:
        dst_channels = list(dst_channels or [cout_e])
        dsts = [torch.empty(tuple(srcs[0].shape[:4]) + (c,), dtype=srcs[0].dtype, device=srcs[0].device) for c in dst_channels]
        accumulate = [0] * len(dsts)
    else:
        dst_channels = list(dst_channels or [t.shape[4] for t in dsts])
        accumulate = list(accumulate or [0] * len(dsts))
    if not conv3d_march_supported(srcs, dst_channels, dilation):
        raise RuntimeError(f"conv3d_march: {[t.shape[4] for t in srcs]} -> {dst_channels} channels, dilation {dilation}, "
                           f"dtype {srcs[0].dtype} is not served by this kernel")
    cout = sum(dst_channels)
    wbuf = torch.empty(lib.seunet_conv3d_march_wpack_bytes(cin, cout), dtype=torch.uint8, device=srcs[0].device)
    w = weight.contiguous().float()
    _lib.check(lib.seunet_conv3d_march_pack(code, w.data_ptr(), ci_w, co_w, int(transpose_flip), cin, cout, wbuf.data_ptr(), _s()),
               "conv3d_march_pack")
    stats, slots = None, 0
    if want_stats:
        slots = lib.seunet_conv3d_march_slots(dilation, cin, cout, dims)
        stats = torch.zeros((dims.n, slots, cout, 2), dtype=torch.float64, device=srcs[0].device)
    b = None
    if bias is not None:
        b = torch.zeros(cout, dtype=torch.float32, device=srcs[0].device)
        b[:bias.numel()] = bias.float()
    _lib.check(lib.seunet_conv3d_march(code, dilation, len(srcs), _lib.ptr_array(list(srcs)), _lib.int_array([t.shape[4] for t in srcs]),
                                       wbuf.data_ptr(), _lib.ptr(b), len(dsts), _lib.ptr_array(list(dsts)),
                                       _lib.int_array(dst_channels), _lib.int_array(accumulate), _lib.ptr(stats), dims, _s()),
               "conv3d_march")
    return list(dsts), stats, slots


def conv3d_wgrad(srcs: Sequence[torch.Tensor], dy: torch.Tensor, cin: int, cout: int, taps: int, dilation: int = 1,
                 impl: int = _lib.CONV_MFMA) -> torch.Tensor:
    lib = _lib.load()
    code = _code(dy)
    k = 3 if taps == 27 else 1
    dw = torch.empty((cout, cin, k, k, k), dtype=torch.float32, device=dy.device)
    nbytes = lib.seunet_conv3d_wgrad_workspace_bytes(taps, cin, cout)
    ws = torch.empty(nbytes, dtype=torch.uint8, device=dy.device)
    _lib.check(lib.seunet_conv3d_wgrad(code, impl, taps, dilation, len(srcs), _lib.ptr_array(list(srcs)),
                                       _lib.int_array([t.shape[4] for t in srcs]), cin, dy.data_ptr(), dy.shape[4],
                                       dw.data_ptr(), ws.data_ptr(), nbytes, _dims_cl(dy), _s()), "conv3d_wgrad")
    return dw


def conv3d_wgrad_stream(x: torch.Tensor, dy: torch.Tensor, cin: int, cout: int, dilation: int = 1) -> torch.Tensor:
    lib = _lib.load()
    code, dims = _code(dy), _dims_cl(dy)
    if not lib.seunet_conv3d_wgrad_stream_supported(code, dilation, x.shape[4], dy.shape[4]):
        raise RuntimeError(f"conv3d_wgrad_stream: {x.shape[4]} x {dy.shape[4]} channels, dilation {dilation} is not served by this kernel")
    dw = torch.empty((cout, cin, 3, 3, 3), dtype=torch.float32, device=dy.device)
    nbytes = lib.seunet_conv3d_wgrad_stream_workspace_bytes(x.shape[4], dy.shape[4], dilation, dims)
    ws = torch.empty(nbytes, dtype=torch.uint8, device=dy.device)
    _lib.check(lib.seunet_conv3d_wgrad_stream(code, dilation, x.data_ptr(), x.shape[4], cin, dy.data_ptr(), dy.shape[4], cout,
                                              dw.data_ptr(), ws.data_ptr(), nbytes, dims, _s()), "conv3d_wgrad_stream")
    return dw


def channel_stats(t: torch.Tensor) -> Tuple[torch.Tensor, int]:
    lib = _lib.load()
    dims = _dims_cl(t)
    slots = lib.seunet_epilogue_slots(dims)
    part = torch.zeros((dims.n, slots, t.shape[4], 2), dtype=torch.float64, device=t.device)
    _lib.check(lib.seunet_channel_stats(_code(t), t.data_ptr(), t.shape[4], part.data_ptr(), dims, _s()), "channel_stats")
    return part, slots


def stats_finalize(partial: torch.Tensor, slots: int, count: int, eps: float = 1e-5, mode: int = 0):
    n, _, c, _ = partial.shape
    a = torch.empty((n, c), dtype=torch.float32, device=partial.device)
    b = torch.empty_like(a)
    _lib.check(_lib.load().seunet_stats_finalize(partial.data_ptr(), slots, c, n, count, eps, mode, a.data_ptr(),
                                                 b.data_ptr(), _s()), "stats_finalize")
    return a, b


def gate_epilogue_fwd(raw, mean, rstd, w_se, w_se2, w_side, b_side, slope=0.01, level_map=None, level_accumulate=0,
                      head_w=None, drop=None, drop_stride=0, want_side=True):
    n, d, h, w, c = raw.shape
    e = torch.empty_like(raw)
    side = torch.empty((n, d, h, w, 2), dtype=torch.float32, device=raw.device) if want_side else None
    f = lambda t: None if t is None else t.contiguous().float().reshape(-1)
    ws, ws2, wsd, bsd, hw = f(w_se), f(w_se2), f(w_side), f(b_side), f(head_w)
    _lib.check(_lib.load().seunet_gate_epilogue_fwd(_code(raw), raw.data_ptr(), mean.data_ptr(), rstd.data_ptr(), c,
                                                    _lib.ptr(ws), _lib.ptr(ws2), _lib.ptr(wsd), _lib.ptr(bsd), slope,
                                                    e.data_ptr(), _lib.ptr(side), _lib.ptr(level_map), level_accumulate,
                                                    _lib.ptr(hw), _lib.ptr(drop), drop_stride, _dims_cl(raw), _s()),
               "gate_epilogue_fwd")
    return e, side


def gate_epilogue_bwd(raw, mean, rstd, w_se, w_se2, w_side, b_side, slope=0.01, g_e=None, g_side=None, g_level=None,
                      head_w=None, drop=None, drop_stride=0, fused_finalize=False):
    lib = _lib.load()
    n, d, h, w, c = raw.shape
    dims = _dims_cl(raw)
    slots = lib.seunet_epilogue_slots(dims)
    dx = torch.empty_like(raw)
    stat = torch.zeros((n, slots, c, 2), dtype=torch.float64, device=raw.device)
    pg = torch.zeros((n * slots, 4 * c + 4), dtype=torch.float32, device=raw.device)
    f = lambda t: None if t is None else t.contiguous().float().reshape(-1)
    ws, ws2, wsd, bsd, hw = f(w_se), f(w_se2), f(w_side), f(b_side), f(head_w)

    def call(m1, m2, out, st, pgp):
        _lib.check(lib.seunet_gate_epilogue_bwd(_code(raw), raw.data_ptr(), mean.data_ptr(), rstd.data_ptr(), c, _lib.ptr(ws),
                                                _lib.ptr(ws2), _lib.ptr(wsd), _lib.ptr(bsd), slope, _lib.ptr(g_e),
                                                _lib.ptr(g_side), _lib.ptr(g_level), _lib.ptr(hw), _lib.ptr(drop), drop_stride,
                                                _lib.ptr(m1), _lib.ptr(m2), _lib.ptr(out), _lib.ptr(st), _lib.ptr(pgp), dims, _s()),
                   "gate_epilogue_bwd")
    call(None, None, None, stat, pg)
    dev = raw.device
    out = {"dw_se": torch.empty(c, device=dev), "dw_se2": torch.empty(c, device=dev), "dw_side": torch.empty(2 * c, device=dev),
           "db_side": torch.empty(2, device=dev), "dhead_w": torch.empty(2, device=dev)}
    if fused_finalize:
        m1 = torch.empty((n, c), dtype=torch.float32, device=dev)
        m2 = torch.empty_like(m1)
        _lib.check(lib.seunet_gate_bwd_finalize(stat.data_ptr(), slots, c, n, d * h * w, m1.data_ptr(), m2.data_ptr(), pg.data_ptr(),
                                                n * slots, out["dw_se"].data_ptr(), _lib.ptr(None if ws2 is None else out["dw_se2"]),
                                                out["dw_side"].data_ptr(), out["db_side"].data_ptr(), out["dhead_w"].data_ptr(), _s()),
                   "gate_bwd_finalize")
        if ws2 is None:
            out["dw_se2"].zero_()
    else:
        m1, m2 = stats_finalize(stat, slots, d * h * w, 0.0, 1)
        _lib.check(lib.seunet_pgrad_reduce(pg.data_ptr(), n * slots, c, out["dw_se"].data_ptr(), out["dw_se2"].data_ptr(),
                                           out["dw_side"].data_ptr(), out["db_side"].data_ptr(), out["dhead_w"].data_ptr(), _s()),
                   "pgrad_reduce")
    call(m1, m2, dx, None, None)
    out["draw"], out["m1"], out["m2"] = dx, m1, m2
    return out


def cat_epilogue_fwd(raw, mean, rstd, raw2=None, mean2=None, rstd2=None, slope=0.01):
    out = torch.empty_like(raw)
    _lib.check(_lib.load().seunet_cat_epilogue_fwd(_code(raw), raw.data_ptr(), mean.data_ptr(), rstd.data_ptr(), _lib.ptr(raw2),
                                                   _lib.ptr(mean2), _lib.ptr(rstd2), raw.shape[4], slope, out.data_ptr(),
                                                   _dims_cl(raw), _s()), "cat_epilogue_fwd")
    return out


def cat_epilogue_bwd(g_out, raw, mean, rstd, raw2=None, mean2=None, rstd2=None, slope=0.01):
    lib = _lib.load()
    n, d, h, w, c = raw.shape
    dims = _dims_cl(raw)
    slots = lib.seunet_epilogue_slots(dims)
    dx = torch.empty_like(raw)
    dx2 = torch.empty_like(raw) if raw2 is not None else None
    st = torch.zeros((n, slots, c, 2), dtype=torch.float64, device=raw.device)
    st2 = torch.zeros_like(st) if raw2 is not None else None

    def call(m1, m2, m1b, m2b, o1, o2, s1, s2):
        _lib.check(lib.seunet_cat_epilogue_bwd(_code(raw), g_out.data_ptr(), raw.data_ptr(), mean.data_ptr(), rstd.data_ptr(),
                                               _lib.ptr(raw2), _lib.ptr(mean2), _lib.ptr(rstd2), c, slope, _lib.ptr(m1), _lib.ptr(m2),
                                               _lib.ptr(m1b), _lib.ptr(m2b), _lib.ptr(o1), _lib.ptr(o2), _lib.ptr(s1), _lib.ptr(s2),
                                               dims, _s()), "cat_epilogue_bwd")
    call(None, None, None, None, None, None, st, st2)
    m1, m2 = stats_finalize(st, slots, d * h * w, 0.0, 1)
    m1b, m2b = stats_finalize(st2, slots, d * h * w, 0.0, 1) if raw2 is not None else (None, None)
    call(m1, m2, m1b, m2b, dx, dx2, None, None)
    return dx, dx2


def xbranch_stats(x_in, w2, in_channel, eps=1e-5):
    lib = _lib.load()
    n, d, h, w, _ = x_in.shape
    dims = _dims_cl(x_in)
    c = w2.shape[0]
    w2f = w2.contiguous().float().reshape(c, in_channel)
    mslots = lib.seunet_xbranch_moment_slots(dims)
    mom = torch.zeros((n, mslots, 5), dtype=torch.float64, device=x_in.device)
    _lib.check(lib.seunet_xbranch_moments(_code(x_in), x_in.data_ptr(), mom.data_ptr(), dims, _s()), "xbranch_moments")
    mean2 = torch.empty((n, c), dtype=torch.float32, device=x_in.device)
    rstd2 = torch.empty_like(mean2)
    tot = torch.empty((n, 5), dtype=torch.float64, device=x_in.device)
    _lib.check(lib.seunet_xbranch_stats(mom.data_ptr(), mslots, w2f.data_ptr(), c, in_channel, n, d * h * w, eps, mean2.data_ptr(),
                                        rstd2.data_ptr(), tot.data_ptr(), _s()), "xbranch_stats")
    return mean2, rstd2, tot


def cat_epilogue_fwd_x(raw, mean, rstd, x_in, w2, in_channel, mean2, rstd2, slope=0.01):
    c = raw.shape[4]
    w2f = w2.contiguous().float().reshape(c, in_channel)
    out = torch.empty_like(raw)
    _lib.check(_lib.load().seunet_cat_epilogue_fwd_x(_code(raw), raw.data_ptr(), mean.data_ptr(), rstd.data_ptr(), x_in.data_ptr(),
                                                     w2f.data_ptr(), in_channel, mean2.data_ptr(), rstd2.data_ptr(), c, slope,
                                                     out.data_ptr(), _dims_cl(raw), _s()), "cat_epilogue_fwd_x")
    return out


def cat_epilogue_fwd_x_pool(raw, mean, rstd, x_in, w2, in_channel, mean2, rstd2, slope=0.01):
    n, d, h, w, c = raw.shape
    w2f = w2.contiguous().float().reshape(c, in_channel)
    out = torch.empty_like(raw)
    pooled = torch.empty((n, d // 2, h // 2, w // 2, c), dtype=raw.dtype, device=raw.device)
    words = torch.empty((n, (d // 2) * (h // 2) * (w // 2), c // 8), dtype=torch.int32, device=raw.device)
    _lib.check(_lib.load().seunet_cat_epilogue_fwd_x_pool(_code(raw), raw.data_ptr(), mean.data_ptr(), rstd.data_ptr(), x_in.data_ptr(),
                                                          w2f.data_ptr(), in_channel, mean2.data_ptr(), rstd2.data_ptr(), c, slope,
                                                          out.data_ptr(), pooled.data_ptr(), words.data_ptr(), _dims_cl(raw), _s()),
# ... 196 lines not shown
```

Before: 586.2 million.

## Batch small-level weight-gradient convolutions into grouped multi-job launches

Result: no change. 585.0 million (-0.2%).

```diff
diff --git a/include/seunet_hip.h b/include/seunet_hip.h
--- a/include/seunet_hip.h
+++ b/include/seunet_hip.h
@@ -55,6 +55,11 @@
 int seunet_conv3d_wgrad(int dtype, int impl, int taps, int dilation, int nsrc, const void* const* src, const int* src_c,
                         int cin, const void* dy, int cout, float* dw, void* workspace, size_t workspace_bytes,
                         seunet_dims dims, seunet_stream_t s);
+int seunet_conv3d_wgrad_batch_cut(int dtype, int njobs, const int* taps, const int* cin, const int* cout, const seunet_dims* dims,
+                                  int* groups, int* total_groups, size_t* bytes);
+int seunet_conv3d_wgrad_batch(int dtype, int njobs, const int* taps, const int* nsrc, const void* const* src, const int* src_c,
+                              const int* cin, const void* const* dy, const int* cout, float* const* dw, const seunet_dims* dims,
+                              void* workspace, size_t workspace_bytes, seunet_stream_t s);
 
 int seunet_epilogue_slots(seunet_dims dims);
 int seunet_channel_stats(int dtype, const void* t, int c, double* partial, seunet_dims dims, seunet_stream_t s);
@@ -303,6 +308,10 @@
   long long src_dist;
 } seunet_conv_info;
 int seunet_net_conv_info(const seunet_net_desc* desc, int index, seunet_conv_info* out);
+#define SEUNET_WGRAD_FLUSH_FULL 1
+#define SEUNET_WGRAD_FLUSH_DECODER 2
+#define SEUNET_WGRAD_FLUSH_END 3
+int seunet_net_wgrad_batched(const seunet_net_desc* desc, int index);
 int seunet_net_backward(const seunet_net_desc* desc, const float* const* params, const float* g_pred0,
                         const float* g_pred1, const float* drop1, const float* drop2, float* const* grads,
                         void* workspace, size_t workspace_bytes, seunet_stream_t s);
diff --git a/se-unet-airseg_amd/_lib.py b/se-unet-airseg_amd/_lib.py
--- a/se-unet-airseg_amd/_lib.py
+++ b/se-unet-airseg_amd/_lib.py
@@ -28,6 +28,7 @@
 
 KERNEL_NAIVE, KERNEL_TILED, KERNEL_STREAM, KERNEL_MARCH, KERNEL_WGRAD1X1 = range(5)
 KERNEL_NAMES = ("Naive", "Tiled", "Stream", "March", "Wgrad1x1")
+WGRAD_FLUSH_FULL, WGRAD_FLUSH_DECODER, WGRAD_FLUSH_END = 1, 2, 3
 
 
 class ConvInfo(C.Structure):
@@ -66,6 +67,8 @@
     "seunet_conv3d_wgrad_stream": (_i, [_i, _i, _vp, _i, _i, _vp, _i, _i, _vp, _vp, _sz, Dims, _vp]),
     "seunet_conv3d_wgrad_workspace_bytes": (_sz, [_i, _i, _i]),
     "seunet_conv3d_wgrad": (_i, [_i, _i, _i, _i, _i, _pp, _ip, _i, _vp, _i, _vp, _vp, _sz, Dims, _vp]),
+    "seunet_conv3d_wgrad_batch_cut": (_i, [_i, _i, _ip, _ip, _ip, C.POINTER(Dims), _ip, _ip, C.POINTER(C.c_size_t)]),
+    "seunet_conv3d_wgrad_batch": (_i, [_i, _i, _ip, _ip, _pp, _ip, _ip, _pp, _ip, _pp, C.POINTER(Dims), _vp, _sz, _vp]),
     "seunet_epilogue_slots": (_i, [Dims]),
     "seunet_channel_stats": (_i, [_i, _vp, _i, _vp, Dims, _vp]),
     "seunet_stats_finalize": (_i, [_vp, _i, _i, _i, _ll, _f, _i, _vp, _vp, _vp]),
@@ -168,6 +171,7 @@
     "seunet_graph_destroy": (_i, [_vp]),
     "seunet_net_read_tensor": (_i, [C.POINTER(NetDesc), _pp, _vp, _sz, C.c_char_p, _i, _vp, _ip, _vp]),
     "seunet_net_conv_info": (_i, [C.POINTER(NetDesc), _i, C.POINTER(ConvInfo)]),
+    "seunet_net_wgrad_batched": (_i, [C.POINTER(NetDesc), _i]),
     "seunet_net_backward": (_i, [C.POINTER(NetDesc), _pp, _vp, _vp, _vp, _vp, _pp, _vp, _sz, _vp]),
     "seunet_net_backward_ev": (_i, [C.POINTER(NetDesc), _pp, _vp, _vp, _vp, _vp, _pp, _vp, _sz, _vp, _vp]),
     "seunet_net_input_grad_bytes": (_sz, [C.POINTER(NetDesc)]),
diff --git a/se-unet-airseg_amd/csrc/abi.cpp b/se-unet-airseg_amd/csrc/abi.cpp
--- a/se-unet-airseg_amd/csrc/abi.cpp
+++ b/se-unet-airseg_amd/csrc/abi.cpp
@@ -166,6 +166,46 @@
   return run_wgrad(k, dtype, taps, dilation, sl, cin, dy, cout, dw, workspace, workspace_bytes, D(dims), S(s));
 }
 
+static int batch_jobs(int njobs, const int* taps, const int* nsrc, const void* const* src, const int* src_c, const int* cin,
+                      const void* const* dy, const int* cout, float* const* dw, const seunet_dims* dims, WgradJob* jobs) {
+  SEUNET_CHECK(taps && cin && cout && dims, "conv3d_wgrad_batch: null argument");
+  SEUNET_CHECK(njobs >= 1 && njobs <= WG_BATCH_JOBS, "conv3d_wgrad_batch: %d jobs in one batch (1 .. %d)", njobs, WG_BATCH_JOBS);
+  for (int j = 0; j < njobs; ++j) {
+    WgradJob& q = jobs[j];
+    q = WgradJob{};
+    if (nsrc) {
+      if (int e = make_src(nsrc[j], src + 3 * j, src_c + 3 * j, q.x)) return e;
+    } else {
+      q.x.n = 1; q.x.C[0] = (cin[j] + 7) / 8 * 8;
+    }
+    q.cin = cin[j]; q.cout = cout[j]; q.taps = taps[j];
+    q.dy = dy ? dy[j] : nullptr;
+    q.dw = dw ? dw[j] : nullptr;
+    q.d = D(dims[j]);
+  }
+  return 0;
+}
+int seunet_conv3d_wgrad_batch_cut(int dtype, int njobs, const int* taps, const int* cin, const int* cout, const seunet_dims* dims,
+                                  int* groups, int* total_groups, size_t* bytes) {
+  SEUNET_CHECK(groups && total_groups && bytes, "conv3d_wgrad_batch_cut: null argument");
+  WgradJob jobs[WG_BATCH_JOBS];
+  if (int e = batch_jobs(njobs, taps, nullptr, nullptr, nullptr, cin, nullptr, cout, nullptr, dims, jobs)) return e;
+  WgradCut cut;
+  if (int e = wgrad_batch_cut(dtype, jobs, njobs, &cut)) return e;
+  for (int j = 0; j < njobs; ++j) groups[j] = cut.G[j];
+  *total_groups = cut.total;
+  *bytes = cut.bytes;
+  return 0;
+}
+int seunet_conv3d_wgrad_batch(int dtype, int njobs, const int* taps, const int* nsrc, const void* const* src, const int* src_c,
+                              const int* cin, const void* const* dy, const int* cout, float* const* dw, const seunet_dims* dims,
+                              void* workspace, size_t workspace_bytes, seunet_stream_t s) {
+  SEUNET_CHECK(nsrc && src && src_c && dy && dw, "conv3d_wgrad_batch: null argument");
+  WgradJob jobs[WG_BATCH_JOBS];
+  if (int e = batch_jobs(njobs, taps, nsrc, src, src_c, cin, dy, cout, dw, dims, jobs)) return e;
+  return launch_wgrad_batch(dtype, jobs, njobs, workspace, workspace_bytes, S(s));
+}
+
 int seunet_epilogue_slots(seunet_dims dims) { return epi_partials(D(dims)); }
 int seunet_channel_stats(int dtype, const void* t, int c, double* partial, seunet_dims dims, seunet_stream_t s) {
   SEUNET_CHECK(t && partial, "channel_stats: null tensor");
diff --git a/se-unet-airseg_amd/csrc/net.cpp b/se-unet-airseg_amd/csrc/net.cpp
--- a/se-unet-airseg_amd/csrc/net.cpp
+++ b/se-unet-airseg_amd/csrc/net.cpp
@@ -222,6 +222,14 @@
       r.x_fwd = ConvKernel::Tiled;
       r.x_wgrad = wgrad_kernel(d.dtype, 1, 1, xs, d.in_channel, r.cout, dm, 0);
     }
+  }
+  static constexpr long long kWgradBatchVoxels = 131072;
+  bool wgrad_batched(int i) const {
+    const OpDesc& o = kOps[i];
+    if (o.kind != OP_GATED && o.kind != OP_CAT) return false;
+    const OpRes& r = op[i];
+    const Dims& dm = dims[kT[o.dst].level];
+    return r.wgrad == ConvKernel::Tiled && (r.taps == 1 || o.dil == 1) && (long long)dm.N * dm.vox() <= kWgradBatchVoxels;
   }
   size_t wpack_bytes(ConvKernel k, int taps, int src_c, int cin, int cout) const {
     switch (k) {
@@ -558,12 +566,36 @@
     return 0;
   }
 
+  std::vector<WgradJob> pending[2];
+
+  int flush_wgrad() {
+    if (pending[0].empty() && pending[1].empty()) return 0;
+    mark("wgrad_batch");
+    for (std::vector<WgradJob>& list : pending) {
+      if (list.empty()) continue;
+      WgradCut cut;
+      if (wgrad_batch_cut(p.d.dtype, list.data(), (int)list.size(), &cut) == 0 && cut.bytes <= p.wgrad_ws_bytes) {
+        if (int e = launch_wgrad_batch(p.d.dtype, list.data(), (int)list.size(), at(p.wgrad_ws), p.wgrad_ws_bytes, s)) return e;
+      } else {
+        for (const WgradJob& q : list)
+          if (int e = launch_wgrad(p.d.dtype, q.taps, 1, q.x, q.cin, q.dy, q.cout, q.dw, at(p.wgrad_ws), p.wgrad_ws_bytes, q.d, s)) return e;
+      }
+      list.clear();
+    }
+    return 0;
+  }
+
   int conv_backward(int i, const SrcList& x, float* const* grads, bool* written) {
     const OpDesc& o = kOps[i];
     const OpRes& r = p.op[i];
     const int lv = kT[o.dst].level;
     const int wi = opp[i].conv1_w;
-    if (grads[wi]) {
+    if (grads[wi] && p.wgrad_batched(i)) {
+      std::vector<WgradJob>& list = pending[r.taps == 27 ? 0 : 1];
+      list.push_back(WgradJob{x, r.cin, at(p.grad[o.dst]), r.cout, grads[wi], p.dims[lv], r.taps});
+      if ((int)list.size() == WG_BATCH_JOBS)
+        if (int e = flush_wgrad()) return e;
+    } else if (grads[wi]) {
       mark("wgrad:", o.name);
       if (int e = run_wgrad(r.wgrad, p.d.dtype, r.taps, o.dil, x, r.cin, at(p.grad[o.dst]), r.cout, grads[wi], at(p.wgrad_ws),
                             p.wgrad_ws_bytes, p.dims[lv], s)) return e;
@@ -622,8 +654,9 @@
       const OpDesc& o = kOps[i];
       const OpRes& r = p.op[i];
       const BlockParams& bp = opp[i];
-      if (decoder_done && strcmp(o.name, "up0") == 0) {
-        SEUNET_HIP(hipEventRecord(decoder_done, s));
+      if (strcmp(o.name, "up0") == 0) {
+        if (int e = flush_wgrad()) return e;
+        if (decoder_done) SEUNET_HIP(hipEventRecord(decoder_done, s));
       }
       if (o.kind == OP_POOL || o.kind == OP_UP) {
         const int t = o.src[0];
@@ -717,6 +750,7 @@
         if (int e = conv_backward(i, srcs(o), grads, written)) return e;
       }
     }
+    if (int e = flush_wgrad()) return e;
     if (!zero_ptrs.empty()) {
       mark("stats");
       if (int e = launch_multi_zero(zero_ptrs.data(), zero_counts.data(), (int)zero_ptrs.size(), s)) return e;
@@ -900,6 +934,32 @@
   return fail("net_conv_info: index %d is past the last convolution (%d)", index, seen);
 }
 
+int seunet_net_wgrad_batched(const seunet_net_desc* desc, int index) {
+  if (!desc) { (void)fail("net_wgrad_batched: null descriptor"); return -1; }
+  Plan p;
+  if (p.init(*desc)) return -1;
+  int flush[kNumOps] = {};
+  std::vector<int> open[2];
+  auto close = [&](int code) {
+    for (std::vector<int>& l : open) { for (int i : l) flush[i] = code; l.clear(); }
+  };
+  for (int i = kNumOps - 1; i >= 0; --i) {
+    if (strcmp(kOps[i].name, "up0") == 0) close(SEUNET_WGRAD_FLUSH_DECODER);
+    if (!p.wgrad_batched(i)) continue;
+    std::vector<int>& l = open[p.op[i].taps == 27 ? 0 : 1];
+    l.push_back(i);
+    if ((int)l.size() == WG_BATCH_JOBS) close(SEUNET_WGRAD_FLUSH_FULL);
+  }
+  close(SEUNET_WGRAD_FLUSH_END);
+  int seen = 0;
+  for (int i = 0; i < kNumOps; ++i) {
+    if (kOps[i].kind != OP_GATED && kOps[i].kind != OP_CAT) continue;
+    if (seen++ == index) return flush[i];
+  }
+  (void)fail("net_wgrad_batched: index %d is not a convolution (0 .. %d)", index, seen - 1);
+  return -1;
+}
+
 int seunet_net_backward(const seunet_net_desc* desc, const float* const* params, const float* g_pred0,
                         const float* g_pred1, const float* drop1, const float* drop2, float* const* grads,
                         void* workspace, size_t workspace_bytes, seunet_stream_t s) {
diff --git a/se-unet-airseg_amd/csrc/seunet_common.h b/se-unet-airseg_amd/csrc/seunet_common.h
--- a/se-unet-airseg_amd/csrc/seunet_common.h
+++ b/se-unet-airseg_amd/csrc/seunet_common.h
@@ -273,6 +273,11 @@
 size_t wgrad_workspace_bytes(int taps, int cin, int cout);
 int launch_wgrad(int dtype, int taps, int dil, const SrcList& x, int cin_logical, const void* dy,
                  int cout, float* dw_torch, void* workspace, size_t ws_bytes, Dims d, hipStream_t s);
+static constexpr int WG_BATCH_JOBS = 8;
+struct WgradJob { SrcList x; int cin; const void* dy; int cout; float* dw; Dims d; int taps; };
+struct WgradCut { int G[WG_BATCH_JOBS], first[WG_BATCH_JOBS + 1], combos[WG_BATCH_JOBS], tiles[WG_BATCH_JOBS], total; size_t bytes; };
+int wgrad_batch_cut(int dtype, const WgradJob* jobs, int n, WgradCut* cut);
+int launch_wgrad_batch(int dtype, const WgradJob* jobs, int n, void* workspace, size_t ws_bytes, hipStream_t s);
 bool wgrad_march_supported(int dtype, int taps, int dil, const SrcList& x, int cin_logical, int cout, Dims d, long long src_dist);
 int launch_wgrad_march(int dtype, int taps, int dil, const SrcList& x, int cin_logical, const void* dy, int cout,
                        float* dw, void* workspace, size_t ws_bytes, Dims d, hipStream_t s);
diff --git a/se-unet-airseg_amd/csrc/wgrad.hip b/se-unet-airseg_amd/csrc/wgrad.hip
--- a/se-unet-airseg_amd/csrc/wgrad.hip
+++ b/se-unet-airseg_amd/csrc/wgrad.hip
@@ -1,6 +1,7 @@
 #include "seunet_common.h"
 #include "mfma.h"
 #include <climits>
+#include <cstddef>
 #include <cstdlib>
 
 namespace seunet {
@@ -39,8 +40,7 @@
 #endif
 
 template <typename T, int TAPS, int DIL, int NW>
-__global__ void __launch_bounds__(NW * 64, NW == 4 ? 2 : 4)
-wgrad_kernel(WgArgs a) {
+__device__ __forceinline__ void wgrad_tiles(const WgArgs& a, const int combo, const int g, const int G, const size_t slab_index) {
 #ifdef SEUNET_STAMP
   unsigned long long ph[6] = {0, 0, 0, 0, 0, 0};
   unsigned long long t_last = __builtin_readcyclecounter();
@@ -64,7 +64,6 @@
 
   const int tid = threadIdx.x, lane = tid & 63, wave = tid >> 6;
   const int col = lane & 31, h = lane >> 5;
-  const int combo = blockIdx.y;
   const int ci0 = (combo / a.co_tiles) * 32, co0 = (combo % a.co_tiles) * 32;
   const long long V = (long long)a.D * a.H * a.W;
   const int tiles_per_par = a.tx * a.ty * a.tz;
@@ -191,7 +190,7 @@
   };
 
   WSTAMP(0);
-  for (int tile = blockIdx.x; tile < total_tiles; tile += gridDim.x) {
+  for (int tile = g; tile < total_tiles; tile += G) {
     __syncthreads();
     WSTAMP(1);
     stage(tile);
@@ -275,7 +274,7 @@
     WSTAMP(4);
   }
   if (TAPS == 27) {
-    float* out = a.slab + ((size_t)combo * gridDim.x + blockIdx.x) * (27 * 1024);
+    float* out = a.slab + slab_index * (27 * 1024);
 #pragma unroll
     for (int ti = 0; ti < NT; ++ti) {
       const int tap = wave + NW * ti;
@@ -298,7 +297,7 @@
       part[wave * 1024 + row * 32 + cc] = acc[0][r];
     }
     __syncthreads();
-    float* out = a.slab + ((size_t)combo * gridDim.x + blockIdx.x) * 1024;
+    float* out = a.slab + slab_index * 1024;
     for (int e = tid; e < 1024; e += NW * 64) {
       float t = part[e];
 #pragma unroll
@@ -309,20 +308,44 @@
 #ifdef SEUNET_STAMP
   WSTAMP(5);
   if (a.debug != nullptr && lane == 0) {
-    const size_t w = ((size_t)blockIdx.y * gridDim.x + blockIdx.x) * NW + wave;
+    const size_t w = slab_index * NW + wave;
     for (int i = 0; i < 6; ++i) a.debug[w * 12 + i] = ph[i];
     for (int i = 6; i < 12; ++i) a.debug[w * 12 + i] = 0;
   }
 #endif
 }
 
-__global__ void __launch_bounds__(256)
-wgrad_reduce_kernel(const float* __restrict__ slab, int nslab, int taps, int cin_w, int cout_w, int co_tiles,
-                    float* __restrict__ dw) {
+template <typename T, int TAPS, int DIL, int NW>
+__global__ void __launch_bounds__(NW * 64, NW == 4 ? 2 : 4)
+wgrad_kernel(WgArgs a) {
+  wgrad_tiles<T, TAPS, DIL, NW>(a, blockIdx.y, blockIdx.x, gridDim.x, (size_t)blockIdx.y * gridDim.x + blockIdx.x);
+}
+
+struct WgBatchArgs {
+  WgArgs job[WG_BATCH_JOBS];
+  int first[WG_BATCH_JOBS + 1];
+  int G[WG_BATCH_JOBS];
+  int n;
+};
+
+template <typename T, int TAPS, int NW>
+__global__ void __launch_bounds__(NW * 64, NW == 4 ? 2 : 4)
+wgrad_batch_kernel(WgBatchArgs b) {
+  const int wg = blockIdx.x;
+  int j = 0;
+#pragma unroll
+  for (int k = 1; k < WG_BATCH_JOBS; ++k) j += (k < b.n && wg >= b.first[k]) ? 1 : 0;
+  const int local = wg - b.first[j], G = b.G[j];
+  static_assert(offsetof(WgBatchArgs, job) == 0, "the job list leads the kernel arguments");
+  const WgArgs& a = ((const WgArgs*)__builtin_amdgcn_kernarg_segment_ptr())[__builtin_amdgcn_readfirstlane(j)];
+  wgrad_tiles<T, TAPS, 1, NW>(a, local / G, local % G, G, (size_t)wg);
+}
+
+__device__ __forceinline__ void wgrad_reduce_block(const float* __restrict__ slab, int nslab, int taps, int cin_w, int cout_w,
+                                                   int co_tiles, int combo, int e0, float* __restrict__ dw) {
   const int per = taps * 1024;
   const int el = threadIdx.x & 15, part = threadIdx.x >> 4;
-  const int e = blockIdx.x * 16 + el;
-  const int combo = blockIdx.y;
+  const int e = e0 + el;
   const float* p = slab + (size_t)combo * nslab * per + e;
   double s0 = 0.0, s1 = 0.0;
   int k = part;
@@ -341,6 +364,26 @@
     const int tap = e >> 10, ci = (combo / co_tiles) * 32 + ((e >> 5) & 31), co = (combo % co_tiles) * 32 + (e & 31);
     if (ci < cin_w && co < cout_w) dw[((size_t)co * cin_w + ci) * taps + tap] = (float)t;
   }
+}
+
+__global__ void __launch_bounds__(256)
+wgrad_reduce_kernel(const float* __restrict__ slab, int nslab, int taps, int cin_w, int cout_w, int co_tiles,
+                    float* __restrict__ dw) {
+  wgrad_reduce_block(slab, nslab, taps, cin_w, cout_w, co_tiles, blockIdx.y, blockIdx.x * 16, dw);
+}
+
+struct WgReduceJob { float* dw; int first, G, cin, cout, co_tiles, combo0; };
+struct WgReduceBatch { WgReduceJob job[WG_BATCH_JOBS]; int n, taps; };
+
+__global__ void __launch_bounds__(256)
+wgrad_reduce_batch_kernel(const float* __restrict__ slab, WgReduceBatch b) {
+  const int pair = blockIdx.y;
+  int j = 0;
+#pragma unroll
+  for (int k = 1; k < WG_BATCH_JOBS; ++k) j += (k < b.n && pair >= b.job[k].combo0) ? 1 : 0;
+  const WgReduceJob& q = b.job[j];
+  wgrad_reduce_block(slab + (size_t)q.first * b.taps * 1024, q.G, b.taps, q.cin, q.cout, q.co_tiles, pair - q.combo0,
+                     blockIdx.x * 16, q.dw);
 }
 
 static inline int wgrad_groups(int combos, int total_tiles) {
@@ -421,6 +464,106 @@
   return 0;
 }
 
+static inline int wgrad_tiles_of(int dtype, Dims d) {
+  const int tz = dtype_size(dtype) == 2 ? WgTile<bf16_t>::TZ : WgTile<float>::TZ;
+  const int ty = dtype_size(dtype) == 2 ? WgTile<bf16_t>::TY : WgTile<float>::TY;
+  return cdiv(d.W, 32) * cdiv(d.H, ty) * cdiv(d.D, tz) * d.N;
+}
+
+int wgrad_batch_cut(int dtype, const WgradJob* jobs, int n, WgradCut* cut) {
+  SEUNET_CHECK(jobs && cut, "wgrad_batch: null argument");
+  SEUNET_CHECK(dtype_ok(dtype), "wgrad_batch: dtype %d unsupported", dtype);
+  SEUNET_CHECK(n >= 1 && n <= WG_BATCH_JOBS, "wgrad_batch: %d jobs in one batch (1 .. %d)", n, WG_BATCH_JOBS);
+  const int taps = jobs[0].taps;
+  SEUNET_CHECK(taps == 27 || taps == 1, "wgrad_batch: taps=%d unsupported", taps);
+  long long weight = 0;
+  int pairs = 0;
+  for (int j = 0; j < n; ++j) {
+    const WgradJob& q = jobs[j];
+    SEUNET_CHECK(q.taps == taps, "wgrad_batch: mixed taps in one batch (job 0 has %d, job %d has %d)", taps, j, q.taps);
+    SEUNET_CHECK(q.x.n >= 1 && q.x.n <= 3, "wgrad_batch: job %d: 1..3 sources", j);
+    SEUNET_CHECK(q.cout >= 8 && q.cout % 8 == 0 && q.cin >= 1 && q.cin <= q.x.total(), "wgrad_batch: job %d: bad channel counts", j);
+    SEUNET_CHECK(q.d.N >= 1 && q.d.D >= 1 && q.d.H >= 1 && q.d.W >= 1, "wgrad_batch: job %d: bad extents", j);
+    cut->tiles[j] = wgrad_tiles_of(dtype, q.d);
+    cut->combos[j] = cdiv(q.cin, 32) * cdiv(q.cout, 32);
+    pairs += cut->combos[j];
+    weight += (long long)cut->tiles[j] * cut->combos[j];
+  }
+  SEUNET_CHECK(pairs <= WG_TILED_SLABS, "wgrad_batch: %d (job, combo) pairs exceed the %d workgroups of a launch", pairs, WG_TILED_SLABS);
+  const long long spare = WG_TILED_SLABS - pairs;
+  int total = 0;
+  for (int j = 0; j < n; ++j) {
+    long long g = 1 + spare * cut->tiles[j] / weight;
+    if (g > cut->tiles[j]) g = cut->tiles[j];
+    cut->G[j] = (int)g;
+    cut->first[j] = total;
+    total += (int)g * cut->combos[j];
+  }
+  cut->first[n] = total;
+  cut->total = total;
+  cut->bytes = 256 + (size_t)total * taps * 1024 * sizeof(float);
+  return 0;
+}
+
+template <typename T, int TAPS, int NW>
+static int wgrad_launch_batch(const WgBatchArgs& b, int groups, hipStream_t s) {
+  constexpr int HALO = (TAPS == 27) ? 1 : 0;
+  constexpr int TZ = WgTile<T>::TZ, TY = WgTile<T>::TY;
+  constexpr int PPV = 32 / (16 / (int)sizeof(T));
+  constexpr int NVH = (TZ + 2 * HALO) * (TY + 2 * HALO) * (32 + 2 * HALO), NVT = TZ * TY * 32;
+  constexpr int LDS = PPV * ((((NVH + 63) / 64) * 64 + 4) + (((NVT + 63) / 64) * 64 + 4)) * 16 + NW * 64 * 32;
+  static unsigned long long configured = 0;
+  if (int e = configure_kernel_lds(configured, reinterpret_cast<const void*>(&wgrad_batch_kernel<T, TAPS, NW>), LDS)) return e;
+  wgrad_batch_kernel<T, TAPS, NW><<<dim3(groups), NW * 64, LDS, s>>>(b);
+  SEUNET_LAUNCH_CHECK();
+  return 0;
+}
+
+int launch_wgrad_batch(int dtype, const WgradJob* jobs, int n, void* workspace, size_t ws_bytes, hipStream_t s) {
+  WgradCut cut;
+  if (int e = wgrad_batch_cut(dtype, jobs, n, &cut)) return e;
+  SEUNET_CHECK(workspace != nullptr, "wgrad_batch: null workspace");
+  SEUNET_CHECK(ws_bytes >= cut.bytes, "wgrad_batch: workspace too small (%zu < %zu bytes)", ws_bytes, cut.bytes);
+  for (int j = 0; j < n; ++j) SEUNET_CHECK(jobs[j].dy && jobs[j].dw && jobs[j].x.ptr[0], "wgrad_batch: job %d: null tensor", j);
+  const void* zero = device_zero_page();
+  SEUNET_CHECK(zero != nullptr, "wgrad_batch: cannot allocate the device zero page");
+  float* slab = reinterpret_cast<float*>(reinterpret_cast<unsigned char*>(workspace) + 256);
+  const int taps = jobs[0].taps;
+  const int tz = dtype_size(dtype) == 2 ? WgTile<bf16_t>::TZ : WgTile<float>::TZ;
+  const int ty = dtype_size(dtype) == 2 ? WgTile<bf16_t>::TY : WgTile<float>::TY;
+  WgBatchArgs b{};
+  WgReduceBatch r{};
+  b.n = r.n = n;
+  r.taps = taps;
+  int pairs = 0;
+  for (int j = 0; j < n; ++j) {
+    const WgradJob& q = jobs[j];
+    WgArgs& a = b.job[j];
+    wg_sources(a, q.x, q.cin);
+    a.dy = q.dy; a.cout = q.cout;
+    a.zero = zero;
+    a.slab = slab;
+    a.N = q.d.N; a.D = q.d.D; a.H = q.d.H; a.W = q.d.W;
+    a.tx = cdiv(q.d.W, 32); a.ty = cdiv(q.d.H, ty); a.tz = cdiv(q.d.D, tz);
+    a.co_tiles = cdiv(q.cout, 32);
+    a.debug = nullptr;
+    b.first[j] = cut.first[j];
+    b.G[j] = cut.G[j];
+    r.job[j] = WgReduceJob{q.dw, cut.first[j], cut.G[j], q.cin, q.cout, a.co_tiles, pairs};
+    pairs += cut.combos[j];
+  }
+  b.first[n] = cut.total;
+  int e;
+  SEUNET_DTYPE_SWITCH(dtype, {
+    if (taps == 1) e = wgrad_launch_batch<T, 1, 4>(b, cut.total, s);
+    else e = wgrad_launch_batch<T, 27, 4>(b, cut.total, s);
+  });
+  if (e) return e;
+  wgrad_reduce_batch_kernel<<<dim3(taps * 1024 / 16, pairs), 256, 0, s>>>(slab, r);
+  SEUNET_LAUNCH_CHECK();
+  return 0;
+}
+
 template <typename T>
 __global__ void wgrad_naive_kernel(WgArgs a, int taps, int dil, float* __restrict__ dw, long long total) {
   const long long V = (long long)a.D * a.H * a.W;
diff --git a/se-unet-airseg_amd/ops.py b/se-unet-airseg_amd/ops.py
--- a/se-unet-airseg_amd/ops.py
+++ b/se-unet-airseg_amd/ops.py
@@ -174,6 +174,37 @@
     return dw
 
 
+def conv3d_wgrad_batch_cut(code: int, jobs: Sequence[Tuple[int, int, int, Tuple[int, int, int, int]]]):
+    lib = _lib.load()
+    n = len(jobs)
+    groups, total, nbytes = (C.c_int * max(n, 1))(), C.c_int(), C.c_size_t()
+    dims = (Dims * max(n, 1))(*[Dims(*j[3]) for j in jobs])
+    _lib.check(lib.seunet_conv3d_wgrad_batch_cut(code, n, _lib.int_array([j[0] for j in jobs]), _lib.int_array([j[1] for j in jobs]),
+                                                 _lib.int_array([j[2] for j in jobs]), dims, groups, C.byref(total), C.byref(nbytes)),
+               "conv3d_wgrad_batch_cut")
+    return [groups[j] for j in range(n)], total.value, nbytes.value
+
+
+def conv3d_wgrad_batch(jobs: Sequence[Tuple[Sequence[torch.Tensor], torch.Tensor, int, int]], taps: int) -> List[torch.Tensor]:
+    lib = _lib.load()
+    code = _code(jobs[0][1])
+    k = 3 if taps == 27 else 1
+    _, _, nbytes = conv3d_wgrad_batch_cut(code, [(taps, cin, cout, tuple(dy.shape[:4])) for _, dy, cin, cout in jobs])
+    dev = jobs[0][1].device
+    dws = [torch.empty((cout, cin, k, k, k), dtype=torch.float32, device=dev) for _, _, cin, cout in jobs]
+    ws = torch.empty(nbytes, dtype=torch.uint8, device=dev)
+    src, src_c = [], []
+    for srcs, _, _, _ in jobs:
+        src += list(srcs) + [None] * (3 - len(srcs))
+        src_c += [t.shape[4] for t in srcs] + [0] * (3 - len(srcs))
+    dims = (Dims * len(jobs))(*[_dims_cl(dy) for _, dy, _, _ in jobs])
+    _lib.check(lib.seunet_conv3d_wgrad_batch(code, len(jobs), _lib.int_array([taps] * len(jobs)), _lib.int_array([len(j[0]) for j in jobs]),
+                                             _lib.ptr_array(src), _lib.int_array(src_c), _lib.int_array([j[2] for j in jobs]),
+                                             _lib.ptr_array([j[1] for j in jobs]), _lib.int_array([j[3] for j in jobs]),
+                                             _lib.ptr_array(dws), dims, ws.data_ptr(), nbytes, _s()), "conv3d_wgrad_batch")
+    return dws
+
+
 def conv3d_wgrad_stream(x: torch.Tensor, dy: torch.Tensor, cin: int, cout: int, dilation: int = 1) -> torch.Tensor:
     lib = _lib.load()
     code, dims = _code(dy), _dims_cl(dy)
```
